# NJU-3DV/Relightable3DGaussian

Hardware: AMD Instinct MI355X
Metric: train iters/s, synthetic lego-like 800x800, 300000 Gaussians (stage-2 hot path) (higher is better)
Workload: dtype f32; 1 GPU; stage-2 train iteration (fused glue kernels + one-launch Adam): shading fwd/bwd (K=64) + rasterize fwd (S=16) + loss + rasterize bwd + Adam; 1 view/rank/step, 300000 Gaussians, 800x800, num_rendered~1755016; parallelism=dp1

## Files before the change

### include/r3dg_hip.h

```cpp
#ifndef R3DG_HIP_H
#define R3DG_HIP_H

#include <stddef.h>
#include <stdint.h>

#ifdef __cplusplus
extern "C" {
#endif

#define R3DG_OK 0
#define R3DG_EINVAL (-1)
#define R3DG_EHIP (-2)
#define R3DG_EALLOC (-3)

typedef void* (*r3dg_alloc_fn)(void* user, size_t bytes);

const char* r3dg_last_error(void);
int r3dg_release_scratch(void);
int r3dg_version(void);

int r3dg_max_features_forward(void);
int r3dg_max_features_backward(void);

size_t r3dg_geometry_state_bytes(int P);
size_t r3dg_image_state_bytes(int width, int height);
size_t r3dg_binning_state_bytes(int64_t num_rendered);
int r3dg_geometry_state_offsets(int P, size_t* offsets9);
size_t r3dg_geometry_state_total_offset(int P);
int r3dg_image_state_offsets(int width, int height, size_t* offsets3);
int r3dg_binning_state_offsets(int64_t num_rendered, size_t* offsets4);

int r3dg_rasterize_forward(void* stream, r3dg_alloc_fn geometry_alloc, r3dg_alloc_fn binning_alloc,
                           r3dg_alloc_fn image_alloc, void* alloc_user, int P, int S, int D, int M,
                           const float* d_background, int width, int height, const float* d_means3D,
                           const float* d_shs, const float* d_colors_precomp, const float* d_features,
                           const float* d_opacities, const float* d_scales, float scale_modifier,
                           const float* d_rotations, const float* d_cov3D_precomp, const float* d_viewmatrix,
                           const float* d_projmatrix, const float* d_cam_pos, float tan_fovx, float tan_fovy,
                           float cx, float cy, int prefiltered, int compute_pseudo_normal, float* d_out_color,
                           float* d_out_opacity, float* d_out_depth, float* d_out_feature, float* d_out_normal,
                           float* d_out_surface_xyz, float* d_out_weights, int32_t* d_radii, int debug,
                           int* num_rendered_out);

int r3dg_rasterize_forward_begin(void* stream, r3dg_alloc_fn geometry_alloc, r3dg_alloc_fn binning_alloc,
                                 r3dg_alloc_fn image_alloc, void* alloc_user, int P, int S, int D, int M,
                                 const float* d_background, int width, int height, const float* d_means3D,
                                 const float* d_shs, const float* d_colors_precomp, const float* d_features,
                                 const float* d_opacities, const float* d_scales, float scale_modifier,
                                 const float* d_rotations, const float* d_cov3D_precomp, const float* d_viewmatrix,
                                 const float* d_projmatrix, const float* d_cam_pos, float tan_fovx, float tan_fovy,
                                 float cx, float cy, int prefiltered, int compute_pseudo_normal, float* d_out_color,
                                 float* d_out_opacity, float* d_out_depth, float* d_out_feature, float* d_out_normal,
                                 float* d_out_surface_xyz, float* d_out_weights, int32_t* d_radii, int debug,
                                 void** ticket);
int r3dg_rasterize_forward_finish(void* ticket, int* num_rendered_out);
int r3dg_rasterize_forward_finish_on(void* ticket, void* ordering_stream, int* num_rendered_out);

int r3dg_bounded_forward_supported(int width, int height);
int r3dg_rasterize_forward_begin_bounded(void* stream, r3dg_alloc_fn geometry_alloc, r3dg_alloc_fn binning_alloc,
                                         r3dg_alloc_fn image_alloc, void* alloc_user, int P, int S, int D, int M,
                                         const float* d_background, int width, int height, const float* d_means3D,
                                         const float* d_shs, const float* d_colors_precomp, const float* d_features,
                                         const float* d_opacities, const float* d_scales, float scale_modifier,
                                         const float* d_rotations, const float* d_cov3D_precomp,
                                         const float* d_viewmatrix, const float* d_projmatrix, const float* d_cam_pos,
                                         float tan_fovx, float tan_fovy, float cx, float cy, int prefiltered,
                                         int compute_pseudo_normal, float* d_out_color, float* d_out_opacity,
                                         float* d_out_depth, float* d_out_feature, float* d_out_normal,
                                         float* d_out_surface_xyz, float* d_out_weights, int32_t* d_radii, int debug,
                                         void* ordering_stream, long long capacity, float* d_overflow_flag,
                                         unsigned int* d_overflow_count, void** ticket);
int r3dg_rasterize_forward_finish_bounded(void* ticket, void* main_stream);

int r3dg_rasterize_backward(void* stream, int P, int S, int D, int M, int R, const float* d_background, int width,
                            int height, const float* d_means3D, const float* d_shs, const float* d_features,
                            const float* d_colors_precomp, const float* d_scales, float scale_modifier,
                            const float* d_rotations, const float* d_cov3D_precomp, const float* d_viewmatrix,
                            const float* d_projmatrix, const float* d_campos, float tan_fovx, float tan_fovy,
                            const int32_t* d_radii, const void* d_geom_buffer, const void* d_binning_buffer,
                            const void* d_img_buffer, const float* d_dL_dpix, const float* d_dL_dpix_o,
                            const float* d_dL_dpix_d, const float* d_dL_dpix_f, float* d_dL_dmean2D,
                            float* d_dL_dconic, float* d_dL_dopacity, float* d_dL_dcolor, float* d_dL_dfeature,
                            float* d_dL_dmean3D, float* d_dL_dcov3D, float* d_dL_dsh, float* d_dL_dscale,
                            float* d_dL_drot, int backward_geometry, int debug);

int r3dg_rasterize_backward_split(void* stream, void* geometry_stream, int P, int S, int D, int M, int R,
                                  const float* d_background, int width, int height, const float* d_means3D,
                                  const float* d_shs, const float* d_features, const float* d_colors_precomp,
                                  const float* d_scales, float scale_modifier, const float* d_rotations,
                                  const float* d_cov3D_precomp, const float* d_viewmatrix, const float* d_projmatrix,
                                  const float* d_campos, float tan_fovx, float tan_fovy, const int32_t* d_radii,
                                  const void* d_geom_buffer, const void* d_binning_buffer, const void* d_img_buffer,
                                  const float* d_dL_dpix, const float* d_dL_dpix_o, const float* d_dL_dpix_d,
                                  const float* d_dL_dpix_f, float* d_dL_dmean2D, float* d_dL_dconic,
                                  float* d_dL_dopacity, float* d_dL_dcolor, float* d_dL_dfeature, float* d_dL_dmean3D,
                                  float* d_dL_dcov3D, float* d_dL_dsh, float* d_dL_dscale, float* d_dL_drot,
                                  int backward_geometry, int debug, int n_active_features,
                                  const int* active_features);

int r3dg_rasterize_backward_features(void* stream, int P, int S, int R, int width, int height, const void* d_geom_buffer,
                                     const void* d_binning_buffer, const void* d_img_buffer, const float* d_dL_dpix_f,
                                     float* d_dL_dfeature, int n_active_features, const int* active_features, int debug);

int r3dg_mark_visible(void* stream, int P, const float* d_means3D, const float* d_viewmatrix,
                      const float* d_projmatrix, uint8_t* d_present);

int r3dg_shade_forward(void* stream, int P, int K, int M, const float* d_base_color, const float* d_roughness,
                       const float* d_normals, const float* d_viewdirs, const float* d_incidents, const float* d_env,
                       int He, int We, const float* d_env_transform, const float* d_visibility,
                       const float* d_incident_dirs, const float* d_incident_areas, float* d_out);
#define R3DG_SHADE_TRAIN_OUTPUTS 1
#define R3DG_SHADE_TAPS_ARE_RADIANCE 2
#define R3DG_SHADE_LEAVE_ROOM 4
#define R3DG_SHADE_ROTATED 8
int r3dg_shade_forward_cached(void* stream, int P, int K, int M, const float* d_base_color, const float* d_roughness,
                              const float* d_normals, const float* d_viewdirs, const float* d_incidents,
                              const float* d_env, int He, int We, const float* d_env_transform,
                              const float* d_visibility, const float* d_incident_dirs, const float* d_incident_areas,
                              float uniform_area, const uint32_t* d_taps, int flags, float* d_out);
int r3dg_shade_build_taps(void* stream, int64_t num_samples, const float* d_incident_dirs, const float* d_env_transform,
                          int He, int We, const float* d_env_radiance, uint32_t* d_taps);
int r3dg_shade_build_transport(void* stream, int P, int K, int M, const float* d_normals, const float* d_incidents,
                               const float* d_visibility, const float* d_incident_dirs, const float* d_incident_areas,
                               float uniform_area, float* d_radiance_inout, float* d_consts);
int r3dg_shade_forward_transport(void* stream, int P, int K, const float* d_base_color, const float* d_roughness,
                                 const float* d_normals, const float* d_viewdirs, const float* d_transport,
                                 const float* d_consts, const float* d_zsamples, const float* d_incident_dirs,
                                 float* d_out);
int r3dg_shade_build_transport_rayset(void* stream, int P, int K, int M, const float* d_normals, const float* d_incidents,
                                      const float* d_visibility, const float* d_zsamples, float uniform_area,
                                      const float* d_env, int He, int We, const float* d_env_transform,
                                      float* d_transport, float* d_consts);
int r3dg_shade_build_transport_baked(void* stream, int P, int K, int M, const float* d_normals, const float* d_incidents,
                                     const float* d_visibility_sh, const float* d_zsamples, float uniform_area,
                                     const float* d_env, int He, int We, const float* d_env_transform,
                                     float* d_transport, float* d_consts);
int r3dg_visibility_sh_expand(void* stream, int P, int K, const float* d_normals, const float* d_zsamples,
                              const float* d_visibility_sh, float* d_visibility_out);
int r3dg_shade_build_split(void* stream, int P, int K, const int32_t* d_perm, const float* d_normals, const float* d_incidents,
                           const float* d_visibility, const float* d_incident_dirs, const float* d_zsamples,
                           float uniform_area, float* d_lt, float* d_vis_t, float* d_consts);
size_t r3dg_shade_env_footprints_bytes(int He, int We);
int r3dg_shade_env_footprints(void* stream, int He, int We, const float* d_env, float* d_env_footprints);
int r3dg_shade_forward_split(void* stream, int P, int K, const int32_t* d_perm, const float* d_base_color,
                             const float* d_roughness, const float* d_normals, const float* d_viewdirs, const float* d_lt,
                             const float* d_vis_t, const float* d_consts, const float* d_zsamples,
                             const float* d_env_transform, const float* d_env_footprints, int He, int We, float* d_out);
int r3dg_shade_frs_supported(int K, int M, int He, int We);
size_t r3dg_shade_frs_tables_bytes(int K);
int r3dg_shade_frs_build_tables(void* stream, int K, const float* d_zsamples, float* d_tables);
int r3dg_shade_frs_classify(void* stream, int P, const float* d_ray_normals, uint8_t* d_valid);
int r3dg_shade_frs_build_taps(void* stream, int P, int K, const float* d_ray_normals, const float* d_zsamples, int He, int We,
                              uint32_t* d_taps);
int r3dg_stream_wait_stream(void* waiter, void* signaller);
int r3dg_spin(void* stream, float microseconds);
int r3dg_store_u64_to_host(void* stream, const void* d_src, void* h_pinned_dst);
int r3dg_clock_probe(void* stream, int iters, unsigned long long* d_out3, float* d_sink, int* wall_clock_khz);

int r3dg_shade_frs_rotate(void* stream, int P, const float* d_incidents, const float* d_ray_normals, float* d_cprime);
int r3dg_shade_frs_forward(void* stream, int P, int K, const float* d_base_color, const float* d_roughness,
                           const float* d_normals, const float* d_viewdirs, const float* d_incidents, const float* d_env,
                           int He, int We, const float* d_visibility, float uniform_area, const uint32_t* d_taps,
                           const float* d_ray_normals, const float* d_zsamples, const float* d_tables,
                           const uint8_t* d_valid, const int32_t* d_invalid_list, int n_invalid, float* d_cprime, int flags,
                           float* d_out, void* listed_stream, float* d_feature_rows);
int r3dg_shade_frs_backward(void* stream, int P, int K, const float* d_base_color, const float* d_roughness,
                            const float* d_normals, const float* d_viewdirs, const float* d_incidents, const float* d_env,
                            int He, int We, const float* d_visibility, float uniform_area, const uint32_t* d_taps,
                            const float* d_ray_normals, const float* d_zsamples, const float* d_tables,
                            const uint8_t* d_valid, const int32_t* d_invalid_list, int n_invalid, const float* d_cprime,
                            float* d_dcprime, const float* d_dL_dpbr, const float* d_dL_ddiffuse_light,
                            float* d_dL_dbase_color, float* d_dL_droughness, float* d_dL_dviewdirs, float* d_dL_dincidents,
                            float* d_dL_denv, const float* d_block_absmax, int n_block_absmax, void* rotate_stream);
#define R3DG_SHADE_NO_ROTATION_BACK ((void*)(intptr_t)-1)
#define R3DG_CHAIN_LISTED_ROWS_IN_DCPRIME 1
#define R3DG_CHAIN_NO_GRADIENT_OUT 2
int r3dg_shade_frs_incident_chain(void* stream, int P, const float* d_ray_normals, const uint8_t* d_valid,
                                  const float* d_dcprime, float* d_dL_dincidents, float* d_incidents, float* d_exp_avg,
                                  float* d_exp_avg_sq, float* d_cprime, float lr, float lr_tail, float beta1, float beta2,
                                  float eps, int step, float grad_scale, const float* d_skip_flag, int chain_flags);

int r3dg_shade_backward(void* stream, int P, int K, int M, const float* d_base_color, const float* d_roughness,
                        const float* d_normals, const float* d_viewdirs, const float* d_incidents, const float* d_env,
                        int He, int We, const float* d_env_transform, const float* d_visibility,
                        const float* d_incident_dirs, const float* d_incident_areas, const float* d_dL_dpbr,
                        const float* d_dL_ddiffuse_light, float* d_dL_dbase_color, float* d_dL_droughness,
                        float* d_dL_dviewdirs, float* d_dL_dincidents, float* d_dL_denv);

int r3dg_shade_backward_cached(void* stream, int P, int K, int M, const float* d_base_color, const float* d_roughness,
                               const float* d_normals, const float* d_viewdirs, const float* d_incidents,
                               const float* d_env, int He, int We, const float* d_env_transform,
                               const float* d_visibility, const float* d_incident_dirs, const float* d_incident_areas,
                               const uint32_t* d_taps, const float* d_dL_dpbr, const float* d_dL_ddiffuse_light,
                               float* d_dL_dbase_color, float* d_dL_droughness, float* d_dL_dviewdirs,
                               float* d_dL_dincidents, float* d_dL_denv, const float* d_block_absmax,
                               int n_block_absmax);

int r3dg_render_equation_forward(void* stream, int P, int Si, int Sd, int Sv, const float* d_base_color,
                                 const float* d_roughness, const float* d_metallic, const float* d_normals,
                                 const float* d_viewdirs, const float* d_incidents_shs, const float* d_direct_shs,
                                 const float* d_visibility_shs, int sample_num, const float* d_rand_float,
                                 float* d_incident_dirs, float* d_pbr, float* d_diffuse_light);
int r3dg_render_equation_forward_complex(void* stream, int P, int Si, int Sd, int Sv, const float* d_base_color,
                                         const float* d_roughness, const float* d_metallic, const float* d_normals,
                                         const float* d_viewdirs, const float* d_incidents_shs,
                                         const float* d_direct_shs, const float* d_visibility_shs, int sample_num,
                                         float* d_incident_dirs, float* d_pbr, float* d_incident_lights,
                                         float* d_local_incident_lights, float* d_global_incident_lights,
                                         float* d_incident_visibility, float* d_diffuse_light,
                                         float* d_local_diffuse_light, float* d_accum, float* d_rgb_d, float* d_rgb_s);
int r3dg_render_equation_backward(void* stream, int P, int Si, int Sd, int Sv, const float* d_base_color,
                                  const float* d_roughness, const float* d_metallic, const float* d_normals,
                                  const float* d_viewdirs, const float* d_incidents_shs, const float* d_direct_shs,
                                  const float* d_visibility_shs, int sample_num, const float* d_incident_dirs,
                                  const float* d_dL_dpbr, const float* d_dL_ddiffuse_light, float* d_dL_dbase_color,
                                  float* d_dL_droughness, float* d_dL_dmetallic, float* d_dL_dnormals,
                                  float* d_dL_dviewdirs, float* d_dL_dincidents_shs, float* d_dL_ddirect_shs,
                                  float* d_dL_dvisibility_shs);

#define R3DG_SUM_SLOTS 32

int r3dg_stage2_activate(void* stream, int P, const float* d_xyz, const float* d_scaling_raw,
                         const float* d_rotation_raw, const float* d_opacity_raw, const float* d_normal_raw,
                         const float* d_base_raw, const float* d_rough_raw, const float* d_campos, float* d_scales,
                         float* d_rotations, float* d_opacity, float* d_normal, float* d_base_color,
                         float* d_roughness, float* d_viewdirs, const float* d_viewmatrix, float* d_features);
int r3dg_stage2_pack_features(void* stream, int P, const float* d_xyz, const float* d_viewmatrix, const float* d_normal,
                              const float* d_base_color, const float* d_roughness, const float* d_shade_out,
                              float* d_features, float* d_light_l1_sum);
int r3dg_stage2_unpack_gradients(void* stream, int P, const float* d_dL_dfeatures, const float* d_shade_out,
                                 float light_weight, float* d_dL_dpbr, float* d_dL_ddiffuse_light,
                                 float* d_block_absmax, float* d_light_l1_sum);
int r3dg_stage2_activate_backward(void* stream, int P, const float* d_xyz, const float* d_scaling_raw,
                                  const float* d_rotation_raw, const float* d_opacity_raw, const float* d_normal_raw,
                                  const float* d_base_raw, const float* d_rough_raw, const float* d_viewmatrix,
                                  const float* d_campos, const float* d_dL_dfeatures, const float* d_dL_dbase_color,
                                  const float* d_dL_droughness, const float* d_dL_dviewdirs, const float* d_dL_dscales,
                                  const float* d_dL_drotations, const float* d_dL_dopacity, const float* d_dL_dmeans3D,
                                  float* d_g_xyz, float* d_g_scaling, float* d_g_rotation, float* d_g_opacity,
                                  float* d_g_normal, float* d_g_base, float* d_g_rough);
int r3dg_stage2_loss(void* stream, int width, int height, const float* d_image, const float* d_opacity,
                     const float* d_feature, const float* d_pseudo_normal, const int32_t* d_n_contrib,
                     const float* d_gt, const float* d_background, const float* d_image_mask, float w_l1, float w_pbr,
                     float w_normal, const float* d_extra_dL_dimage, const float* d_extra_dL_dsrgb, float* d_dL_dimage,
                     float* d_dL_dopacity, float* d_dL_dfeature, float* d_sums,
                     int sparse_feature_gradients);
int r3dg_stage2_smooth_forward(void* stream, int width, int height, const float* d_opacity, const float* d_feature,
                               const int32_t* d_n_contrib, const float* d_gt, const float* d_image_mask,
                               float w_base_color, float w_roughness, float w_light, float* d_scratch, float* d_sums3);
int r3dg_stage2_smooth_backward(void* stream, int width, int height, const float* d_opacity, const float* d_feature,
                                const int32_t* d_n_contrib, const float* d_image_mask, const float* d_scratch,
                                float w_base_color, float w_roughness, float w_light, int accumulate_normal,
                                float* d_dL_dopacity, float* d_dL_dfeature);
int r3dg_stage2_smooth_fused(void* stream, int width, int height, const float* d_opacity, const float* d_feature,
                             const int32_t* d_n_contrib, const float* d_gt, const float* d_image_mask, float w_base_color,
                             float w_roughness, float w_light, int accumulate_normal, float* d_dL_dopacity,
                             float* d_dL_dfeature, float* d_sums3);
int r3dg_stage2_pbr_srgb(void* stream, int width, int height, const float* d_opacity, const float* d_feature,
                         const int32_t* d_n_contrib, const float* d_background, float* d_srgb);

int r3dg_stage2_activate_with(void* stream, int P, const float* d_xyz, const float* d_scaling_raw,
                              const float* d_rotation_raw, const float* d_opacity_raw, const float* d_normal_raw,
                              const float* d_base_raw, const float* d_rough_raw, const float* d_campos, float* d_scales,
                              float* d_rotations, float* d_opacity, float* d_normal, float* d_base_color,
                              float* d_roughness, float* d_viewdirs, const float* d_viewmatrix, float* d_features,
                              int n_env, const float* d_env_raw, float* d_env, float* d_zero, int n_zero);
int r3dg_stage2_activate_backward_with(void* stream, int P, const float* d_xyz, const float* d_scaling_raw,
                                       const float* d_rotation_raw, const float* d_opacity_raw, const float* d_normal_raw,
                                       const float* d_base_raw, const float* d_rough_raw, const float* d_viewmatrix,
                                       const float* d_campos, const float* d_dL_dfeatures, const float* d_dL_dbase_color,
                                       const float* d_dL_droughness, const float* d_dL_dviewdirs, const float* d_dL_dscales,
                                       const float* d_dL_drot, const float* d_dL_dopacity, const float* d_dL_dmeans3D,
                                       float* d_g_xyz, float* d_g_scaling, float* d_g_rotation, float* d_g_opacity,
                                       float* d_g_normal, float* d_g_base, float* d_g_rough, int He, int We,
                                       const float* d_env_raw, const float* d_env, float* d_dL_denv, float w_tv,
                                       float* d_g_env_raw, float* d_tv_sum, int consume);
int r3dg_stage2_normals_srgb(void* stream, int width, int height, const float* d_viewmatrix, float tan_fovx, float tan_fovy,
                             float cx, float cy, const float* d_opacity, const float* d_depth, float* d_pseudo_normal,
                             float* d_surface_xyz, const float* d_feature, const int32_t* d_n_contrib,
                             const float* d_background, float* d_srgb);

int r3dg_ssim_forward(void* stream, int width, int height, int channels, const float* d_x, const float* d_y,
                      float* d_partials, float* d_sum);
int r3dg_ssim_backward(void* stream, int width, int height, int channels, const float* d_x, const float* d_y,
                       const float* d_partials, float scale, float* d_grad_x);
int r3dg_ssim_forward_pair(void* stream, int width, int height, int channels, const float* d_x0, const float* d_x1,
                           const float* d_y, float* d_partials0, float* d_partials1, float* d_sum0, float* d_sum1);
int r3dg_ssim_backward_pair(void* stream, int width, int height, int channels, const float* d_x0, const float* d_x1,
                            const float* d_y, const float* d_partials0, const float* d_partials1, float scale0,
                            float scale1, float* d_grad_x0, float* d_grad_x1);

int r3dg_stage1_pack_features(void* stream, int P, const float* d_xyz, const float* d_viewmatrix, const float* d_normal,
                              float* d_features);
int r3dg_stage1_loss(void* stream, int width, int height, const float* d_image, const float* d_opacity,
                     const float* d_feature, const float* d_pseudo_normal, const int32_t* d_n_contrib, const float* d_gt,
                     const float* d_image_mask, float w_l1, float w_mask_entropy, float w_normal, float w_normal_smooth,
                     float w_depth_var, const float* d_extra_dL_dimage, float* d_edge_scratch, float* d_dL_dimage,
                     float* d_dL_dopacity, float* d_dL_dfeature, float* d_sums);
int r3dg_stage1_activate_backward(void* stream, int P, const float* d_xyz, const float* d_scaling_raw,
                                  const float* d_rotation_raw, const float* d_opacity_raw, const float* d_normal_raw,
                                  const float* d_viewmatrix, const float* d_dL_dfeatures, const float* d_dL_dscales,
                                  const float* d_dL_drotations, const float* d_dL_dopacity, const float* d_dL_dmeans3D,
                                  float* d_g_xyz, float* d_g_scaling, float* d_g_rotation, float* d_g_opacity,
                                  float* d_g_normal);

int r3dg_supervision_count(void* stream, int width, int height, const float* d_gt_depth, const float* d_image_mask,
                           uint32_t* d_count);
int r3dg_stage2_supervision(void* stream, int width, int height, const float* d_opacity, const float* d_feature,
                            const int32_t* d_n_contrib, const float* d_gt_depth, const float* d_mvs_normal,
                            const float* d_image_mask, const uint32_t* d_count, float w_depth, float w_normal_mvs,
                            int accumulate_normal, float* d_dL_dopacity, float* d_dL_dfeature, float* d_sums2);
int r3dg_stage1_depth_smooth(void* stream, int width, int height, const float* d_opacity, const float* d_feature,
                             const int32_t* d_n_contrib, const float* d_gt, float w_depth_smooth, float* d_edge_scratch,
                             float* d_dL_dopacity, float* d_dL_dfeature, float* d_sum);
int r3dg_stage1_gaussian_terms(void* stream, int P, const float* d_weights, const float* d_opacity, const float* d_normal,
                               const float* d_scales, const float* d_xyz, const float* d_campos, float w_point_entropy,
                               float w_orientation, float w_scaling, float* d_dL_dopacity, float* d_dL_dfeatures,
                               float* d_dL_dscales, float* d_dL_dmeans3D, float* d_sums3);

int r3dg_stage2_env_backward(void* stream, int He, int We, const float* d_raw, const float* d_env, float* d_dL_denv,
                             float w_tv, float* d_g_raw, float* d_tv_sum, int consume);

#define R3DG_ADAM_MAX_GROUPS 16
typedef struct r3dg_adam_group {
    float* param;
    const float* grad;
    float* exp_avg;
    float* exp_avg_sq;
    uint64_t n;
    float lr, lr_tail;
    uint32_t period, split;
} r3dg_adam_group;
int r3dg_adam_step(void* stream, int n_groups, const r3dg_adam_group* groups, float beta1, float beta2, float eps,
                   int step, float grad_scale, const float* d_skip_flag);

int r3dg_rasterize_backward_sh_adam_supported(int M);
int r3dg_rasterize_backward_split_sh_adam(void* stream, void* geometry_stream, int P, int S, int D, int M, int R,
                                          const float* d_background, int width, int height, const float* d_means3D,
                                          const float* d_shs, const float* d_features, const float* d_colors_precomp,
                                          const float* d_scales, float scale_modifier, const float* d_rotations,
                                          const float* d_cov3D_precomp, const float* d_viewmatrix,
                                          const float* d_projmatrix, const float* d_campos, float tan_fovx, float tan_fovy,
                                          const int32_t* d_radii, const void* d_geom_buffer, const void* d_binning_buffer,
                                          const void* d_img_buffer, const float* d_dL_dpix, const float* d_dL_dpix_o,
                                          const float* d_dL_dpix_d, const float* d_dL_dpix_f, float* d_dL_dmean2D,
                                          float* d_dL_dconic, float* d_dL_dopacity, float* d_dL_dcolor,
                                          float* d_dL_dfeature, float* d_dL_dmean3D, float* d_dL_dcov3D, float* d_dL_dsh,
                                          float* d_dL_dscale, float* d_dL_drot, int backward_geometry, int debug,
                                          int n_active_features, const int* active_features,
                                          const r3dg_adam_group* sh_adam, float beta1, float beta2, float eps, int step,
                                          float grad_scale, const float* d_skip_flag);

int r3dg_relight_pack_features(void* stream, int P, const float* d_xyz, const float* d_viewmatrix, const float* d_normal,
                               const float* d_base_color, const float* d_roughness, const float* d_shade_out,
                               float* d_features);
int r3dg_relight_compose(void* stream, int width, int height, float focal_x, float focal_y, float cx, float cy,
                         const float* d_viewmatrix, const float* d_light_transform, const float* d_envmap, int He, int We,
                         const float* d_image, const float* d_opacity, const float* d_feature,
                         const int32_t* d_n_contrib, float* d_pbr_env, float* d_render_env, float* d_env_only);

#define R3DG_EVAL_ROW 8
#define R3DG_EVAL_MEDIAN_STATE_WORDS 1024
int r3dg_relight_capture(void* stream, int width, int height, const float* d_feature, const float* d_opacity,
                         const int32_t* d_n_contrib, const float* d_background, const float* d_mask, float* d_pbr,
                         float* d_base_color, float* d_roughness, float* d_normal, float* d_visibility, float* d_diffuse,
                         float* d_specular, float* d_lights, float* d_local_lights, float* d_global_lights,
                         float* d_depth_var);
int r3dg_eval_image_metrics(void* stream, int width, int height, int channels, const float* d_pred, const float* d_gt,
                            const float* d_mask, const float* d_fill, int fill_is_image, double* d_tile_sums,
                            double* d_row);
int r3dg_eval_median_ratio(void* stream, int width, int height, const float* d_pred, const float* d_gt,
                           const float* d_mask, uint32_t* d_state, double* d_row);

#define R3DG_SCENE_COLUMNS 130
#define R3DG_SCENE_STAGE1_COLUMNS 62
#define R3DG_SCENE_GROUPS 13
#define R3DG_SCENE_MAX_COLUMNS 250
#define R3DG_SCENE_PLACEMENT_FLOATS 111
#define R3DG_SCENE_ZERO_INCIDENTS 1
#define R3DG_SCENE_ROTATE_SH 2
int r3dg_scene_place_records(void* stream, int P, int A, const float* d_records, const int32_t* d_column_map,
                             const float* d_placement, int flags, long long row_offset, void** dst_groups);
int r3dg_scene_place_groups(void* stream, int P, void** src_groups, const float* d_placement, int flags,
                            long long row_offset, void** dst_groups);
int r3dg_scene_pack_records(void* stream, int P, int columns, void** src_groups, float* d_records);

int r3dg_relight_quantize(void* stream, int width, int height, int channels, const float* d_image, uint8_t* d_bytes);

int r3dg_view_unpack(void* stream, int width, int height, int channels, const uint8_t* d_pixels, const float* d_background,
                     float* d_image, float* d_mask);

int r3dg_view_unpack_masked(void* stream, int width, int height, const uint8_t* d_pixels, const uint8_t* d_mask_bytes,
                            float* d_image, float* d_mask);

#define R3DG_VIEW_RESIZE_MAX_SCALE 16
int r3dg_view_resize(void* stream, int width, int height, int channels, const uint8_t* d_pixels, const uint8_t* d_mask_bytes,
                     const float* d_background, int out_width, int out_height, float* d_image, float* d_mask);

int r3dg_densify_accumulate(void* stream, int P, const float* d_viewspace_grad, const float* d_normal_grad,
                            const int32_t* d_radii, const float* d_weights, float* d_xyz_gradient_accum,
                            float* d_normal_gradient_accum, float* d_denom, float* d_weights_accum,
                            float* d_max_radii2D,
                            const float* d_skip_flag);

typedef struct r3dg_densify_config {
    int32_t mode;
    int32_t n_split;
    float grad_threshold, grad_normal_threshold, min_opacity, weights_threshold;
    float dense_size, world_size_limit, split_divisor, max_screen_size;
} r3dg_densify_config;

size_t r3dg_densify_temp_bytes(int P);
int r3dg_densify_plan(void* stream, int P, const r3dg_densify_config* config, const float* d_scaling_raw,
                      const float* d_opacity_raw, const float* d_xyz_gradient_accum,
                      const float* d_normal_gradient_accum, const float* d_denom, const float* d_weights_accum,
                      const float* d_max_radii2D, int32_t* d_src_row, int32_t* d_kind, int32_t* d_counts, void* d_temp);

#define R3DG_DENSIFY_MAX_GROUPS 24
#define R3DG_DENSIFY_ROLE_COPY 0
#define R3DG_DENSIFY_ROLE_XYZ 1
#define R3DG_DENSIFY_ROLE_SCALING 2
typedef struct r3dg_densify_group {
    const float* src_param;
    const float* src_exp_avg;
    const float* src_exp_avg_sq;
    float* dst_param;
    float* dst_exp_avg;
    float* dst_exp_avg_sq;
    uint32_t row_floats, role;
} r3dg_densify_group;
int r3dg_densify_gather(void* stream, int rows_out, const int32_t* d_src_row, const int32_t* d_kind, int n_groups,
                        const r3dg_densify_group* groups, const float* d_xyz, const float* d_scaling_raw,
                        const float* d_rotation_raw, const float* d_normal_table, float split_divisor);

int r3dg_reset_opacity(void* stream, int P, float* d_opacity_raw, float* d_exp_avg, float* d_exp_avg_sq);

size_t r3dg_knn_temp_bytes(int P);
int r3dg_knn_dist2(void* stream, int P, const float* d_points, float* d_mean_dist2, void* d_temp);

size_t r3dg_bvh_build_temp_bytes(int P);
int r3dg_bvh_build(void* stream, int P, int32_t* d_nodes, float* d_aabbs, int64_t* d_morton, void* d_temp);
int r3dg_bvh_trace_opacity(void* stream, int64_t num_rays, int num_gaussians, const int32_t* d_nodes, const float* d_aabbs,
                           const float* d_rays_o, const float* d_rays_d, const float* d_means3D,
                           const float* d_covs3D, const float* d_opacities, const float* d_normals,
                           int32_t* d_num_contributes, float* d_rendered_opacity, int32_t* d_stack_overflow);

size_t r3dg_bvh_trace_records_bytes(int num_gaussians);
int r3dg_bvh_pack_traversal(void* stream, int num_gaussians, const int32_t* d_nodes, const float* d_aabbs,
                            const float* d_means3D, const float* d_covs3D, const float* d_opacities,
                            const float* d_normals, void* d_records);
int r3dg_bvh_trace_opacity_packed(void* stream, int64_t num_rays, int num_gaussians, void* d_records, const float* d_rays_o,
                                  const float* d_rays_d, int32_t* d_num_contributes, float* d_rendered_opacity,
                                  int32_t* d_stack_overflow);

int r3dg_bvh_prepare_leaves(void* stream, int P, const float* d_means3D, const float* d_scales, const float* d_rotations,
                            int32_t* d_nodes, float* d_aabbs, float* d_covs3D_inv);
int r3dg_bvh_trace_bundles(void* stream, int num_gaussians, int K, void* d_records, const int32_t* d_nodes,
                           const float* d_zsamples, int leaf_lo, int leaf_hi, float origin_offset, float* d_visibility,
                           int32_t* d_num_contributes, float* d_dirs_out, int32_t* d_stack_overflow);

int r3dg_bvh_trace_hemisphere(void* stream, int num_gaussians, int T, void* d_records, const int32_t* d_nodes,
                              const float* d_raw_dirs, int leaf_lo, int leaf_hi, float origin_offset, float* d_visibility,
                              float* d_dirs_out, int32_t* d_num_contributes, int32_t* d_stack_overflow);
int r3dg_visibility_sh_fit(void* stream, int P, int T, int64_t steps_done, const float* d_dirs, const float* d_visibility,
                           float lr, float beta1, float beta2, float eps, float* d_coeffs, float* d_exp_avg,
                           float* d_exp_avg_sq, float* d_loss_partials);
int r3dg_visibility_sh_fit_loss_rows(int P);
int r3dg_bvh_trace_visits(void* stream, int num_gaussians, const void* d_records, uint64_t* node_and_leaf_steps);

int r3dg_bvh_trace_count(void* stream, int64_t num_rays, const int32_t* d_nodes, const float* d_aabbs,
                         const float* d_rays_o, const float* d_rays_d, int32_t* d_num_contributes,
                         int32_t* d_stack_overflow);
int r3dg_bvh_trace_fill(void* stream, int64_t num_rays, const int32_t* d_nodes, const float* d_aabbs,
                        const float* d_rays_o, const float* d_rays_d, const float* d_means3D,
                        const int32_t* d_num_contributes, const int64_t* d_offsets_inclusive, uint64_t* d_keys,
                        int32_t* d_point_list, float* d_position_list, int32_t* d_ray_id_list);

size_t r3dg_sort_temp_bytes(int64_t n);
int r3dg_sort_pairs(void* stream, int64_t n, uint64_t* d_keys_in, uint32_t* d_vals_in, uint64_t* d_keys_out,
                    uint32_t* d_vals_out, int end_bit, void* d_temp);

enum r3dg_option {
    R3DG_OPT_TILE_ORDER = 0,
    R3DG_OPT_CULL,
    R3DG_OPT_TILE_BINNING,
    R3DG_OPT_BINNING_BLOCK_K,
    R3DG_OPT_STAGE_SH_ROWS,
    R3DG_OPT_SHADE_FWD_BLOCKS_PER_CU,
    R3DG_OPT_TRACE_FORMULATION,
    R3DG_OPT_TRACE_REFILL,
    R3DG_OPT_TRACE_NODE_WEIGHT,
    R3DG_OPT_TRACE_LEAF_WEIGHT,
    R3DG_OPT_RESERVE_CUS,
    R3DG_OPT_TRACE_COUNT_VISITS,
    R3DG_OPT_BWD_LEAN,
    R3DG_OPT_COUNT
};
int r3dg_set_option(int option, int value);
int r3dg_get_option(int option, int* value);
void* r3dg_context_create(void);
void r3dg_context_destroy(void* ctx);
int r3dg_context_set_option(void* ctx, int option, int value);
int r3dg_context_make_current(void* ctx, void** previous);
int r3dg_selftest_transpose_reduce(void* stream, int N, int dpp, const float* d_in, float* d_out, int* d_chan,
                                   int* d_owner);

int r3dg_profile_enable(int on);
int r3dg_profile_pause(int paused);
int r3dg_profile_num_stages(void);
const char* r3dg_profile_stage_name(int stage);
int r3dg_profile_read(double* ms_out, int* count_out);

#ifdef __cplusplus
}
#endif
#endif
```

### relightable3dgaussian_amd/_abi.py

```python
import ctypes as C
import os
import re

HEADER = os.path.join(os.path.dirname(os.path.dirname(os.path.abspath(__file__))), "include", "r3dg_hip.h")
ALLOC_FN = C.CFUNCTYPE(C.c_void_p, C.c_void_p, C.c_size_t)
_ALLOC_FN_DECL = "typedef void* (*r3dg_alloc_fn)(void* user, size_t bytes)"

_SCALARS = {"int": C.c_int, "unsigned int": C.c_uint, "long long": C.c_longlong, "unsigned long long": C.c_ulonglong,
            "float": C.c_float, "double": C.c_double, "size_t": C.c_size_t, "int32_t": C.c_int32, "uint32_t": C.c_uint32,
            "int64_t": C.c_int64, "uint64_t": C.c_uint64, "uint8_t": C.c_uint8}
_RETURNS = dict(_SCALARS, **{"void": None, "void *": C.c_void_p, "const char *": C.c_char_p})
_HOST_POINTEES = ("int", "size_t", "double", "uint64_t")
_INT_EXPR = r"(?:0[xX][0-9a-fA-F]+|\d+|<<|>>|[\s()+\-*|&~])+"


def parse(text):
    def fail(pos, what):
        raise ValueError("r3dg_hip.h:%d: %s" % (text.count("\n", 0, pos) + 1, what))

    def blank(m):
        return "\n" * m.group(0).count("\n")

    def declarator(pos, decl, what):
        tok = decl.replace("*", " * ").split()
        name = tok.pop() if tok else ""
        stars = tok.count("*")
        base = " ".join(t for t in tok if t not in ("const", "*"))
        if not re.fullmatch(r"[A-Za-z_]\w*", name) or name in _SCALARS or not base or tok[len(tok) - stars:] != ["*"] * stars:
            fail(pos, "%s %r is not `type name`" % (what, decl.strip()))
        return base, stars, name

    text = re.sub(r"/\*.*?\*/", blank, text, flags=re.S)
    text = re.sub(r"^#ifdef __cplusplus\n.*?^#endif", blank, text, flags=re.S | re.M)
    prototypes, constants, structs = {}, {}, {}

    def define(m):
        name, value = m.group(1), m.group(2).strip()
        if name.startswith("R3DG_") and value:
            if name == "R3DG_SHADE_NO_ROTATION_BACK":
                value = "-1"
            if not re.fullmatch(_INT_EXPR, value):
                fail(m.start(), "#define %s: %r is not an integer expression" % (name, value))
            constants[name] = int(eval(value, {"__builtins__": {}}))
        return ""
    text = re.sub(r"^#[ \t]*define[ \t]+(\w+)(.*)$", define, text, flags=re.M)
    text = re.sub(r"^#.*$", "", text, flags=re.M)

    def struct(m):
        fields = []
        for decl in filter(str.strip, m.group(2).split(";")):
            first, *more = decl.split(",")
            for d in [first] + [declarator(m.start(), first, "field")[0] + " " + d for d in more]:
                base, stars, name = declarator(m.start(), d, "field")
                if base not in _SCALARS or stars > 1:
                    fail(m.start(), "field %r: unknown type" % d.strip())
                fields.append((name, C.c_void_p if stars else _SCALARS[base]))
        structs[m.group(1)] = type(m.group(1), (C.Structure,), {"_fields_": fields})
        return blank(m)
    text = re.sub(r"typedef\s+struct\s+(r3dg_\w+)\s*\{([^{}]*)\}\s*\1\s*;", struct, text)

    enum = re.search(r"enum\s+r3dg_option\s*\{([^{}]*)\}\s*;", text)
    entries = [[s.strip() for s in e.split("=")] for e in enum.group(1).split(",")] if enum else [[""]]
    if any(not re.fullmatch(r"R3DG_OPT_[A-Z0-9_]+", e[0]) or e[1:] not in ([], [str(i)]) for i, e in enumerate(entries)) or \
            entries[-1][0] != "R3DG_OPT_COUNT":
        fail(enum.start() if enum else 0, "enum r3dg_option: expected R3DG_OPT_* numbered from 0, R3DG_OPT_COUNT last")
    options = tuple(e[0][len("R3DG_OPT_"):] for e in entries[:-1])
    text = text[:enum.start()] + blank(enum) + text[enum.end():]

    for m in re.finditer(r"\s*([^;]*[^;\s])\s*;?", text):
        stmt, at = " ".join(m.group(1).split()), m.start(1)
        if stmt == _ALLOC_FN_DECL:
            continue
        p = re.fullmatch(r"([\w\s*]+?)\s*\b(r3dg_\w+)\s*\(([^()]*)\)", stmt)
        ret = " ".join(p.group(1).replace("*", " * ").split()) if p else None
        if ret not in _RETURNS:
            fail(at, "not a prototype this reader understands: %r" % stmt)
        args = []
        for decl in ([] if p.group(3).strip() == "void" else p.group(3).split(",")):
            base, stars, name = declarator(at, decl, p.group(2) + ": parameter")
            known = base in _SCALARS or (base == "void" and stars > 0)
            if stars == 0 and (known or base == "r3dg_alloc_fn"):
                args.append(ALLOC_FN if base == "r3dg_alloc_fn" else _SCALARS[base])
            elif stars == 2 and known:
                args.append(C.POINTER(C.c_void_p))
            elif stars == 1 and (base == "void" or base in structs or (known and name.startswith("d_"))):
                args.append(C.c_void_p)
            elif stars == 1 and base in _HOST_POINTEES:
                args.append(C.POINTER(_SCALARS[base]))
            else:
                fail(at, "%s: cannot classify parameter %r" % (p.group(2), decl.strip()))
        prototypes[p.group(2)] = (_RETURNS[ret], args)
    return prototypes, constants, options, structs


with open(HEADER) as _f:
    prototypes, constants, options, structs = parse(_f.read())
```

### relightable3dgaussian_amd/csrc/capi_stage.hip

```cpp
#include "capi_internal.hpp"

using namespace r3dg;

extern "C" {

int r3dg_stage2_activate(void* stream_, int P, const float* xyz, const float* scaling_raw, const float* rotation_raw,
                         const float* opacity_raw, const float* normal_raw, const float* base_raw,
                         const float* rough_raw, const float* campos, float* scales, float* rot, float* opacity,
                         float* normal, float* base_color, float* roughness, float* viewdirs, const float* viewmatrix,
                         float* features)
{
    return r3dg_stage2_activate_with(stream_, P, xyz, scaling_raw, rotation_raw, opacity_raw, normal_raw, base_raw, rough_raw,
                                     campos, scales, rot, opacity, normal, base_color, roughness, viewdirs, viewmatrix, features,
                                     0, nullptr, nullptr, nullptr, 0);
}

int r3dg_stage2_activate_with(void* stream_, int P, const float* xyz, const float* scaling_raw, const float* rotation_raw,
                              const float* opacity_raw, const float* normal_raw, const float* base_raw,
                              const float* rough_raw, const float* campos, float* scales, float* rot, float* opacity,
                              float* normal, float* base_color, float* roughness, float* viewdirs, const float* viewmatrix,
                              float* features, int n_env, const float* env_raw, float* env, float* zero, int n_zero)
{
    if (P < 0) return invalid("stage2_activate: bad P");
    if (n_env < 0 || n_zero < 0) return invalid("stage2_activate: bad side-job size");
    if (n_env > 0 && (!env_raw || !env)) return invalid("stage2_activate: null texture buffer");
    if (n_zero > 0 && !zero) return invalid("stage2_activate: null buffer to zero");
    if (P == 0 && n_env == 0 && n_zero == 0) return R3DG_OK;
    if (P == 0) {
        return guarded([&]() -> int {
            launch_s2_activate((hipStream_t)stream_, 0, nullptr, nullptr, nullptr, nullptr, nullptr, nullptr, nullptr, nullptr,
                               nullptr, nullptr, nullptr, nullptr, nullptr, nullptr, nullptr, nullptr, nullptr, n_env, env_raw,
                               env, zero, n_zero);
            return R3DG_OK;
        });
    }
    if (!xyz || !scaling_raw || !rotation_raw || !opacity_raw || !normal_raw || !scales || !rot || !opacity || !normal)
        return invalid("stage2_activate: null buffer");
    if (base_raw && (!rough_raw || !campos || !base_color || !roughness || !viewdirs))
        return invalid("stage2_activate: stage-2 inputs/outputs incomplete");
    if (features && (!base_raw || !viewmatrix)) return invalid("stage2_activate: feature rows need the stage-2 inputs and the view matrix");
    return guarded([&]() -> int {
        StageTimer t((hipStream_t)stream_, ST_S2_ACTIVATE);
        launch_s2_activate((hipStream_t)stream_, P, xyz, scaling_raw, rotation_raw, opacity_raw, normal_raw, base_raw,
                           rough_raw, campos, scales, rot, opacity, normal, base_color, roughness, viewdirs, viewmatrix, features,
                           n_env, env_raw, env, zero, n_zero);
        return R3DG_OK;
    });
}

int r3dg_stage2_pack_features(void* stream_, int P, const float* xyz, const float* viewmatrix, const float* normal,
                              const float* base_color, const float* roughness, const float* shade_out, float* features,
                              float* light_l1_sum)
{
    if (P < 0) return invalid("stage2_pack_features: bad P");
    if (P == 0) return R3DG_OK;
    if (!xyz || !viewmatrix || !normal || !base_color || !roughness || !shade_out || !features)
        return invalid("stage2_pack_features: null buffer");
    return guarded([&]() -> int {
        StageTimer t((hipStream_t)stream_, ST_S2_PACK);
        launch_s2_pack((hipStream_t)stream_, P, xyz, viewmatrix, normal, base_color, roughness, shade_out, features,
                       light_l1_sum);
        return R3DG_OK;
    });
}

int r3dg_stage2_unpack_gradients(void* stream_, int P, const float* dL_dfeatures, const float* shade_out,
                                 float light_weight, float* dL_dpbr, float* dL_ddiffuse, float* block_absmax,
                                 float* light_l1_sum)
{
    if (P < 0) return invalid("stage2_unpack_gradients: bad P");
    if (P == 0) return R3DG_OK;
    if (!dL_dfeatures || !shade_out || !dL_dpbr || !dL_ddiffuse) return invalid("stage2_unpack_gradients: null buffer");
    return guarded([&]() -> int {
        StageTimer t((hipStream_t)stream_, ST_S2_UNPACK);
        launch_s2_unpack((hipStream_t)stream_, P, dL_dfeatures, shade_out, light_weight, dL_dpbr, dL_ddiffuse, block_absmax,
                         light_l1_sum);
        return R3DG_OK;
    });
}

int r3dg_stage2_activate_backward(void* stream_, int P, const float* xyz, const float* scaling_raw,
                                  const float* rotation_raw, const float* opacity_raw, const float* normal_raw,
                                  const float* base_raw, const float* rough_raw, const float* viewmatrix,
                                  const float* campos, const float* dL_dfeatures, const float* dL_dbase_shade,
                                  const float* dL_drough_shade, const float* dL_dviewdirs, const float* dL_dscales,
                                  const float* dL_drot, const float* dL_dopacity, const float* dL_dmeans3D, float* g_xyz,
                                  float* g_scaling, float* g_rotation, float* g_opacity, float* g_normal, float* g_base,
                                  float* g_rough)
{
    return r3dg_stage2_activate_backward_with(stream_, P, xyz, scaling_raw, rotation_raw, opacity_raw, normal_raw, base_raw,
                                              rough_raw, viewmatrix, campos, dL_dfeatures, dL_dbase_shade, dL_drough_shade,
                                              dL_dviewdirs, dL_dscales, dL_drot, dL_dopacity, dL_dmeans3D, g_xyz, g_scaling,
                                              g_rotation, g_opacity, g_normal, g_base, g_rough, 0, 0, nullptr, nullptr, nullptr,
                                              0.f, nullptr, nullptr, 0);
}

int r3dg_stage2_activate_backward_with(void* stream_, int P, const float* xyz, const float* scaling_raw,
                                  const float* rotation_raw, const float* opacity_raw, const float* normal_raw,
                                  const float* base_raw, const float* rough_raw, const float* viewmatrix,
                                  const float* campos, const float* dL_dfeatures, const float* dL_dbase_shade,
                                  const float* dL_drough_shade, const float* dL_dviewdirs, const float* dL_dscales,
                                  const float* dL_drot, const float* dL_dopacity, const float* dL_dmeans3D, float* g_xyz,
                                  float* g_scaling, float* g_rotation, float* g_opacity, float* g_normal, float* g_base,
                                  float* g_rough, int He, int We,
                                       const float* env_raw, const float* env, float* dL_denv, float w_tv,
                                       float* g_env_raw, float* tv_sum, int consume)
{
    if (P < 0) return invalid("stage2_activate_backward: bad P");
    if (He < 0 || We < 0) return invalid("stage2_activate_backward: bad texture size");
    const bool env_job = He * We != 0;
    if (env_job && (!env_raw || !env || !dL_denv || !g_env_raw)) return invalid("stage2_activate_backward: null texture buffer");
    if (P == 0) return env_job ? r3dg_stage2_env_backward(stream_, He, We, env_raw, env, dL_denv, w_tv, g_env_raw, tv_sum, consume) : R3DG_OK;
    if (!base_raw || !rough_raw || !dL_dfeatures || !dL_dbase_shade || !dL_drough_shade || !g_base || !g_rough)
        return invalid("stage2_activate_backward: null buffer");
    if (g_xyz != nullptr &&
        (!xyz || !scaling_raw || !rotation_raw || !opacity_raw || !normal_raw || !viewmatrix || !campos || !dL_dviewdirs ||
         !dL_dscales || !dL_drot || !dL_dopacity || !dL_dmeans3D || !g_scaling || !g_rotation || !g_opacity || !g_normal))
        return invalid("stage2_activate_backward: null buffer");
    return guarded([&]() -> int {
        StageTimer t((hipStream_t)stream_, ST_S2_ACTIVATE_BWD);
        launch_s2_activate_backward((hipStream_t)stream_, P, xyz, scaling_raw, rotation_raw, opacity_raw, normal_raw,
                                    base_raw, rough_raw, viewmatrix, campos, dL_dfeatures, dL_dbase_shade,
                                    dL_drough_shade, dL_dviewdirs, dL_dscales, dL_drot, dL_dopacity, dL_dmeans3D, g_xyz,
                                    g_scaling, g_rotation, g_opacity, g_normal, g_base, g_rough, env_job ? He : 0, env_job ? We : 0,
                                    env_job ? env_raw : nullptr, env, dL_denv, w_tv, g_env_raw, tv_sum, consume);
        return R3DG_OK;
    });
}

int r3dg_stage2_loss(void* stream_, int width, int height, const float* image, const float* opacity,
                     const float* feature, const float* pseudo_normal, const int32_t* n_contrib, const float* gt,
                     const float* bg, const float* image_mask, float w_l1, float w_pbr, float w_normal,
                     const float* extra_dimage, const float* extra_dsrgb, float* dL_dimage, float* dL_dopacity,
                     float* dL_dfeature, float* sums, int sparse_feature_gradients)
{
    if (width < 0 || height < 0) return invalid("stage2_loss: bad image size");
    if ((long long)width * height == 0) return R3DG_OK;
    if (!image || !opacity || !feature || !pseudo_normal || !n_contrib || !gt || !bg || !dL_dimage || !dL_dopacity ||
        !dL_dfeature || !sums)
        return invalid("stage2_loss: null buffer");
    return guarded([&]() -> int {
        StageTimer t((hipStream_t)stream_, ST_S2_LOSS);
        launch_s2_loss((hipStream_t)stream_, width * height, image, opacity, feature, pseudo_normal, n_contrib, gt, bg,
                       image_mask, w_l1, w_pbr, w_normal, extra_dimage, extra_dsrgb, dL_dimage, dL_dopacity, dL_dfeature, sums,
                       sparse_feature_gradients);
        return R3DG_OK;
    });
}

int r3dg_stage2_smooth_forward(void* stream_, int width, int height, const float* opacity, const float* feature,
                               const int32_t* n_contrib, const float* gt, const float* image_mask, float w_base_color,
                               float w_roughness, float w_light, float* scratch, float* sums3)
{
    if (width < 0 || height < 0) return invalid("stage2_smooth_forward: bad image size");
    if ((long long)width * height == 0) return R3DG_OK;
    if (!opacity || !feature || !n_contrib || !gt || !scratch || !sums3) return invalid("stage2_smooth_forward: null buffer");
    return guarded([&]() -> int {
        StageTimer t((hipStream_t)stream_, ST_S2_LOSS);
        launch_s2_smooth_forward((hipStream_t)stream_, width, height, opacity, feature, n_contrib, gt, image_mask,
                                 w_base_color, w_roughness, w_light, scratch, sums3);
        return R3DG_OK;
    });
}

int r3dg_stage2_smooth_backward(void* stream_, int width, int height, const float* opacity, const float* feature,
                                const int32_t* n_contrib, const float* image_mask, const float* scratch, float w_base_color,
                                float w_roughness, float w_light, int accumulate_normal, float* dL_dopacity,
                                float* dL_dfeature)
{
    if (width < 0 || height < 0) return invalid("stage2_smooth_backward: bad image size");
    if ((long long)width * height == 0) return R3DG_OK;
    if (!opacity || !feature || !n_contrib || !scratch || !dL_dopacity || !dL_dfeature)
        return invalid("stage2_smooth_backward: null buffer");
    return guarded([&]() -> int {
        StageTimer t((hipStream_t)stream_, ST_S2_LOSS);
        launch_s2_smooth_backward((hipStream_t)stream_, width, height, opacity, feature, n_contrib, image_mask, scratch,
                                  w_base_color != 0.f, w_roughness != 0.f, w_light != 0.f, accumulate_normal, dL_dopacity,
                                  dL_dfeature);
        return R3DG_OK;
    });
}

int r3dg_stage2_smooth_fused(void* stream_, int width, int height, const float* opacity, const float* feature,
                             const int32_t* n_contrib, const float* gt, const float* image_mask, float w_base_color,
                             float w_roughness, float w_light, int accumulate_normal, float* dL_dopacity, float* dL_dfeature,
                             float* sums3)
{
    if (width < 0 || height < 0) return invalid("stage2_smooth_fused: bad image size");
    if ((long long)width * height == 0) return R3DG_OK;
    if (!opacity || !feature || !n_contrib || !gt || !dL_dopacity || !dL_dfeature || !sums3)
        return invalid("stage2_smooth_fused: null buffer");
    return guarded([&]() -> int {
        StageTimer t((hipStream_t)stream_, ST_S2_LOSS);
        launch_s2_smooth_fused((hipStream_t)stream_, width, height, opacity, feature, n_contrib, gt, image_mask, w_base_color,
                               w_roughness, w_light, accumulate_normal, dL_dopacity, dL_dfeature, sums3);
        return R3DG_OK;
    });
}

int r3dg_stage1_pack_features(void* stream_, int P, const float* xyz, const float* viewmatrix, const float* normal,
                              float* features)
{
    if (P < 0) return invalid("stage1_pack_features: bad P");
    if (P == 0) return R3DG_OK;
    if (!xyz || !viewmatrix || !normal || !features) return invalid("stage1_pack_features: null buffer");
    return guarded([&]() -> int {
        StageTimer t((hipStream_t)stream_, ST_S2_PACK);
        launch_s1_pack((hipStream_t)stream_, P, xyz, viewmatrix, normal, features);
        return R3DG_OK;
    });
}

int r3dg_stage1_loss(void* stream_, int width, int height, const float* image, const float* opacity,
                     const float* feature, const float* pseudo_normal, const int32_t* n_contrib, const float* gt,
                     const float* image_mask, float w_l1, float w_mask_entropy, float w_normal, float w_normal_smooth,
                     float w_depth_var, const float* extra_dimage, float* edge_scratch, float* dL_dimage,
                     float* dL_dopacity, float* dL_dfeature, float* sums)
{
    if (width < 0 || height < 0) return invalid("stage1_loss: bad image size");
    if ((long long)width * height == 0) return R3DG_OK;
    if (!image || !opacity || !feature || !pseudo_normal || !n_contrib || !gt || !dL_dimage || !dL_dopacity ||
        !dL_dfeature || !sums)
        return invalid("stage1_loss: null buffer");
    if (w_normal_smooth != 0.f && !edge_scratch) return invalid("stage1_loss: the normal-smoothness term needs edge_scratch");
    return guarded([&]() -> int {
        StageTimer t((hipStream_t)stream_, ST_S2_LOSS);
        if (w_normal_smooth != 0.f)
            launch_s1_edge((hipStream_t)stream_, width, height, feature, opacity, n_contrib, gt, edge_scratch, sums + 4 * R3DG_SUM_SLOTS);
        launch_s1_loss((hipStream_t)stream_, width, height, image, opacity, feature, pseudo_normal, n_contrib, gt, image_mask,
                       w_l1, w_mask_entropy, w_normal, w_normal_smooth, w_depth_var, extra_dimage,
                       w_normal_smooth != 0.f ? edge_scratch : nullptr, dL_dimage, dL_dopacity, dL_dfeature, sums);
        return R3DG_OK;
    });
}

int r3dg_stage1_activate_backward(void* stream_, int P, const float* xyz, const float* scaling_raw,
                                  const float* rotation_raw, const float* opacity_raw, const float* normal_raw,
                                  const float* viewmatrix, const float* dL_dfeatures, const float* dL_dscales,
                                  const float* dL_drot, const float* dL_dopacity, const float* dL_dmeans3D, float* g_xyz,
                                  float* g_scaling, float* g_rotation, float* g_opacity, float* g_normal)
{
    if (P < 0) return invalid("stage1_activate_backward: bad P");
    if (P == 0) return R3DG_OK;
    if (!xyz || !scaling_raw || !rotation_raw || !opacity_raw || !normal_raw || !viewmatrix || !dL_dfeatures ||
        !dL_dscales || !dL_drot || !dL_dopacity || !dL_dmeans3D || !g_xyz || !g_scaling || !g_rotation || !g_opacity ||
        !g_normal)
        return invalid("stage1_activate_backward: null buffer");
    return guarded([&]() -> int {
        StageTimer t((hipStream_t)stream_, ST_S2_ACTIVATE_BWD);
        launch_s1_activate_backward((hipStream_t)stream_, P, xyz, scaling_raw, rotation_raw, opacity_raw, normal_raw,
                                    viewmatrix, dL_dfeatures, dL_dscales, dL_drot, dL_dopacity, dL_dmeans3D, g_xyz,
                                    g_scaling, g_rotation, g_opacity, g_normal);
        return R3DG_OK;
    });
}

int r3dg_stage2_pbr_srgb(void* stream_, int width, int height, const float* opacity, const float* feature,
                         const int32_t* n_contrib, const float* bg, float* srgb)
{
    if (width < 0 || height < 0) return invalid("stage2_pbr_srgb: bad image size");
    if ((long long)width * height == 0) return R3DG_OK;
    if (!opacity || !feature || !n_contrib || !bg || !srgb) return invalid("stage2_pbr_srgb: null buffer");
    return guarded([&]() -> int {
        launch_s2_pbr_srgb((hipStream_t)stream_, width * height, opacity, feature, n_contrib, bg, srgb);
        return R3DG_OK;
    });
}

int r3dg_stage2_normals_srgb(void* stream_, int width, int height, const float* viewmatrix, float tan_fovx, float tan_fovy,
                             float cx, float cy, const float* opacity, const float* depth, float* pseudo_normal,
                             float* surface_xyz, const float* feature, const int32_t* n_contrib, const float* bg, float* srgb)
{
    if (width < 0 || height < 0) return invalid("stage2_normals_srgb: bad image size");
    if ((long long)width * height == 0) return R3DG_OK;
    if ((long long)width * height > 0x7fffffffLL) return invalid("stage2_normals_srgb: image too large");
    if (!viewmatrix || !opacity || !depth || !pseudo_normal || !surface_xyz || !feature || !n_contrib || !bg || !srgb)
        return invalid("stage2_normals_srgb: null buffer");
    return guarded([&]() -> int {
        StageTimer t((hipStream_t)stream_, ST_NORMAL);
        const float focal_y = height / (2.0f * tan_fovy), focal_x = width / (2.0f * tan_fovx);
        launch_s2_normals_srgb((hipStream_t)stream_, width, height, viewmatrix, focal_x, focal_y, cx, cy, opacity, depth,
                               pseudo_normal, surface_xyz, feature, n_contrib, bg, srgb);
        return R3DG_OK;
    });
}

int r3dg_ssim_forward_pair(void* stream_, int width, int height, int channels, const float* x0, const float* x1,
                           const float* y, float* partials0, float* partials1, float* sum0, float* sum1)
{
    if (width < 0 || height < 0 || channels < 0) return invalid("ssim_forward: bad shape");
    if ((long long)width * height * channels == 0) return R3DG_OK;
    if (!x0 || !y || !partials0 || (x1 && !partials1)) return invalid("ssim_forward: null buffer");
    if ((long long)channels * 2 > 65535) return invalid("ssim_forward: too many channels");
    return guarded([&]() -> int {
        StageTimer t((hipStream_t)stream_, ST_SSIM);
        const float* x[2] = {x0, x1};
        float* partials[2] = {partials0, partials1};
        float* sum[2] = {sum0, sum1};
        launch_ssim_forward((hipStream_t)stream_, width, height, channels, x1 ? 2 : 1, x, y, partials, sum);
        return R3DG_OK;
    });
}

int r3dg_ssim_backward_pair(void* stream_, int width, int height, int channels, const float* x0, const float* x1,
                            const float* y, const float* partials0, const float* partials1, float scale0, float scale1,
                            float* grad_x0, float* grad_x1)
{
    if (width < 0 || height < 0 || channels < 0) return invalid("ssim_backward: bad shape");
    if ((long long)width * height * channels == 0) return R3DG_OK;
    if (!x0 || !y || !partials0 || !grad_x0 || (x1 && (!partials1 || !grad_x1))) return invalid("ssim_backward: null buffer");
    if ((long long)channels * 2 > 65535) return invalid("ssim_backward: too many channels");
    return guarded([&]() -> int {
        StageTimer t((hipStream_t)stream_, ST_SSIM);
        const float* x[2] = {x0, x1};
        float* partials[2] = {const_cast<float*>(partials0), const_cast<float*>(partials1)};
        const float scale[2] = {scale0, scale1};
        float* grad[2] = {grad_x0, grad_x1};
        launch_ssim_backward((hipStream_t)stream_, width, height, channels, x1 ? 2 : 1, x, y, partials, scale, grad);
        return R3DG_OK;
    });
}

int r3dg_ssim_forward(void* stream_, int width, int height, int channels, const float* x, const float* y,
                      float* partials, float* sum)
{
    return r3dg_ssim_forward_pair(stream_, width, height, channels, x, nullptr, y, partials, nullptr, sum, nullptr);
}

int r3dg_ssim_backward(void* stream_, int width, int height, int channels, const float* x, const float* y,
                       const float* partials, float scale, float* grad_x)
{
    return r3dg_ssim_backward_pair(stream_, width, height, channels, x, nullptr, y, partials, nullptr, scale, 0.f, grad_x,
                                   nullptr);
}

int r3dg_stage2_env_backward(void* stream_, int He, int We, const float* raw, const float* env, float* dL_denv,
                             float w_tv, float* g_raw, float* tv_sum, int consume)
{
    if (He < 0 || We < 0) return invalid("stage2_env_backward: bad texture size");
    if (He * We == 0) return R3DG_OK;
    if (!raw || !env || !dL_denv || !g_raw) return invalid("stage2_env_backward: null buffer");
    return guarded([&]() -> int {
        launch_s2_env_backward((hipStream_t)stream_, He, We, raw, env, dL_denv, w_tv, g_raw, tv_sum, consume);
        return R3DG_OK;
    });
}

int r3dg_adam_step(void* stream_, int n_groups, const r3dg_adam_group* groups, float beta1, float beta2, float eps,
                   int step, float grad_scale, const float* skip_flag)
{
    if (n_groups < 0 || n_groups > R3DG_ADAM_MAX_GROUPS) return invalid("adam_step: bad group count");
    if (step < 1) return invalid("adam_step: step counts from 1");
    if (n_groups == 0) return R3DG_OK;
    if (!groups) return invalid("adam_step: null group table");
    for (int i = 0; i < n_groups; i++) {
        if (groups[i].n >= (1ull << 32)) return invalid("adam_step: group larger than 2^32 elements");
        if (groups[i].n && (!groups[i].param || !groups[i].grad || !groups[i].exp_avg || !groups[i].exp_avg_sq))
            return invalid("adam_step: null buffer in group");
    }
    return guarded([&]() -> int {
        StageTimer t((hipStream_t)stream_, ST_ADAM);
        launch_adam((hipStream_t)stream_, n_groups, groups, beta1, beta2, eps, step, grad_scale, skip_flag);
        return R3DG_OK;
    });
}

int r3dg_relight_pack_features(void* stream_, int P, const float* xyz, const float* viewmatrix, const float* normal,
                               const float* base_color, const float* roughness, const float* shade_out, float* features)
{
    if (P < 0) return invalid("relight_pack_features: bad P");
    if (P == 0) return R3DG_OK;
    if (!xyz || !viewmatrix || !normal || !base_color || !roughness || !shade_out || !features)
        return invalid("relight_pack_features: null buffer");
    if ((size_t)features & 15) return invalid("relight_pack_features: features must be 16-byte aligned");
    return guarded([&]() -> int {
        StageTimer t((hipStream_t)stream_, ST_RELIGHT_PACK);
        launch_relight_pack((hipStream_t)stream_, P, xyz, viewmatrix, normal, base_color, roughness, shade_out, features);
        return R3DG_OK;
    });
}

int r3dg_relight_compose(void* stream_, int width, int height, float focal_x, float focal_y, float cx, float cy,
                         const float* viewmatrix, const float* light_transform, const float* envmap, int He, int We,
                         const float* image, const float* opacity, const float* feature, const int32_t* n_contrib,
                         float* pbr_env, float* render_env, float* env_only)
{
    if (width < 0 || height < 0 || He < 1 || We < 1) return invalid("relight_compose: bad shape");
    if ((long long)width * height == 0) return R3DG_OK;
    if ((long long)width * height >= (1ll << 31)) return invalid("relight_compose: image too large");
    if (!viewmatrix || !envmap || !opacity || !feature || !n_contrib) return invalid("relight_compose: null buffer");
    if (render_env && !image) return invalid("relight_compose: render_env needs the rendered image");
    if (!(focal_x > 0.f) || !(focal_y > 0.f)) return invalid("relight_compose: focal lengths must be positive");
    return guarded([&]() -> int {
        StageTimer t((hipStream_t)stream_, ST_RELIGHT_COMPOSE);
        launch_relight_compose((hipStream_t)stream_, width, height, focal_x, focal_y, cx, cy, viewmatrix, light_transform,
                               envmap, He, We, image, opacity, feature, n_contrib, pbr_env, render_env, env_only);
        return R3DG_OK;
    });
}

int r3dg_relight_capture(void* stream_, int width, int height, const float* feature, const float* opacity,
                         const int32_t* n_contrib, const float* background, const float* mask, float* pbr,
                         float* base_color, float* roughness, float* normal, float* visibility, float* diffuse,
                         float* specular, float* lights, float* local_lights, float* global_lights, float* depth_var)
{
    if (width < 0 || height < 0) return invalid("relight_capture: bad shape");
    if ((long long)width * height == 0) return R3DG_OK;
    if ((long long)width * height >= (1ll << 31)) return invalid("relight_capture: image too large");
    if (!feature || !opacity || !n_contrib) return invalid("relight_capture: null buffer");
    if ((pbr || mask) && !background) return invalid("relight_capture: the pbr map and the mask need a background");
    const CaptureMaps maps = {pbr, base_color, roughness, normal, visibility, diffuse, specular, lights, local_lights,
                              global_lights, depth_var};
    return guarded([&]() -> int {
        launch_relight_capture((hipStream_t)stream_, width, height, feature, opacity, n_contrib, background, mask, maps);
        return R3DG_OK;
    });
}

int r3dg_eval_image_metrics(void* stream_, int width, int height, int channels, const float* pred, const float* gt,
                            const float* mask, const float* fill, int fill_is_image, double* tile_sums, double* row)
{
    if (width < 1 || height < 1 || channels < 1 || channels > 3) return invalid("eval_image_metrics: bad shape");
    if ((long long)width * height >= (1ll << 31)) return invalid("eval_image_metrics: image too large");
    if (!pred || !gt || !tile_sums || !row) return invalid("eval_image_metrics: null buffer");
    if (fill && !mask) return invalid("eval_image_metrics: a fill needs a mask");
    return guarded([&]() -> int {
        launch_eval_image_metrics((hipStream_t)stream_, width, height, channels, pred, gt, mask, fill, fill_is_image, tile_sums,
                                  row);
        return R3DG_OK;
    });
}

int r3dg_eval_median_ratio(void* stream_, int width, int height, const float* pred, const float* gt, const float* mask,
                           uint32_t* state, double* row)
{
    if (width < 0 || height < 0) return invalid("eval_median_ratio: bad shape");
    if ((long long)width * height >= (1ll << 31)) return invalid("eval_median_ratio: image too large");
    if (!state || !row) return invalid("eval_median_ratio: null buffer");
    if ((long long)width * height != 0 && (!pred || !gt)) return invalid("eval_median_ratio: null image");
    return guarded([&]() -> int {
        launch_eval_median_ratio((hipStream_t)stream_, width, height, pred, gt, mask, state, row);
        return R3DG_OK;
    });
}

int r3dg_densify_accumulate(void* stream_, int P, const float* viewspace_grad, const float* normal_grad,
                            const int32_t* radii, const float* weights, float* xyz_accum, float* normal_accum,
                            float* denom, float* weights_accum, float* max_radii2D, const float* skip_flag)
{
    if (P < 0) return invalid("densify_accumulate: bad P");
    if (P == 0) return R3DG_OK;
    if (!viewspace_grad || !radii || !weights || !xyz_accum || !normal_accum || !denom || !weights_accum || !max_radii2D)
        return invalid("densify_accumulate: null buffer");
    return guarded([&]() -> int {
        StageTimer t((hipStream_t)stream_, ST_DENSIFY);
        launch_densify_accumulate((hipStream_t)stream_, P, viewspace_grad, normal_grad, radii, weights, xyz_accum,
                                  normal_accum, denom, weights_accum, max_radii2D, skip_flag);
        return R3DG_OK;
    });
}

size_t r3dg_densify_temp_bytes(int P) { return densify_temp_bytes((size_t)(P > 0 ? P : 0)); }

int r3dg_densify_plan(void* stream_, int P, const r3dg_densify_config* cfg, const float* scaling_raw,
                      const float* opacity_raw, const float* xyz_accum, const float* normal_accum, const float* denom,
                      const float* weights_accum, const float* max_radii2D, int32_t* src_row, int32_t* kind,
                      int32_t* counts, void* temp)
{
    if (P < 0) return invalid("densify_plan: bad P");
    if (!cfg || !counts) return invalid("densify_plan: null config / counts");
    if (cfg->mode != 0 && cfg->mode != 1) return invalid("densify_plan: mode is 0 (densify_and_prune) or 1 (prune)");
    if (cfg->n_split < 1 || cfg->n_split > 8) return invalid("densify_plan: n_split out of range");
    if (cfg->mode == 0 && !(cfg->split_divisor > 0.f)) return invalid("densify_plan: split_divisor must be positive");
    if ((int64_t)P * (cfg->n_split > 2 ? cfg->n_split : 2) >= (1ll << 31)) return invalid("densify_plan: row map too large");
    if (P > 0 && (!scaling_raw || !opacity_raw || !xyz_accum || !normal_accum || !denom || !weights_accum ||
                  !max_radii2D || !src_row || !kind || !temp))
        return invalid("densify_plan: null buffer");
    return guarded([&]() -> int {
        hipStream_t s = (hipStream_t)stream_;
        if (P == 0) {
            R3DG_HIP(hipMemsetAsync(counts, 0, 8 * sizeof(int32_t), s));
            return R3DG_OK;
        }
        StageTimer t(s, ST_DENSIFY);
        launch_densify_plan(s, P, *cfg, scaling_raw, opacity_raw, xyz_accum, normal_accum, denom, weights_accum,
                            max_radii2D, src_row, kind, counts, temp);
        return R3DG_OK;
    });
}

int r3dg_densify_gather(void* stream_, int rows_out, const int32_t* src_row, const int32_t* kind, int n_groups,
                        const r3dg_densify_group* groups, const float* xyz, const float* scaling_raw,
                        const float* rotation_raw, const float* normal_table, float split_divisor)
{
    if (rows_out < 0) return invalid("densify_gather: bad row count");
    if (n_groups < 0 || n_groups > R3DG_DENSIFY_MAX_GROUPS) return invalid("densify_gather: bad group count");
    if (rows_out == 0 || n_groups == 0) return R3DG_OK;
    if (!groups || !src_row || !kind) return invalid("densify_gather: null table / row map");
    for (int i = 0; i < n_groups; i++) {
        const r3dg_densify_group& g = groups[i];
        if (g.row_floats == 0 || !g.src_param || !g.dst_param) return invalid("densify_gather: empty group");
        if ((g.src_exp_avg != nullptr) != (g.src_exp_avg_sq != nullptr) ||
            (g.src_exp_avg && (!g.dst_exp_avg || !g.dst_exp_avg_sq)))
            return invalid("densify_gather: moments must be given as complete source/destination pairs");
        if (g.role == R3DG_DENSIFY_ROLE_XYZ && g.row_floats != 3) return invalid("densify_gather: xyz rows are 3 floats");
        if (g.role == R3DG_DENSIFY_ROLE_SCALING && g.row_floats != 3)
            return invalid("densify_gather: scaling rows are 3 floats");
        if (g.role > R3DG_DENSIFY_ROLE_SCALING) return invalid("densify_gather: unknown role");
        if (g.role != R3DG_DENSIFY_ROLE_COPY && (!xyz || !scaling_raw || !rotation_raw || !(split_divisor > 0.f)))
            return invalid("densify_gather: split sources missing");
        if ((uint64_t)rows_out * g.row_floats >= (1ull << 41)) return invalid("densify_gather: group too large");
    }
    return guarded([&]() -> int {
        StageTimer t((hipStream_t)stream_, ST_DENSIFY);
        launch_densify_gather((hipStream_t)stream_, rows_out, src_row, kind, n_groups, groups, xyz, scaling_raw,
                              rotation_raw, normal_table, split_divisor);
        return R3DG_OK;
    });
}

int r3dg_reset_opacity(void* stream_, int P, float* opacity_raw, float* exp_avg, float* exp_avg_sq)
{
    if (P < 0) return invalid("reset_opacity: bad P");
    if (P == 0) return R3DG_OK;
    if (!opacity_raw) return invalid("reset_opacity: null buffer");
    return guarded([&]() -> int {
        launch_reset_opacity((hipStream_t)stream_, P, 0.01f, opacity_raw, exp_avg, exp_avg_sq);
        return R3DG_OK;
    });
}

}
```

### relightable3dgaussian_amd/csrc/launchers.hpp

```cpp
#pragma once
#include "common.hpp"

namespace r3dg {

__attribute__((visibility("hidden"))) int persistent_cus();

void release_gradient_records();
void launch_mark_visible(hipStream_t s, int P, const float* means3D, const float* vm, uint8_t* present);
void launch_preprocess(hipStream_t s, int P, int D, int M, const float* means3D, const float* scales, float scale_modifier,
                       const float* rotations, const float* opacities, const float* shs, uint8_t* clamped,
                       const float* cov3D_precomp, const float* colors_precomp, const float* vm, const float* pm,
                       const float* cam_pos, int W, int H, float tan_fovx, float tan_fovy, float focal_x, float focal_y,
                       int* radii, float* means2D, float* depths, float* cov3Ds, float* rgb, float* conic_opacity,
                       float* splat, int gx, int gy, uint32_t* tiles_touched, uint32_t* block_sums,
                       unsigned long long* total, bool scan_now, uint32_t* zero_words, int zero_n);
void launch_duplicate_with_keys(hipStream_t s, int P, const float* means2D, const float* depths,
                                const uint32_t* tiles_touched, const uint32_t* block_offsets, uint32_t* point_offsets,
                                uint64_t* keys, uint32_t* values, const int* radii, int gx, int gy);
void launch_identify_tile_ranges(hipStream_t s, int L, const uint64_t* keys, uint32_t* ranges);
void launch_tile_order(hipStream_t s, int T, const uint32_t* ranges, uint32_t* order, uint32_t small_cap, uint32_t* big_list,
                       uint32_t* big_count);
void launch_render_forward(hipStream_t s, int W, int H, int S, const uint32_t* tile_order, const uint32_t* ranges,
                           const uint32_t* point_list, const float* splat, const float* features, float* final_T,
                           uint32_t* n_contrib, const float* bg, float* out_color, float* out_opacity, float* out_depth,
                           float* out_feature, float* out_weights);
void launch_pseudo_normal(hipStream_t s, int W, int H, const float* vm, float focal_x, float focal_y, float cx, float cy,
                          const float* opacities, const float* depths, float* normals, float* surface_xyz, bool debug);
void launch_render_backward(hipStream_t s, int P, int W, int H, int S, int n_active, const int* active,
                            const uint32_t* tile_order, const uint32_t* ranges, const uint32_t* point_list, const float* bg,
                            const float* splat, const float* features, const float* final_Ts, const uint32_t* n_contrib,
                            const float* dL_dpix, const float* dL_dpix_o, const float* dL_dpix_d, const float* dL_dpix_f,
                            float* dL_dmean2D, float* dL_dconic, float* dL_dopacity, float* dL_dcolor, float* dL_dfeature,
                            int bg_geom);
void launch_render_backward_features(hipStream_t s, int W, int H, int S, int n_active, const int* active,
                                     const uint32_t* tile_order, const uint32_t* ranges, const uint32_t* point_list,
                                     const float* splat, const float* final_Ts, const uint32_t* n_contrib,
                                     const float* dL_dpix_f, float* dL_dfeature);
struct ShAdamArgs {
    r3dg_adam_group g;
    float beta1, beta2, eps, bias1, inv_sqrt_bias2, grad_scale;
    const float* skip_flag;
};
bool preprocess_backward_applies_adam(int M);
void launch_preprocess_backward(hipStream_t s, int P, int D, int M, const float* means, const int* radii, const float* shs,
                                const uint8_t* clamped, const float* scales, const float* rotations, float scale_modifier,
                                const float* cov3Ds, const float* vm, const float* proj, float h_x, float h_y,
                                float tan_fovx, float tan_fovy, const float* campos, float* dL_dmean2D,
                                const float* dL_dconic, const float* conic_opacity, int W, int H, float* dL_dmeans,
                                const float* dL_dcolor, float* dL_dcov3D, float* dL_dsh, float* dL_dscale, float* dL_drot,
                                const ShAdamArgs* adam);
void launch_shade_forward(hipStream_t s, int P, int K, int M, const float* base_color, const float* roughness,
                          const float* normals, const float* viewdirs, const float* incidents, const float* env, int He,
                          int We, const float* tr, const float* visibility, const float* dirs, const float* areas,
                          float* out, const uint32_t* taps, bool train_outputs, float uniform_area, bool taps_are_radiance,
                          bool leave_room);
size_t shade_frs_table_floats(int K);
bool shade_frs_supported(int K, int M, int He, int We);
void launch_shade_frs_build_tables(hipStream_t s, int K, const float* zsamples, float* tables);
void launch_shade_frs_classify(hipStream_t s, int P, const float* ray_normals, uint8_t* valid);
void launch_shade_frs_build_taps(hipStream_t s, int P, int K, const float* ray_normals, const float* zsamples, int He,
                                 int We, uint32_t* taps);
void launch_shade_frs_forward_aux(hipStream_t s, int P, const float* incidents, const float* ray_normals, float* cprime);
void launch_shade_frs_forward_main(hipStream_t s, int P, int K, const float* base_color, const float* roughness,
                                   const float* normals, const float* viewdirs, const float* env, int He, int We,
                                   const float* visibility, float uniform_area, const uint32_t* taps,
                                   const float* ray_normals, const float* tables, const uint8_t* valid, const float* cprime,
                                   bool leave_room, float* out, float* feat);
void launch_shade_frs_forward_listed(hipStream_t s, int K, const float* base_color, const float* roughness,
                                     const float* normals, const float* viewdirs, const float* incidents, const float* env,
                                     int He, int We, const float* visibility, const float* ray_normals,
                                     const float* zsamples, float uniform_area, const int* invalid_list, int n_invalid,
                                     float* out, float* feat);
void launch_shade_frs_incident_chain(hipStream_t s, int P, const float* ray_normals, const uint8_t* valid, const float* dcp,
                                     float* d_inc, float* incidents, float* exp_avg, float* exp_avg_sq, float* cprime,
                                     float lr, float lr_tail, float beta1, float beta2, float eps, int step,
                                     float grad_scale, const float* skip_flag, int listed_in_dcprime, bool write_gradient);
const unsigned int* launch_shade_frs_backward_aux(hipStream_t s, int P, const float* g_pbr, const float* g_diff,
                                                  const float* block_absmax, int n_block_absmax, int* gmax_n);
void launch_shade_frs_backward_main(hipStream_t s, int P, int K, const float* base_color, const float* roughness,
                                    const float* normals, const float* viewdirs, const float* env, int He, int We,
                                    const float* visibility, float uniform_area, const uint32_t* taps,
                                    const float* ray_normals, const float* tables, const uint8_t* valid, const float* cprime,
                                    float* dcp, const float* g_pbr, const float* g_diff, float* d_base, float* d_rough,
                                    float* d_view, float* d_env, const unsigned int* gmax, int gmax_n);
void launch_shade_frs_backward_rotate(hipStream_t s, int P, const float* ray_normals, const float* dcp, float* d_inc,
                                      const uint8_t* valid);
void launch_shade_frs_backward_listed(hipStream_t s, int K, const float* base_color, const float* roughness,
                                      const float* normals, const float* viewdirs, const float* incidents, const float* env,
                                      int He, int We, const float* visibility, const float* ray_normals,
                                      const float* zsamples, float uniform_area, const int* invalid_list, int n_invalid,
                                      const float* g_pbr, const float* g_diff, float* d_base, float* d_rough, float* d_view,
                                      float* d_inc, float* d_env, const unsigned int* gmax, int gmax_n);
void launch_shade_build_taps(hipStream_t s, size_t n, const float* dirs, const float* tr, int He, int We, const float* env,
                             uint32_t* taps);
void launch_shade_build_split(hipStream_t s, int P, int K, const int* perm, const float* normals, const float* incidents,
                              const float* visibility, const float* dirs, const float* zsamples, float uniform_area,
                              float* lt, float* vis_t, float* consts);
void launch_shade_forward_split(hipStream_t s, int P, int K, const int* perm, const float* base_color,
                                const float* roughness, const float* normals, const float* viewdirs, const float* lt,
                                const float* vis_t, const float* consts, const float* zsamples, const float* tr,
                                const float* env4, int He, int We, float* out);
void launch_shade_env_footprints(hipStream_t s, int He, int We, const float* env, float* fp);
void launch_shade_build_transport(hipStream_t s, int P, int K, int M, const float* normals, const float* incidents,
                                  const float* visibility, const float* dirs, const float* areas, float uniform_area,
                                  float* radiance_to_transport, float* consts);
void launch_shade_build_transport_rayset(hipStream_t s, int P, int K, int M, const float* normals, const float* incidents,
                                         const float* visibility, const float* zsamples, float uniform_area, const float* env,
                                         int He, int We, const float* tr, float* transport, float* consts);
void launch_shade_build_transport_baked(hipStream_t s, int P, int K, int M, const float* normals, const float* incidents,
                                        const float* visibility_sh, const float* zsamples, float uniform_area, const float* env,
                                        int He, int We, const float* tr, float* transport, float* consts);
void launch_visibility_sh_expand(hipStream_t s, int P, int K, const float* normals, const float* zsamples,
                                 const float* visibility_sh, float* out);
void launch_shade_forward_transport(hipStream_t s, int P, int K, const float* base_color, const float* roughness,
                                    const float* normals, const float* viewdirs, const float* transport, const float* consts,
                                    const float* zsamples, const float* dirs, float* out);
void launch_shade_backward(hipStream_t s, int P, int K, int M, const float* base_color, const float* roughness,
                           const float* normals, const float* viewdirs, const float* incidents, const float* env, int He,
                           int We, const float* tr, const float* visibility, const float* dirs, const float* areas,
                           const float* g_pbr, const float* g_diff, float* d_base, float* d_rough, float* d_view,
                           float* d_inc, float* d_env, const uint32_t* taps, const float* block_absmax, int n_block_absmax);
void launch_re_forward(hipStream_t s, bool complex_, int P, int Si, int Sd, int Sv, const float* base_color,
                       const float* roughness, const float* metallic, const float* normals, const float* viewdirs,
                       const float* inc, const float* direct, const float* vis, int K, const float* rand_float,
                       float* incident_dirs, float* out_pbr, float* out_lights, float* out_local, float* out_global,
                       float* out_vis, float* out_diffuse, float* out_local_diffuse, float* out_accum, float* out_rgb_d,
                       float* out_rgb_s);
void launch_re_backward(hipStream_t s, int P, int Si, int Sd, int Sv, const float* base_color, const float* roughness,
                        const float* metallic, const float* normals, const float* viewdirs, const float* inc,
                        const float* direct, const float* vis, int K, const float* incident_dirs, const float* dL_dpbr,
                        const float* dL_ddl, float* dL_dbase, float* dL_drough, float* dL_dmetal, float* dL_dnormals,
                        float* dL_dviewdirs, float* dL_dinc, float* dL_ddirect, float* dL_dvis);
void launch_s2_activate(hipStream_t s, int P, const float* xyz, const float* scaling_raw, const float* rotation_raw,
                        const float* opacity_raw, const float* normal_raw, const float* base_raw, const float* rough_raw,
                        const float* campos, float* scales, float* rot, float* opacity, float* normal, float* base_color,
                        float* roughness, float* viewdirs, const float* viewmatrix, float* features, int n_env,
                        const float* env_raw, float* env, float* zero, int n_zero);
void launch_s2_pack(hipStream_t s, int P, const float* xyz, const float* viewmatrix, const float* normal,
                    const float* base_color, const float* roughness, const float* shade_out, float* features,
                    float* light_l1_sum);
void launch_s2_unpack(hipStream_t s, int P, const float* dL_dfeatures, const float* shade_out, float light_weight,
                      float* dL_dpbr, float* dL_ddiffuse, float* block_absmax, float* light_l1_sum);
void launch_s2_activate_backward(hipStream_t s, int P, const float* xyz, const float* scaling_raw, const float* rotation_raw,
                                 const float* opacity_raw, const float* normal_raw, const float* base_raw,
                                 const float* rough_raw, const float* viewmatrix, const float* campos,
                                 const float* dL_dfeatures, const float* dL_dbase_shade, const float* dL_drough_shade,
                                 const float* dL_dviewdirs, const float* dL_dscales, const float* dL_drot,
                                 const float* dL_dopacity, const float* dL_dmeans3D, float* g_xyz, float* g_scaling,
                                 float* g_rotation, float* g_opacity, float* g_normal, float* g_base, float* g_rough, int He,
                                 int We, const float* env_raw, const float* env, float* dL_denv, float w_tv,
                                 float* g_env_raw, float* tv_sum, int consume);
void launch_s2_loss(hipStream_t s, int HW, const float* image, const float* opacity, const float* feature,
                    const float* pseudo_normal, const int* n_contrib, const float* gt, const float* bg,
                    const float* image_mask, float w_l1, float w_pbr, float w_normal, const float* extra_dimage,
                    const float* extra_dsrgb, float* dL_dimage, float* dL_dopacity, float* dL_dfeature, float* sums,
                    int sparse);
void launch_s2_smooth_forward(hipStream_t s, int W, int H, const float* opacity, const float* feature, const int* n_contrib,
                              const float* gt, const float* image_mask, float w_base, float w_rough, float w_light,
                              float* scratch, float* sums3);
void launch_s2_smooth_fused(hipStream_t s, int W, int H, const float* opacity, const float* feature, const int* n_contrib,
                            const float* gt, const float* image_mask, float w_base, float w_rough, float w_light,
                            int accumulate_normal, float* dL_dopacity, float* dL_dfeature, float* sums3);
void launch_s2_smooth_backward(hipStream_t s, int W, int H, const float* opacity, const float* feature, const int* n_contrib,
                               const float* image_mask, const float* scratch, int has_base, int has_rough, int has_light,
                               int accumulate_normal, float* dL_dopacity, float* dL_dfeature);
void launch_s2_pbr_srgb(hipStream_t s, int HW, const float* opacity, const float* feature, const int* n_contrib,
                        const float* bg, float* srgb);
void launch_s2_normals_srgb(hipStream_t s, int W, int H, const float* vm, float focal_x, float focal_y, float cx, float cy,
                            const float* opacity, const float* depths, float* normals, float* surface_xyz,
                            const float* feature, const int* n_contrib, const float* bg, float* srgb);
void launch_ssim_forward(hipStream_t s, int W, int H, int C, int n_images, const float* const* x, const float* y,
                         float* const* partials, float* const* sum);
void launch_ssim_backward(hipStream_t s, int W, int H, int C, int n_images, const float* const* x, const float* y,
                          float* const* partials, const float* scale, float* const* grad_x);
void launch_adam(hipStream_t s, int n_groups, const r3dg_adam_group* groups, float beta1, float beta2, float eps, int step,
                 float grad_scale, const float* skip_flag);
void launch_s1_pack(hipStream_t s, int P, const float* xyz, const float* viewmatrix, const float* normal, float* features);
void launch_s1_edge(hipStream_t s, int W, int H, const float* feature, const float* opacity, const int* n_contrib,
                    const float* gt, float* edge_g, float* sum_out);
void launch_s1_loss(hipStream_t s, int W, int H, const float* image, const float* opacity, const float* feature,
                    const float* pseudo_normal, const int* n_contrib, const float* gt, const float* image_mask, float w_l1,
                    float w_entropy, float w_normal, float w_smooth, float w_var, const float* extra_dimage,
                    const float* edge_g, float* dL_dimage, float* dL_dopacity, float* dL_dfeature, float* sums);
void launch_s1_activate_backward(hipStream_t s, int P, const float* xyz, const float* scaling_raw, const float* rotation_raw,
                                 const float* opacity_raw, const float* normal_raw, const float* viewmatrix,
                                 const float* dL_dfeatures, const float* dL_dscales, const float* dL_drot,
                                 const float* dL_dopacity, const float* dL_dmeans3D, float* g_xyz, float* g_scaling,
                                 float* g_rotation, float* g_opacity, float* g_normal);
void launch_s2_env_backward(hipStream_t s, int He, int We, const float* raw, const float* env, float* dL_denv, float w_tv,
                            float* g_raw, float* tv_sum, int consume);
uint32_t tile_sort_small_cap();
void launch_tile_sort(hipStream_t s, int T, const uint32_t* tile_order, const uint32_t* ranges, const uint32_t* big_list,
                      uint32_t* big_count, uint64_t* keys, uint32_t* vals, uint64_t* scratch, bool entries);
void launch_tile_binning(hipStream_t s, int P, int T, const float* means2D, const float* depths, const int* radii,
                         const uint32_t* tiles_touched, uint32_t* block_offsets, int gx, int gy, uint32_t* tile_counts,
                         uint32_t* cursor, uint32_t* ranges, uint32_t* point_offsets, uint64_t* entries,
                         unsigned long long* total, long long capacity, float* overflow_flag, unsigned int* overflow_count,
                         bool fused, uint32_t* order, uint32_t small_cap, uint32_t* big_list, uint32_t* big_count);
int tile_binning_max_tiles();
void launch_densify_accumulate(hipStream_t s, int P, const float* viewspace_grad, const float* normal_grad, const int* radii,
                               const float* weights, float* xyz_accum, float* normal_accum, float* denom,
                               float* weights_accum, float* max_radii2D, const float* skip_flag);
size_t densify_temp_bytes(size_t P);
void launch_densify_plan(hipStream_t s, int P, const r3dg_densify_config& cfg, const float* scaling_raw,
                         const float* opacity_raw, const float* xyz_accum, const float* normal_accum, const float* denom,
                         const float* weights_accum, const float* max_radii2D, int32_t* src_row, int32_t* kind,
                         int32_t* counts, void* temp);
void launch_densify_gather(hipStream_t s, int P_out, const int32_t* src_row, const int32_t* kind, int n_groups,
                           const r3dg_densify_group* groups, const float* xyz, const float* scaling_raw,
                           const float* rotation_raw, const float* normal_table, float split_divisor);
void launch_reset_opacity(hipStream_t s, int P, float cap, float* opacity_raw, float* exp_avg, float* exp_avg_sq);
void launch_relight_pack(hipStream_t s, int P, const float* xyz, const float* viewmatrix, const float* normal,
                         const float* base_color, const float* roughness, const float* shade_out, float* features);
void launch_relight_compose(hipStream_t s, int W, int H, float fx, float fy, float cx, float cy, const float* viewmatrix,
                            const float* tr, const float* env, int He, int We, const float* image, const float* opacity,
                            const float* feature, const int* n_contrib, float* pbr_env, float* render_env, float* env_only);
struct CaptureMaps {
    float *pbr, *base_color, *roughness, *normal, *visibility, *diffuse, *specular, *lights, *local_lights, *global_lights,
        *depth_var;
};
void launch_relight_capture(hipStream_t s, int W, int H, const float* feature, const float* opacity, const int* n_contrib,
                            const float* background, const float* mask, const CaptureMaps& maps);
struct SceneGroups {
    float* p[R3DG_SCENE_GROUPS];
};
void launch_scene_place_records(hipStream_t s, int P, int A, const float* records, const int* column_map, const float* placement,
                                int flags, long long row_offset, const SceneGroups& dst);
void launch_scene_place_groups(hipStream_t s, int P, const SceneGroups& src, const float* placement, int flags,
                               long long row_offset, const SceneGroups& dst);
void launch_scene_pack_records(hipStream_t s, int P, int columns, const SceneGroups& src, float* records);
void launch_relight_quantize(hipStream_t s, int W, int H, int C, const float* image, uint8_t* bytes);
void launch_view_unpack(hipStream_t s, int W, int H, int C, const uint8_t* pixels, const float* background, float* image,
                        float* mask);
void launch_view_unpack_masked(hipStream_t s, int W, int H, const uint8_t* pixels, const uint8_t* mask_bytes, float* image,
                               float* mask);
void launch_view_resize(hipStream_t s, int W, int H, int C, const uint8_t* pixels, const uint8_t* mask_bytes, const float* background,
                        int OW, int OH, float* image, float* mask);
void launch_eval_metric_tiles(hipStream_t s, int W, int H, int C, const float* pred, const float* gt, const float* mask,
                              const float* fill, int fill_is_image, double* tile_sums);
void launch_eval_image_metrics(hipStream_t s, int W, int H, int C, const float* pred, const float* gt, const float* mask,
                               const float* fill, int fill_is_image, double* tile_sums, double* row);
void launch_eval_median_ratio(hipStream_t s, int W, int H, const float* pred, const float* gt, const float* mask,
                              uint32_t* state, double* row);
size_t knn_temp_bytes(size_t P);
void knn_dist2(hipStream_t s, int P, const float* pts, float* dists, void* temp);
size_t bvh_build_temp_bytes(size_t P);
void bvh_build(hipStream_t s, int P, int32_t* nodes, float* aabbs, uint64_t* morton, void* temp);
void bvh_prepare_leaves(hipStream_t s, int P, const float* means, const float* scales, const float* rotations, int32_t* nodes,
                        float* aabbs, float* covs_inv);
void bvh_trace_count(hipStream_t s, int num_rays, const int32_t* nodes, const float* aabbs, const float* rays_o,
                     const float* rays_d, int32_t* counts, int* overflow);
void bvh_trace_fill(hipStream_t s, int num_rays, const int32_t* nodes, const float* aabbs, const float* rays_o,
                    const float* rays_d, const float* means, const int32_t* counts, const int64_t* offsets_inclusive,
                    uint64_t* keys, int32_t* points, float* positions, int32_t* ray_ids);
void bvh_trace_opacity(hipStream_t s, int num_rays, int P, const int32_t* nodes, const float* aabbs, const float* rays_o,
                       const float* rays_d, const float* means, const float* covs, const float* opac, const float* normals,
                       int32_t* contributes, float* out, int* overflow);
size_t bvh_trace_records_bytes(size_t P);
void bvh_pack_traversal(hipStream_t s, int P, const int32_t* nodes, const float* aabbs, const float* means,
                        const float* covs, const float* opac, const float* normals, void* records);
void bvh_trace_visits(hipStream_t s, int P, const void* records, unsigned long long out[2]);
void bvh_trace_opacity_packed(hipStream_t s, int num_rays, int P, void* records, const float* rays_o, const float* rays_d,
                              int32_t* contributes, float* out, int* overflow);
void bvh_trace_bundles(hipStream_t s, int P, int K, void* records, const int32_t* nodes, const float* zsamples, int leaf_lo,
                       int leaf_hi, float origin_offset, float* out, int32_t* contributes, float* dirs_out, int* overflow);
void bvh_trace_hemisphere(hipStream_t s, int P, int T, void* records, const int32_t* nodes, const float* raw_dirs, int leaf_lo,
                          int leaf_hi, float origin_offset, float* out, float* dirs_out, int32_t* contributes, int* overflow);
int visibility_sh_fit_loss_rows(int P);
void visibility_sh_fit(hipStream_t s, int P, int T, long long steps_done, const float* dirs, const float* visibility, float lr,
                       float beta1, float beta2, float eps, float* coeffs, float* exp_avg, float* exp_avg_sq,
                       float* loss_partials);
void launch_transpose_selftest(hipStream_t s, int N, int dpp, const float* in, float* out, int* chan, int* owner);

}
```

### relightable3dgaussian_amd/csrc/stage2_glue.hip

```cpp
#include "launchers.hpp"
#include "glue_math.hpp"
#include "pseudo_normal.hpp"
#include "r3dg_hip.h"

namespace r3dg {

struct ActivateSide {
    int nb_main;
    int n_env;
    const float* env_raw;
    float* env;
    float* zero;
    int n_zero;
};

__global__ void __launch_bounds__(256)
s2_activate_kernel(int P, const float* __restrict__ xyz, const float* __restrict__ scaling_raw,
                   const float* __restrict__ rotation_raw, const float* __restrict__ opacity_raw,
                   const float* __restrict__ normal_raw, const float* __restrict__ base_raw,
                   const float* __restrict__ rough_raw, const float* __restrict__ campos,
                   float* __restrict__ scales, float* __restrict__ rot, float* __restrict__ opacity,
                   float* __restrict__ normal, float* __restrict__ base_color, float* __restrict__ roughness,
                   float* __restrict__ viewdirs, const float* __restrict__ viewmatrix, float* __restrict__ features,
                   ActivateSide side)
{
    if ((int)blockIdx.x >= side.nb_main) {
        const int nb_side = (int)gridDim.x - side.nb_main;
        for (int k = ((int)blockIdx.x - side.nb_main) * 256 + (int)threadIdx.x; k < side.n_env; k += nb_side * 256) {
            const float r = side.env_raw[k];
            side.env[k] = r > 20.f ? r : log1pf(expf(r));
        }
        for (int k = ((int)blockIdx.x - side.nb_main) * 256 + (int)threadIdx.x; k < side.n_zero; k += nb_side * 256)
            side.zero[k] = 0.f;
        return;
    }
    const int i = blockIdx.x * 256 + threadIdx.x;
    if (i >= P) return;
    const size_t i3 = 3 * (size_t)i, i4 = 4 * (size_t)i;
#pragma unroll
    for (int c = 0; c < 3; c++) scales[i3 + c] = __expf(scaling_raw[i3 + c]);
    {
        const float q[4] = {rotation_raw[i4], rotation_raw[i4 + 1], rotation_raw[i4 + 2], rotation_raw[i4 + 3]};
        const float inv = 1.f / fmaxf(sqrtf(q[0] * q[0] + q[1] * q[1] + q[2] * q[2] + q[3] * q[3]), 1e-12f);
#pragma unroll
        for (int c = 0; c < 4; c++) rot[i4 + c] = q[c] * inv;
    }
    opacity[i] = sigmoidf_(opacity_raw[i]);
    float inv, nrm[3];
    {
        const float v[3] = {normal_raw[i3], normal_raw[i3 + 1], normal_raw[i3 + 2]};
        normalize3(v, 1e-3f, nrm, inv);
        normal[i3] = nrm[0]; normal[i3 + 1] = nrm[1]; normal[i3 + 2] = nrm[2];
    }
    if (base_raw != nullptr) {
        float bc[3];
#pragma unroll
        for (int c = 0; c < 3; c++) base_color[i3 + c] = bc[c] = 0.03f + 0.77f * sigmoidf_(base_raw[i3 + c]);
        const float rg = 0.09f + 0.9f * sigmoidf_(rough_raw[i]);
        roughness[i] = rg;
        const float p[3] = {xyz[i3], xyz[i3 + 1], xyz[i3 + 2]};
        const float d[3] = {campos[0] - p[0], campos[1] - p[1], campos[2] - p[2]};
        float o[3];
        normalize3(d, 1e-12f, o, inv);
        viewdirs[i3] = o[0]; viewdirs[i3 + 1] = o[1]; viewdirs[i3 + 2] = o[2];
        if (features != nullptr) {
            const float depth = p[0] * viewmatrix[2] + p[1] * viewmatrix[6] + p[2] * viewmatrix[10] + viewmatrix[14];
            float* f = features + 16 * (size_t)i;
            *reinterpret_cast<float2*>(f) = make_float2(depth, depth * depth);
            f[5] = nrm[0]; f[6] = nrm[1]; f[7] = nrm[2];
            *reinterpret_cast<float4*>(f + 8) = make_float4(bc[0], bc[1], bc[2], rg);
        }
    }
}

__global__ void __launch_bounds__(256)
s2_pack_features_kernel(int P, const float* __restrict__ xyz, const float* __restrict__ viewmatrix,
                        const float* __restrict__ normal, const float* __restrict__ base_color,
                        const float* __restrict__ roughness, const float* __restrict__ shade_out,
                        float* __restrict__ features, float* __restrict__ light_l1_sum)
{
    __shared__ float s_part[4];
    const int i = blockIdx.x * 256 + threadIdx.x;
    float l1 = 0.f;
    if (i < P) {
        const size_t i3 = 3 * (size_t)i;
        const float depth = xyz[i3] * viewmatrix[2] + xyz[i3 + 1] * viewmatrix[6] + xyz[i3 + 2] * viewmatrix[10] +
                            viewmatrix[14];
        const float* so = shade_out + 19 * (size_t)i;
        const float dl[3] = {so[3], so[4], so[5]};
        float4* f = reinterpret_cast<float4*>(features + 16 * (size_t)i);
        f[0] = make_float4(depth, depth * depth, so[0], so[1]);
        f[1] = make_float4(so[2], normal[i3], normal[i3 + 1], normal[i3 + 2]);
        f[2] = make_float4(base_color[i3], base_color[i3 + 1], base_color[i3 + 2], roughness[i]);
        f[3] = make_float4(dl[0], dl[1], dl[2], so[18]);
        const float m = (dl[0] + dl[1] + dl[2]) / 3.f;
        l1 = fabsf(dl[0] - m) + fabsf(dl[1] - m) + fabsf(dl[2] - m);
    }
    const float tot = block_sum_256(l1, s_part);
    if (threadIdx.x == 0 && light_l1_sum != nullptr) atomicAdd(sum_slot(light_l1_sum), tot);
}


__global__ void __launch_bounds__(256)
s2_unpack_kernel(int P, const float* __restrict__ dL_dfeatures, const float* __restrict__ shade_out, float light_weight,
                 float* __restrict__ dL_dpbr, float* __restrict__ dL_ddiffuse, float* __restrict__ block_absmax,
                 float* __restrict__ light_l1_sum)
{
    __shared__ float s_m[4];
    __shared__ float s_l1[4];
    const int i = blockIdx.x * 256 + threadIdx.x;
    float m = 0.f, l1 = 0.f;
    bool bad = false;
    if (i < P) {
        const float4* g = reinterpret_cast<const float4*>(dL_dfeatures + 16 * (size_t)i);
        const float4 g0 = g[0], g1 = g[1], g3 = g[3];
        const size_t i3 = 3 * (size_t)i;
        dL_dpbr[i3] = g0.z; dL_dpbr[i3 + 1] = g0.w; dL_dpbr[i3 + 2] = g1.x;
        const float* so = shade_out + 19 * (size_t)i;
        const float dl[3] = {so[3], so[4], so[5]};
        const float mean = (dl[0] + dl[1] + dl[2]) / 3.f;
        const float s[3] = {signf_(dl[0] - mean), signf_(dl[1] - mean), signf_(dl[2] - mean)};
        const float sm = (s[0] + s[1] + s[2]) / 3.f;
        l1 = fabsf(dl[0] - mean) + fabsf(dl[1] - mean) + fabsf(dl[2] - mean);
        const float d0 = g3.x + light_weight * (s[0] - sm), d1 = g3.y + light_weight * (s[1] - sm),
                    d2 = g3.z + light_weight * (s[2] - sm);
        dL_ddiffuse[i3] = d0; dL_ddiffuse[i3 + 1] = d1; dL_ddiffuse[i3 + 2] = d2;
        const float v[6] = {fabsf(g0.z), fabsf(g0.w), fabsf(g1.x), fabsf(d0), fabsf(d1), fabsf(d2)};
#pragma unroll
        for (int c = 0; c < 6; c++) {
            bad = bad || !(v[c] <= 3.0e38f);
            m = fmaxf(m, v[c]);
        }
    }
    if (light_l1_sum != nullptr) {
        const float tot = block_sum_256(l1, s_l1);
        if (threadIdx.x == 0) atomicAdd(sum_slot(light_l1_sum), tot);
    }
    if (block_absmax == nullptr) return;
#pragma unroll
    for (int o = 32; o > 0; o >>= 1) m = fmaxf(m, __shfl_xor(m, o, 64));
    if (__ballot(bad) != 0ull) m = __uint_as_float(0x7f800000u);
    if ((threadIdx.x & 63) == 0) s_m[threadIdx.x >> 6] = m;
    __syncthreads();
    if (threadIdx.x == 0) block_absmax[blockIdx.x] = fmaxf(fmaxf(s_m[0], s_m[1]), fmaxf(s_m[2], s_m[3]));
}

struct EnvBackward {
    int He, We;
    const float* raw;
    const float* env;
    float* dL_denv;
    float w_tv;
    float* g_raw;
    float* tv_sum;
    int consume;
};

__device__ __forceinline__ void env_backward_block(int block, const EnvBackward& a)
{
    __shared__ float s_part[4];
    const int He = a.He, We = a.We;
    const int n = He * We * 3;
    const int i = block * 256 + threadIdx.x;
    float tv = 0.f;
    if (i < n) {
        const int w = (i / 3) % We, h = i / (3 * We);
        const float inv_v = He > 1 ? 1.f / (3.f * (He - 1) * We) : 0.f, inv_h = We > 1 ? 1.f / (3.f * He * (We - 1)) : 0.f;
        const float x = a.env[i];
        float g = 0.f;
        if (h > 0) g += inv_v * 2.f * (x - a.env[i - 3 * We]);
        if (h < He - 1) { const float d = a.env[i + 3 * We] - x; g -= inv_v * 2.f * d; tv += inv_v * d * d; }
        if (w > 0) g += inv_h * 2.f * (x - a.env[i - 3]);
        if (w < We - 1) { const float d = a.env[i + 3] - x; g -= inv_h * 2.f * d; tv += inv_h * d * d; }
        const float r = a.raw[i];
        const float dsoft = r > 20.f ? 1.f : sigmoidf_(r);
        a.g_raw[i] = (a.dL_denv[i] + a.w_tv * g) * dsoft;
        if (a.consume) a.dL_denv[i] = 0.f;
    }
    const float tot = block_sum_256(tv, s_part);
    if (threadIdx.x == 0 && a.tv_sum != nullptr) atomicAdd(sum_slot(a.tv_sum), tot);
}

__global__ void __launch_bounds__(256)
s2_env_backward_kernel(EnvBackward a)
{
    env_backward_block((int)blockIdx.x, a);
}

__global__ void __launch_bounds__(256)
s2_activate_backward_kernel(int P, const float* __restrict__ xyz, const float* __restrict__ scaling_raw,
                            const float* __restrict__ rotation_raw, const float* __restrict__ opacity_raw,
                            const float* __restrict__ normal_raw, const float* __restrict__ base_raw,
                            const float* __restrict__ rough_raw, const float* __restrict__ viewmatrix,
                            const float* __restrict__ campos, const float* __restrict__ dL_dfeatures,
                            const float* __restrict__ dL_dbase_shade, const float* __restrict__ dL_drough_shade,
                            const float* __restrict__ dL_dviewdirs, const float* __restrict__ dL_dscales,
                            const float* __restrict__ dL_drot, const float* __restrict__ dL_dopacity,
                            const float* __restrict__ dL_dmeans3D, float* __restrict__ g_xyz,
                            float* __restrict__ g_scaling, float* __restrict__ g_rotation,
                            float* __restrict__ g_opacity, float* __restrict__ g_normal, float* __restrict__ g_base,
                            float* __restrict__ g_rough, int nb_main, EnvBackward env_job)
{
    if ((int)blockIdx.x >= nb_main) {
        env_backward_block((int)blockIdx.x - nb_main, env_job);
        return;
    }
    const int i = blockIdx.x * 256 + threadIdx.x;
    if (i >= P) return;
    const size_t i3 = 3 * (size_t)i, i4 = 4 * (size_t)i;
    const float4* gf = reinterpret_cast<const float4*>(dL_dfeatures + 16 * (size_t)i);
    const float4 f0 = gf[0], f1 = gf[1], f2 = gf[2];
    {
        const float gfeat[3] = {f2.x, f2.y, f2.z};
#pragma unroll
        for (int c = 0; c < 3; c++) {
            const float s = sigmoidf_(base_raw[i3 + c]);
            g_base[i3 + c] = (gfeat[c] + dL_dbase_shade[i3 + c]) * 0.77f * s * (1.f - s);
        }
        const float s = sigmoidf_(rough_raw[i]);
        g_rough[i] = (f2.w + dL_drough_shade[i]) * 0.9f * s * (1.f - s);
    }
    if (g_xyz == nullptr) return;

#pragma unroll
    for (int c = 0; c < 3; c++) g_scaling[i3 + c] = dL_dscales[i3 + c] * __expf(scaling_raw[i3 + c]);
    {
        const float q[4] = {rotation_raw[i4], rotation_raw[i4 + 1], rotation_raw[i4 + 2], rotation_raw[i4 + 3]};
        const float g[4] = {dL_drot[i4], dL_drot[i4 + 1], dL_drot[i4 + 2], dL_drot[i4 + 3]};
        const float n = sqrtf(q[0] * q[0] + q[1] * q[1] + q[2] * q[2] + q[3] * q[3]);
        if (n > 1e-12f) {
            const float inv = 1.f / n;
            const float u[4] = {q[0] / n, q[1] / n, q[2] / n, q[3] / n};
            const float d = u[0] * g[0] + u[1] * g[1] + u[2] * g[2] + u[3] * g[3];
#pragma unroll
            for (int c = 0; c < 4; c++) g_rotation[i4 + c] = (g[c] - u[c] * d) * inv;
        } else {
#pragma unroll
            for (int c = 0; c < 4; c++) g_rotation[i4 + c] = g[c] * 1e12f;
        }
    }
    {
        const float s = sigmoidf_(opacity_raw[i]);
        g_opacity[i] = dL_dopacity[i] * s * (1.f - s);
    }
    {
        const float v[3] = {normal_raw[i3], normal_raw[i3 + 1], normal_raw[i3 + 2]};
        const float g[3] = {f1.y, f1.z, f1.w};
        float o[3];
        normalize3_backward(v, 1e-3f, g, o);
        g_normal[i3] = o[0]; g_normal[i3 + 1] = o[1]; g_normal[i3 + 2] = o[2];
    }
    {
        const float p[3] = {xyz[i3], xyz[i3 + 1], xyz[i3 + 2]};
        const float depth = p[0] * viewmatrix[2] + p[1] * viewmatrix[6] + p[2] * viewmatrix[10] + viewmatrix[14];
        const float gd = f0.x + 2.f * depth * f0.y;
        const float d[3] = {campos[0] - p[0], campos[1] - p[1], campos[2] - p[2]};
        const float gv[3] = {dL_dviewdirs[i3], dL_dviewdirs[i3 + 1], dL_dviewdirs[i3 + 2]};
        float gdd[3];
        normalize3_backward(d, 1e-12f, gv, gdd);
        g_xyz[i3] = dL_dmeans3D[i3] + gd * viewmatrix[2] - gdd[0];
        g_xyz[i3 + 1] = dL_dmeans3D[i3 + 1] + gd * viewmatrix[6] - gdd[1];
        g_xyz[i3 + 2] = dL_dmeans3D[i3 + 2] + gd * viewmatrix[10] - gdd[2];
    }
}

__global__ void __launch_bounds__(256)
s2_pbr_srgb_kernel(int HW, const float* __restrict__ opacity, const float* __restrict__ feature,
                   const int* __restrict__ n_contrib, const float* __restrict__ bg, float* __restrict__ srgb)
{
    const int i = blockIdx.x * 256 + threadIdx.x;
    if (i >= HW) return;
    const float op = opacity[i];
    const float scale = n_contrib[i] > 0 ? 1.f / fmaxf(op, 1e-5f) : 0.f;
#pragma unroll
    for (int c = 0; c < 3; c++) {
        const float x = feature[(size_t)(2 + c) * HW + i] * scale * op + (1.f - op) * bg[c];
        const float v = x <= 0.0031308f ? 12.92f * x : 1.055f * srgb_pow(fmaxf(x, 0.0031308f), 1.f / 2.4f) - 0.055f;
        srgb[(size_t)c * HW + i] = fminf(fmaxf(v, 0.f), 1.f);
    }
}

__global__ void __launch_bounds__(256)
s2_normals_srgb_kernel(int W, int H, float focal_x, float focal_y, float cx, float cy, const float* __restrict__ vm,
                       const float* __restrict__ opacity, const float* __restrict__ depths, float* __restrict__ normals,
                       float* __restrict__ surface_xyz, const float* __restrict__ feature, const int* __restrict__ n_contrib,
                       const float* __restrict__ bg, float* __restrict__ srgb)
{
    const int x = blockIdx.x * 64 + (threadIdx.x & 63), y = blockIdx.y * 4 + (threadIdx.x >> 6);
    if (x >= W || y >= H) return;
    const int HW = W * H, i = y * W + x;
    {
        const float op = opacity[i];
        const float scale = n_contrib[i] > 0 ? 1.f / fmaxf(op, 1e-5f) : 0.f;
#pragma unroll
        for (int c = 0; c < 3; c++) {
            const float v0 = feature[(size_t)(2 + c) * HW + i] * scale * op + (1.f - op) * bg[c];
            const float v = v0 <= 0.0031308f ? 12.92f * v0 : 1.055f * srgb_pow(fmaxf(v0, 0.0031308f), 1.f / 2.4f) - 0.055f;
            srgb[(size_t)c * HW + i] = fminf(fmaxf(v, 0.f), 1.f);
        }
    }
    pseudo_normal_pixel(x, y, W, H, focal_x, focal_y, cx, cy, vm, opacity, depths, normals, surface_xyz);
}

template <bool SPARSE>
__global__ void __launch_bounds__(256)
s2_loss_kernel(int HW, const float* __restrict__ image, const float* __restrict__ opacity,
               const float* __restrict__ feature, const float* __restrict__ pseudo_normal,
               const int* __restrict__ n_contrib, const float* __restrict__ gt, const float* __restrict__ bg,
               const float* __restrict__ image_mask, float w_l1, float w_pbr, float w_normal,
               const float* __restrict__ extra_dimage,
               const float* __restrict__ extra_dsrgb, float* __restrict__ dL_dimage,
               float* __restrict__ dL_dopacity, float* __restrict__ dL_dfeature, float* __restrict__ sums)
{
    __shared__ float s_part[4];
    float s_l1 = 0.f, s_pbr = 0.f, s_n = 0.f;
    for (int i = blockIdx.x * 256 + threadIdx.x; i < HW; i += gridDim.x * 256) {
        const float op = opacity[i];
        const int nc = n_contrib[i];
        float v_gt[3], v_im[3], v_ei[3], v_F[3], v_es[3], v_Fn[3], v_pn[3];
        const bool normal_on = !SPARSE || w_normal != 0.f;
#pragma unroll
        for (int c = 0; c < 3; c++) {
            v_gt[c] = gt[(size_t)c * HW + i];
            v_im[c] = image[(size_t)c * HW + i];
            v_F[c] = feature[(size_t)(2 + c) * HW + i];
        }
#pragma unroll
        for (int c = 0; c < 3; c++) {
            v_ei[c] = extra_dimage ? extra_dimage[(size_t)c * HW + i] : 0.f;
            v_es[c] = extra_dsrgb ? extra_dsrgb[(size_t)c * HW + i] : 0.f;
        }
        float mk = 1.f;
        if (normal_on) {
            mk = image_mask ? image_mask[i] : 1.f;
#pragma unroll
            for (int c = 0; c < 3; c++) {
                v_Fn[c] = feature[(size_t)(5 + c) * HW + i];
                v_pn[c] = pseudo_normal[(size_t)c * HW + i];
            }
        }
        const bool mask = nc > 0;
        const float opc = fmaxf(op, 1e-5f);
        const float scale = mask ? 1.f / opc : 0.f;
        const float dscale_dop = (mask && op >= 1e-5f) ? -1.f / (opc * opc) : 0.f;
        float g_op = 0.f;
#pragma unroll
        for (int c = 0; c < 3; c++) {
            const float g = v_gt[c];
            const float d0 = v_im[c] - g;
            s_l1 += fabsf(d0);
            dL_dimage[(size_t)c * HW + i] = w_l1 * signf_(d0) + v_ei[c];
            const float F = v_F[c];
            const float r = F * scale;
            const float x = r * op + (1.f - op) * bg[c];
            const bool lin = x <= 0.0031308f;
            const float xs = fmaxf(x, 0.0031308f);
            const float curve = lin ? 12.92f * x : 1.055f * srgb_pow(xs, 1.f / 2.4f) - 0.055f;
            const bool unclipped = curve >= 0.f && curve <= 1.f;
            const float srgb = fminf(fmaxf(curve, 0.f), 1.f);
            const float d1 = srgb - g;
            s_pbr += fabsf(d1);
            const float dsrgb = !unclipped ? 0.f : (lin ? 12.92f : 1.055f / 2.4f * srgb_pow(xs, 1.f / 2.4f - 1.f));
            const float gx = (w_pbr * signf_(d1) + v_es[c]) * dsrgb;
            dL_dfeature[(size_t)(2 + c) * HW + i] = gx * op * scale;
            g_op += gx * (r - bg[c] + op * F * dscale_dop);
            if (normal_on) {
                const float Fn = v_Fn[c];
                const float dn = (Fn * scale - v_pn[c]) * mk;
                s_n += dn * dn;
                const float gn = 2.f * w_normal * dn * mk;
                dL_dfeature[(size_t)(5 + c) * HW + i] = gn * scale;
                g_op += gn * Fn * dscale_dop;
            }
        }
        dL_dopacity[i] = g_op;
        if (!SPARSE) {
            dL_dfeature[i] = 0.f;
            dL_dfeature[(size_t)HW + i] = 0.f;
#pragma unroll
            for (int c = 8; c < 16; c++) dL_dfeature[(size_t)c * HW + i] = 0.f;
        }
    }
    const float t0 = block_sum_256(s_l1, s_part);
    __syncthreads();
    const float t1 = block_sum_256(s_pbr, s_part);
    __syncthreads();
    const float t2 = block_sum_256(s_n, s_part);
    if (threadIdx.x == 0) {
        atomicAdd(sum_slot(sums + 0 * R3DG_SUM_SLOTS), t0);
        atomicAdd(sum_slot(sums + 1 * R3DG_SUM_SLOTS), t1);
        atomicAdd(sum_slot(sums + 2 * R3DG_SUM_SLOTS), t2);
    }
}

void launch_s2_activate(hipStream_t s, int P, const float* xyz, const float* scaling_raw, const float* rotation_raw,
                        const float* opacity_raw, const float* normal_raw, const float* base_raw,
                        const float* rough_raw, const float* campos, float* scales, float* rot, float* opacity,
                        float* normal, float* base_color, float* roughness, float* viewdirs, const float* viewmatrix,
                        float* features, int n_env, const float* env_raw, float* env, float* zero, int n_zero)
{
    ActivateSide side;
    side.nb_main = (P + 255) / 256;
    side.n_env = env_raw != nullptr && env != nullptr ? n_env : 0;
    side.env_raw = env_raw;
    side.env = env;
    side.zero = zero;
    side.n_zero = zero != nullptr ? n_zero : 0;
    const int work = side.n_env > side.n_zero ? side.n_env : side.n_zero;
    const int nb_side = work > 0 ? (work + 255) / 256 < 8 ? (work + 255) / 256 : 8 : 0;
    s2_activate_kernel<<<side.nb_main + nb_side, 256, 0, s>>>(P, xyz, scaling_raw, rotation_raw, opacity_raw, normal_raw,
                                                              base_raw, rough_raw, campos, scales, rot, opacity, normal,
                                                              base_color, roughness, viewdirs, viewmatrix, features, side);
    check_launch(s, false, "s2_activate_kernel");
}

void launch_s2_pack(hipStream_t s, int P, const float* xyz, const float* viewmatrix, const float* normal,
                    const float* base_color, const float* roughness, const float* shade_out, float* features,
                    float* light_l1_sum)
{
    s2_pack_features_kernel<<<(P + 255) / 256, 256, 0, s>>>(P, xyz, viewmatrix, normal, base_color, roughness,
                                                            shade_out, features, light_l1_sum);
    check_launch(s, false, "s2_pack_features_kernel");
}

void launch_s2_unpack(hipStream_t s, int P, const float* dL_dfeatures, const float* shade_out, float light_weight,
                      float* dL_dpbr, float* dL_ddiffuse, float* block_absmax, float* light_l1_sum)
{
    s2_unpack_kernel<<<(P + 255) / 256, 256, 0, s>>>(P, dL_dfeatures, shade_out, light_weight, dL_dpbr, dL_ddiffuse,
                                                    block_absmax, light_l1_sum);
    check_launch(s, false, "s2_unpack_kernel");
}

void launch_s2_activate_backward(hipStream_t s, int P, const float* xyz, const float* scaling_raw,
                                 const float* rotation_raw, const float* opacity_raw, const float* normal_raw,
                                 const float* base_raw, const float* rough_raw, const float* viewmatrix,
                                 const float* campos, const float* dL_dfeatures, const float* dL_dbase_shade,
                                 const float* dL_drough_shade, const float* dL_dviewdirs, const float* dL_dscales,
                                 const float* dL_drot, const float* dL_dopacity, const float* dL_dmeans3D, float* g_xyz,
                                 float* g_scaling, float* g_rotation, float* g_opacity, float* g_normal, float* g_base,
                                 float* g_rough, int He, int We, const float* env_raw, const float* env, float* dL_denv,
                                 float w_tv, float* g_env_raw, float* tv_sum, int consume)
{
    EnvBackward job;
    job.He = He; job.We = We; job.raw = env_raw; job.env = env; job.dL_denv = dL_denv; job.w_tv = w_tv; job.g_raw = g_env_raw;
    job.tv_sum = tv_sum; job.consume = consume;
    const int nb_main = (P + 255) / 256;
    const int nb_env = env_raw != nullptr ? (He * We * 3 + 255) / 256 : 0;
    s2_activate_backward_kernel<<<nb_main + nb_env, 256, 0, s>>>(
        P, xyz, scaling_raw, rotation_raw, opacity_raw, normal_raw, base_raw, rough_raw, viewmatrix, campos,
        dL_dfeatures, dL_dbase_shade, dL_drough_shade, dL_dviewdirs, dL_dscales, dL_drot, dL_dopacity, dL_dmeans3D, g_xyz,
        g_scaling, g_rotation, g_opacity, g_normal, g_base, g_rough, nb_main, job);
    check_launch(s, false, "s2_activate_backward_kernel");
}

void launch_s2_normals_srgb(hipStream_t s, int W, int H, const float* vm, float focal_x, float focal_y, float cx, float cy,
                            const float* opacity, const float* depths, float* normals, float* surface_xyz, const float* feature,
                            const int* n_contrib, const float* bg, float* srgb)
{
    dim3 grid((W + 63) / 64, (H + 3) / 4);
    s2_normals_srgb_kernel<<<grid, 256, 0, s>>>(W, H, focal_x, focal_y, cx, cy, vm, opacity, depths, normals, surface_xyz,
                                                feature, n_contrib, bg, srgb);
    check_launch(s, false, "s2_normals_srgb_kernel");
}

void launch_s2_pbr_srgb(hipStream_t s, int HW, const float* opacity, const float* feature, const int* n_contrib,
                        const float* bg, float* srgb)
{
    s2_pbr_srgb_kernel<<<(HW + 255) / 256, 256, 0, s>>>(HW, opacity, feature, n_contrib, bg, srgb);
    check_launch(s, false, "s2_pbr_srgb_kernel");
}

constexpr int LOSS_BLOCKS = 768;

void launch_s2_loss(hipStream_t s, int HW, const float* image, const float* opacity, const float* feature,
                    const float* pseudo_normal, const int* n_contrib, const float* gt, const float* bg,
                    const float* image_mask, float w_l1, float w_pbr, float w_normal, const float* extra_dimage,
                    const float* extra_dsrgb, float* dL_dimage, float* dL_dopacity, float* dL_dfeature, float* sums,
                    int sparse)
{
    if (sparse)
        s2_loss_kernel<true><<<min((HW + 255) / 256, LOSS_BLOCKS), 256, 0, s>>>(
            HW, image, opacity, feature, pseudo_normal, n_contrib, gt, bg, image_mask, w_l1, w_pbr, w_normal, extra_dimage,
            extra_dsrgb, dL_dimage, dL_dopacity, dL_dfeature, sums);
    else
        s2_loss_kernel<false><<<min((HW + 255) / 256, LOSS_BLOCKS), 256, 0, s>>>(
            HW, image, opacity, feature, pseudo_normal, n_contrib, gt, bg, image_mask, w_l1, w_pbr, w_normal, extra_dimage,
            extra_dsrgb, dL_dimage, dL_dopacity, dL_dfeature, sums);
    check_launch(s, false, "s2_loss_kernel");
}

void launch_s2_env_backward(hipStream_t s, int He, int We, const float* raw, const float* env, float* dL_denv,
                            float w_tv, float* g_raw, float* tv_sum, int consume)
{
    EnvBackward job;
    job.He = He; job.We = We; job.raw = raw; job.env = env; job.dL_denv = dL_denv; job.w_tv = w_tv; job.g_raw = g_raw;
    job.tv_sum = tv_sum; job.consume = consume;
    s2_env_backward_kernel<<<(He * We * 3 + 255) / 256, 256, 0, s>>>(job);
    check_launch(s, false, "s2_env_backward_kernel");
}

}
```

### relightable3dgaussian_amd/fused_adam.py

```python
import ctypes as C

import torch

from . import _abi, _lib

AdamGroup = _abi.structs["r3dg_adam_group"]


class FusedAdam:
    MAX_GROUPS = _abi.constants["R3DG_ADAM_MAX_GROUPS"]

    def __init__(self, groups, betas=(0.9, 0.999), eps=1e-15):
        if len(groups) > self.MAX_GROUPS:
            raise RuntimeError("FusedAdam supports at most %d groups" % self.MAX_GROUPS)
        self.groups = groups
        self.betas, self.eps = betas, eps
        self.step_count = 0
        for g in groups:
            p = g["param"]
            if not p.is_contiguous() or p.dtype != torch.float32:
                raise RuntimeError("FusedAdam needs contiguous float32 parameters")
            if g.get("lr_tail") is None:
                g["lr_tail"] = g["lr"]
            g["exp_avg"] = torch.zeros_like(p)
            g["exp_avg_sq"] = torch.zeros_like(p)

    def step(self, grads, grad_scale=1.0, skip_flag=None):
        self.begin_step()
        self.step_groups(range(len(self.groups)), grads, grad_scale, skip_flag)

    def begin_step(self):
        self.step_count += 1

    def fused_step_of(self, i, step, grad_scale=1.0, skip_flag=None):
        g = self.groups[i]
        p = g["param"]
        self._fused_desc = AdamGroup(p.data_ptr(), None, g["exp_avg"].data_ptr(), g["exp_avg_sq"].data_ptr(), p.numel(),
                                     g["lr"], g["lr_tail"], g.get("period", 0), g.get("split", 0))
        return (C.addressof(self._fused_desc), self.betas[0], self.betas[1], self.eps, int(step), float(grad_scale),
                skip_flag.data_ptr() if skip_flag is not None else None)

    def step_groups(self, indices, grads, grad_scale=1.0, skip_flag=None):
        L = _lib.lib()
        indices = list(indices)
        table = (AdamGroup * len(indices))()
        for j, i in enumerate(indices):
            g, gr = self.groups[i], grads[i]
            p = g["param"]
            if gr.shape != p.shape or not gr.is_contiguous() or gr.dtype != torch.float32:
                raise RuntimeError("FusedAdam: gradient %d does not match its parameter" % i)
            table[j] = AdamGroup(p.data_ptr(), gr.data_ptr(), g["exp_avg"].data_ptr(), g["exp_avg_sq"].data_ptr(),
                                 p.numel(), g["lr"], g["lr_tail"], g.get("period", 0), g.get("split", 0))
        with torch.cuda.device(self.groups[0]["param"].device):
            st = L.r3dg_adam_step(_lib.current_stream(), len(indices), C.cast(table, C.c_void_p), self.betas[0],
                                  self.betas[1], self.eps, self.step_count, float(grad_scale),
                                  skip_flag.data_ptr() if skip_flag is not None else None)
        _lib.check(st, "adam_step")
```

### relightable3dgaussian_amd/fused_step.py

```python
import collections
import contextlib
import os

import torch
import torch.nn.functional as F

from . import _lib, rasterizer_ops, shading_ops
from .fused_adam import AdamGroup, FusedAdam
from .fused_base import _STREAMS, SUM_SLOTS, FusedStepBase, _in_context, _world_of, grad_slab, learning_rates, shared_stream
from .fused_samples import SampleSet, of_samples
from .fused_stage1 import FusedStage1Step
from .grad_comm import BucketComm
from .shading_ops import LEAVE_ROOM, TRAIN_OUTPUTS
from .train_step import FROZEN_GEOMETRY_GROUPS, LAMBDA_DSSIM, STAGE2_WEIGHTS, update_visibility, update_visibility_device

PARAM_NAMES = ("xyz", "normal", "scaling", "rotation", "opacity", "shs", "base_color", "roughness", "incidents", "env")

_View = collections.namedtuple("_View", "cam bg gt mask H W N vm campos main raw order_stream gt_depth mvs_normal")


class FusedStage2Step(FusedStepBase):

    _chain_kernel = True
    _opt_order = PARAM_NAMES

    def __init__(self, params, sample_num, lr=1e-4, lr_rest_scale=1.0, loss_weights=None, process_group=None, lrs=None,
                 bounded=True, device_visibility=False):
        unknown = set(loss_weights or ()) - set(STAGE2_WEIGHTS)
        if unknown:
            raise RuntimeError("FusedStage2Step: unknown loss weights %s" % sorted(unknown))
        dev = params.xyz.device
        super().__init__(params, [k for k in PARAM_NAMES if k not in ("shs", "incidents")], process_group,
                         *_world_of(process_group), bounded, order_stream=shared_stream(dev, "order"))
        P, self.K = self.P, sample_num
        self._incidents = torch.cat([params.incidents_dc.detach(), params.incidents_rest.detach()], 1).contiguous()
        if self._incidents.shape[1] != self.M:
            raise RuntimeError("FusedStage2Step: colour and incident-light SH must hold the same number of coefficients")
        for k in ("visibility_dc", "visibility_rest"):
            t = getattr(params, k, None)
            setattr(self, k, None if t is None else t.detach().clone().contiguous())
        self.w = dict(STAGE2_WEIGHTS, **(loss_weights or {}))
        rate, tail = learning_rates(lr, lrs, lr_rest_scale)
        self.frozen = {k for k in PARAM_NAMES if rate(k) == 0.0 and (k not in ("shs", "incidents") or tail(k) == 0.0)}
        self.frozen_geometry = all(k in self.frozen for k in FROZEN_GEOMETRY_GROUPS)
        f = dict(dtype=torch.float32, device=dev)
        self.a_scales, self.a_rot = torch.empty(P, 3, **f), torch.empty(P, 4, **f)
        self.a_opacity, self.a_normal = torch.empty(P, 1, **f), torch.empty(P, 3, **f)
        self.a_base, self.a_rough = torch.empty(P, 3, **f), torch.empty(P, 1, **f)
        self.a_viewdirs = torch.empty(P, 3, **f)
        self.shade_out = torch.empty(P, shading_ops.NOUT, **f)
        self.features = torch.empty(P, 16, **f)
        self._supervised = self.w["depth"] != 0.0 or self.w["normal_mvs_depth"] != 0.0
        self.sums = torch.zeros(12 if self._supervised else 10, SUM_SLOTS, **f)
        self._sup_counts = {}
        self._sup_count_cur = None
        self.d_pbr, self.d_diffuse = torch.empty(P, 3, **f), torch.empty(P, 3, **f)
        self._absmax = torch.zeros((P + 255) // 256, **f)
        geo = ("xyz", "normal", "scaling", "rotation", "opacity")
        if self.frozen_geometry:
            order = ("flag", "base_color", "roughness", "env", "incidents", "shs") + geo
        else:
            order = ("shs", "flag") + geo + ("base_color", "roughness", "env", "incidents")
        raw = {k: self._incidents if k == "incidents" else getattr(self, k) for k in PARAM_NAMES}
        self.grad_flat, self.grads, start = grad_slab(order, raw, dev)
        self._flag = self.grads.pop("flag")
        self._skip_cur = None
        flat, s_inc = self.grad_flat, start["incidents"]
        if self.frozen_geometry:
            self._bucket_a, self._bucket_c, self._bucket_b = None, flat[:s_inc], flat[s_inc:start["shs"]]
            self._bucket_all = flat[:start["shs"]]
        else:
            self._bucket_a, self._bucket_c, self._bucket_b = flat[:start["xyz"]], flat[start["xyz"]:s_inc], flat[s_inc:]
            self._bucket_all = flat
        self._comm = BucketComm(dev, process_group, self.world, self.dp)
        self.exposed_comm_ms, self.comm_table = self._comm.exposed_comm_ms, self._comm.comm_table
        self._handles = self._pending_b = None
        self._acc = torch.empty((11 + 16) * P, **f)
        self._early_pending = False
        self._early = self._b_early = self._a_late = False
        self._dp_chain = None
        self._env_c = self._d_env = None
        self._adam_stream = self._geo_done = None
        self._direct_rows = os.environ.get("R3DG_DIRECT_ROWS", "1") != "0"
        if self.dp:
            self._ctx.set("RESERVE_CUS", int(os.environ.get("R3DG_RESERVE_CUS_FOR_COMM", "8")))
            if int(os.environ.get("GPU_MAX_HW_QUEUES", "4")) < 8:
                import warnings
                warnings.warn("FusedStage2Step under data parallelism: GPU_MAX_HW_QUEUES=%s (< 8) -- RCCL's streams and this "
                              "iteration's three streams will share hardware queues and serialise; export GPU_MAX_HW_QUEUES=8 "
                              "before the process starts (bench.py does)" % os.environ.get("GPU_MAX_HW_QUEUES", "unset (4)"))
        self.serial_streams = False
        self.last_active_features = None
        self._single_bucket = self.dp and os.environ.get("R3DG_DP_BUCKETS", "3") == "1"
        self._samples = SampleSet(sample_num, self.M, (update_visibility, update_visibility_device), process_group, device_visibility)
        with torch.no_grad(), self._ctx:
            self.refresh_activations()
            self._samples.acquire(self.xyz, self.a_scales, self.a_rot, self.a_opacity, self.a_normal)
        self._pre_rotated = None
        self._chain_deferred = None
        two_rates = lambda k: dict(lr_tail=tail(k), period=3 * self.M, split=3) if k in ("shs", "incidents") else {}
        self.opt = FusedAdam([dict(param=raw[k], lr=rate(k), **two_rates(k)) for k in self._opt_order])
        live = lambda idx: tuple(i for i in idx if self._opt_order[i] not in self.frozen)
        self._groups_a, self._groups_c, self._groups_b = live((5,)), live((0, 1, 2, 3, 4, 6, 7, 9)), live((8,))

    visibility, incident_dirs, incident_areas, tracer, device_visibility = map(of_samples, (
        "visibility", "incident_dirs", "incident_areas", "tracer", "device_visibility"))
    visibility_refreshes, _ray_normals, _frs, _taps, _taps_src, _uniform_area = map(of_samples, (
        "refreshes", "ray_normals", "frs", "taps", "src", "uniform_area"))

    incidents_dc = property(lambda self: self.incidents[:, :1])
    incidents_rest = property(lambda self: self.incidents[:, 1:])

    @property
    def incidents(self):
        if self._early_pending:
            self.flush()
        return self._incidents

    @incidents.setter
    def incidents(self, value):
        if self._early_pending:
            self.flush()
        self._incidents = value
        self._pre_rotated = None

    measure_comm = property(lambda self: self._comm.measure_comm, lambda self, v: setattr(self._comm, "measure_comm", v))
    comm_probe_every = property(lambda self: self._comm.comm_probe_every,
                                lambda self, v: setattr(self._comm, "comm_probe_every", v))

    get_scaling = lambda self: torch.exp(self.scaling)
    get_rotation = lambda self: F.normalize(self.rotation)
    get_opacity = lambda self: torch.sigmoid(self.opacity)
    get_shs = lambda self: self.shs
    get_normal = lambda self: F.normalize(self.normal, dim=-1, eps=1e-3)

    def refresh_activations(self, cam=None, env_out=None, zero=None):
        L = _lib.lib()
        campos = cam.camera_center if cam is not None else torch.zeros(3, device=self.dev)
        with torch.cuda.device(self.dev):
            st = L.r3dg_stage2_activate_with(
                _lib.current_stream(), self.P, self.xyz.data_ptr(), self.scaling.data_ptr(), self.rotation.data_ptr(),
                self.opacity.data_ptr(), self.normal.data_ptr(), self.base_color.data_ptr(), self.roughness.data_ptr(),
                campos.contiguous().data_ptr(), self.a_scales.data_ptr(), self.a_rot.data_ptr(),
                self.a_opacity.data_ptr(), self.a_normal.data_ptr(), self.a_base.data_ptr(), self.a_rough.data_ptr(),
                self.a_viewdirs.data_ptr(),
                cam.world_view_transform.contiguous().data_ptr() if cam is not None and self._direct_rows else None,
                self.features.data_ptr() if cam is not None and self._direct_rows else None,
                0 if env_out is None else env_out.numel(), None if env_out is None else self.env.data_ptr(),
                None if env_out is None else env_out.data_ptr(), None if zero is None else zero.data_ptr(),
                0 if zero is None else zero.numel())
        _lib.check(st, "stage2_activate")

    @_in_context
    def refresh_visibility(self):
        self.flush()
        self.refresh_activations()
        self._samples.refresh(self.xyz, self.a_scales, self.a_rot, self.a_opacity, self.a_normal)
        self._pre_rotated = None

    def taps(self, He, We):
        return self._samples.select(He, We)

    def _rotation_is_current(self):
        pr = self._pre_rotated
        return pr is not None and pr[0] is self._samples.frs and pr[1] is self._incidents and pr[2] == self._incidents._version

    def _early_stream(self):
        if self._adam_stream is None:
            self._adam_stream = shared_stream(self.dev, "early")
        return self._adam_stream

    def _aux_stream(self):
        if self._samples.frs is None or self.dp or self.serial_streams:
            return None
        return self._early_stream()

    def _listed_stream(self):
        frs = self._samples.frs
        if frs is None or frs.n_invalid == 0 or self.serial_streams:
            return None
        return self._early_stream()

    @_in_context
    def forward_backward(self, cam, bg, gt, early_adam=False, image_mask=None, split_geometry=None, chain_incidents=False,
                         gt_depth=None, mvs_normal=None, sh_adam_in_backward=False):
        H, W = cam.image_height, cam.image_width
        if self._supervised and (gt_depth is None or (self.w["normal_mvs_depth"] != 0.0 and mvs_normal is None)):
            raise RuntimeError("FusedStage2Step: the depth / normal_mvs_depth terms need gt_depth%s" % (
                "" if self.w["normal_mvs_depth"] == 0.0 else " and mvs_normal"))
        main = torch.cuda.current_stream(self.dev)
        v = _View(cam, bg, gt, image_mask, H, W, H * W, cam.world_view_transform.contiguous(), cam.camera_center.contiguous(),
                  main, main.cuda_stream, None if self.serial_streams else self._order_stream, gt_depth, mvs_normal)
        with torch.cuda.device(self.dev):
            pending, env_c, flag_cur, use_bounded, rotated_for = self._front_end(v)
            taps, packed = self._shade_forward(v, env_c, rotated_for)
            fw = pending.finish(v.order_stream)
            self._skip_cur = flag_cur
            g, active = self._image_loss(v, fw)
            fused_a = sh_adam_in_backward and self._fuses_sh_adam()
            dL_dfeatures, bw, geo_stream, handle_a = self._raster_backward(
                v, fw, g, active, early_adam if split_geometry is None else split_geometry, fused_a)
            b_early = self._schedule_early(v, handle_a, geo_stream, use_bounded, early_adam, chain_incidents, fused_a)
            self._shade_backward(v, env_c, taps, packed, dL_dfeatures, bw, geo_stream, b_early, chain_incidents)
            self._remaining_buckets(handle_a)
        return self._end_forward_backward(fw, None if bw is None else bw[0], use_bounded, v.N)

    def _front_end(self, v):
        rotated_for = None
        aux = self._aux_stream()
        if self._chain_deferred is not None:
            self.flush()
        if aux is not None:
            _lib.stream_wait(aux, v.main)
            rotated_for = self._samples.frs
            if not self._rotation_is_current():
                with torch.cuda.stream(aux):
                    rotated_for.rotate(self._incidents)
        if self._env_c is None or self._env_c.shape != self.env.shape[1:]:
            self._env_c = torch.empty(tuple(self.env.shape[1:]), dtype=torch.float32, device=self.dev)
        env_c = self._env_c
        self.refresh_activations(v.cam, env_out=env_c, zero=self.sums)
        self._iter += 1
        flag_cur = self._flag_of_iteration()
        use_bounded = self._use_bounded(v.W, v.H)
        if self._early_pending and (aux is None or not (use_bounded and v.order_stream is not None)):
            _lib.stream_wait(v.main, self._adam_stream)
            self._early_pending = False
        if use_bounded:
            bounded = dict(capacity=self._capacity, overflow_flag=flag_cur, overflow_count=self._overflow_count,
                           ordering_stream=v.order_stream)
        else:
            flag_cur.zero_()
            bounded = {}
        cam, empty = v.cam, torch.Tensor([])
        pending = rasterizer_ops.rasterize_gaussians_begin(
            v.bg, self.xyz, self.features, empty, self.a_opacity, self.a_scales, self.a_rot, 1.0, empty, v.vm,
            cam.full_proj_transform, cam.tanfovx, cam.tanfovy, cam.cx, cam.cy, v.H, v.W, self.shs, 3, v.campos, False,
            True, False, want_weights=False,
            defer_pseudo_normal=True, **bounded)
        if self._pending_b is not None:
            self.flush()
        if aux is not None:
            _lib.stream_wait(v.main, aux)
            self._early_pending = False
        return pending, env_c, flag_cur, use_bounded, rotated_for

    def _shade_forward(self, v, env_c, rotated_for):
        L = _lib.lib()
        He, We = env_c.shape[0], env_c.shape[1]
        sm = self._samples
        taps = sm.select(He, We)
        frs, area = sm.frs, sm.uniform_area
        if frs is not None:
            rotated = rotated_for is frs or (self.dp and self._rotation_is_current())
            frs.forward(self.a_base, self.a_rough, self.a_normal, self.a_viewdirs, self._incidents, env_c,
                        sm.visibility, self.shade_out, uniform_area=area,
                        leave_room=v.order_stream is not None and not self.dp,
                        listed_stream=self._listed_stream(), rotated=rotated,
                        feature_rows=self.features if self._direct_rows else None)
        else:
            _lib.check(L.r3dg_shade_forward_cached(
                v.raw, self.P, self.K, self.M, self.a_base.data_ptr(), self.a_rough.data_ptr(), self.a_normal.data_ptr(),
                self.a_viewdirs.data_ptr(), self._incidents.data_ptr(), env_c.data_ptr(), He, We, None,
                sm.visibility.data_ptr(), sm.incident_dirs.data_ptr(),
                None if area is not None else sm.incident_areas.data_ptr(), area or 0.0,
                taps.data_ptr(), TRAIN_OUTPUTS | (LEAVE_ROOM if v.order_stream is not None else 0),
                self.shade_out.data_ptr()), "shade_forward")
        if frs is not None and self._listed_stream() is not None:
            _lib.stream_wait(v.main, self._listed_stream())
        packed = not (frs is not None and self._direct_rows)
        if packed:
            _lib.check(L.r3dg_stage2_pack_features(v.raw, self.P, self.xyz.data_ptr(), v.vm.data_ptr(), self.a_normal.data_ptr(),
                self.a_base.data_ptr(), self.a_rough.data_ptr(), self.shade_out.data_ptr(), self.features.data_ptr(),
                self.sums[3].data_ptr()), "stage2_pack_features")
        return taps, packed

    def _image_loss(self, v, fw):
        L = _lib.lib()
        cam, W, H, N = v.cam, v.W, v.H, v.N
        _R, n_contrib, image, opacity, depth, feature, pseudo_normal, sxyz = fw[:8]
        g = torch.empty((47, H, W), dtype=torch.float32, device=self.dev)
        gt_c, bg_c = v.gt.contiguous(), v.bg.contiguous()
        srgb, part_i, part_p, gs_i, gs_p = g[20:23], g[23:32], g[32:41], g[41:44], g[44:47]
        lam = LAMBDA_DSSIM
        _lib.check(L.r3dg_stage2_normals_srgb(v.raw, W, H, v.vm.data_ptr(), float(cam.tanfovx), float(cam.tanfovy), float(cam.cx),
            float(cam.cy), opacity.data_ptr(), depth.data_ptr(), pseudo_normal.data_ptr(), sxyz.data_ptr(), feature.data_ptr(),
            n_contrib.data_ptr(), bg_c.data_ptr(), srgb.data_ptr()), "stage2_normals_srgb")
        _lib.check(L.r3dg_ssim_forward_pair(v.raw, W, H, 3, image.data_ptr(), srgb.data_ptr(), gt_c.data_ptr(), part_i.data_ptr(),
                                            part_p.data_ptr(), self.sums[5].data_ptr(), self.sums[6].data_ptr()), "ssim_forward")
        _lib.check(L.r3dg_ssim_backward_pair(v.raw, W, H, 3, image.data_ptr(), srgb.data_ptr(), gt_c.data_ptr(),
                                             part_i.data_ptr(), part_p.data_ptr(), -self.w["l1"] * lam / (3.0 * N),
                                             -self.w["pbr"] * lam / (3.0 * N), gs_i.data_ptr(), gs_p.data_ptr()),
                   "ssim_backward")
        mask_c = None if v.mask is None else v.mask.contiguous()
        _lib.check(L.r3dg_stage2_loss(v.raw, W, H, image.data_ptr(), opacity.data_ptr(), feature.data_ptr(),
            pseudo_normal.data_ptr(), n_contrib.data_ptr(), gt_c.data_ptr(), bg_c.data_ptr(), _lib.ptr(mask_c),
            self.w["l1"] * (1.0 - lam) / (3.0 * N), self.w["pbr"] * (1.0 - lam) / (3.0 * N), self.w["normal"] / (3.0 * N),
            gs_i.data_ptr(), gs_p.data_ptr(), g[0:3].data_ptr(), g[3:4].data_ptr(), g[4:20].data_ptr(), self.sums.data_ptr(), 1),
            "stage2_loss")
        active = [2, 3, 4] + ([5, 6, 7] if self.w["normal"] != 0.0 else [])
        w_bc, w_r, w_ls = (self.w[k] / (3.0 * N) for k in ("base_color_smooth", "roughness_smooth", "light_smooth"))
        if w_bc != 0.0 or w_r != 0.0 or w_ls != 0.0:
            _lib.check(L.r3dg_stage2_smooth_fused(v.raw, W, H, opacity.data_ptr(), feature.data_ptr(), n_contrib.data_ptr(),
                gt_c.data_ptr(), _lib.ptr(mask_c), w_bc, w_r, w_ls, 1 if self.w["normal"] != 0.0 else 0, g[3:4].data_ptr(),
                g[4:20].data_ptr(), self.sums[7].data_ptr()), "stage2_smooth_fused")
            active += ([8, 9, 10] if w_bc != 0.0 else []) + ([11] if w_r != 0.0 else [])
            if w_ls != 0.0:
                active += [12, 13, 14] + ([5, 6, 7] if self.w["normal"] == 0.0 else [])
        if self._supervised:
            w_d, w_nm = self.w["depth"], self.w["normal_mvs_depth"] / (3.0 * N)
            depth_c = v.gt_depth.contiguous()
            mvs_c = None if w_nm == 0.0 else v.mvs_normal.contiguous()
            self._sup_count_cur = self._supervision_count(v, depth_c, mask_c) if w_d != 0.0 else None
            _lib.check(L.r3dg_stage2_supervision(v.raw, W, H, opacity.data_ptr(), feature.data_ptr(), n_contrib.data_ptr(),
                depth_c.data_ptr(), _lib.ptr(mvs_c), _lib.ptr(mask_c), _lib.ptr(self._sup_count_cur), w_d, w_nm,
                1 if 5 in active else 0, g[3:4].data_ptr(), g[4:20].data_ptr(), self.sums[10].data_ptr()), "stage2_supervision")
            active += ([0] if w_d != 0.0 else []) + ([5, 6, 7] if w_nm != 0.0 and 5 not in active else [])
        self.last_active_features = sorted(set(active))
        return g, active

    def _supervision_count(self, v, depth_c, mask_c):
        key = id(v.gt_depth)
        hit = self._sup_counts.get(key)
        mv = None if v.mask is None else v.mask._version
        if hit is not None and hit[0] is v.gt_depth and hit[1] is v.mask and hit[2] == (v.gt_depth._version, mv):
            return hit[3]
        count = torch.empty(1, dtype=torch.int32, device=self.dev)
        _lib.check(_lib.lib().r3dg_supervision_count(v.raw, v.W, v.H, depth_c.data_ptr(), _lib.ptr(mask_c), count.data_ptr()),
                   "supervision_count")
        self._sup_counts[key] = (v.gt_depth, v.mask, (v.gt_depth._version, mv), count)
        return count

    def _fuses_sh_adam(self):
        can = getattr(rasterizer_ops.rasterize_gaussians_backward, "sh_adam_supported", None)
        return (not self.dp and bool(self._groups_a) and not self.frozen_geometry and can is not None
                and os.environ.get("R3DG_SH_ADAM_IN_BACKWARD", "1") != "0" and can(self.M))

    def _raster_backward(self, v, fw, g, active, split_geometry, fused_a=False):
        cam, empty = v.cam, torch.Tensor([])
        R, radii, geom, binning, img = fw[0], fw[9], fw[10], fw[11], fw[12]
        geo_stream = None
        if self.frozen_geometry:
            active = [a for a in active if a not in (0, 5, 6, 7)]
            dL_dfeatures = rasterizer_ops.rasterize_gaussians_backward_features(
                self.P, 16, v.H, v.W, g[4:20], geom, R, binning, img, active_features=sorted(active))
            bw = None
        else:
            geo_stream = self._listed_stream() if split_geometry else None
            fused = dict(sh_adam=self.opt.fused_step_of(self._groups_a[0], self.opt.step_count + 1, 1.0, self._skip_cur)) \
                if fused_a else {}
            bw = rasterizer_ops.rasterize_gaussians_backward(
                v.bg, self.xyz, self.features, radii, empty, self.a_scales, self.a_rot, 1.0, empty, v.vm,
                cam.full_proj_transform, cam.tanfovx, cam.tanfovy, g[0:3], g[3:4], empty, g[4:20],
                self.shs, 3, v.campos, geom, R, binning, img, True, False, dL_dsh_out=self.grads["shs"],
                geometry_stream=geo_stream, active_features=sorted(active), zeroed_accumulators=self._acc, **fused)
            dL_dfeatures = bw[4]
            if geo_stream is not None:
                if self._geo_done is None:
                    self._geo_done = torch.cuda.Event()
                self._geo_done.record(geo_stream)
        handle_a = None
        if self._bucket_a is not None and not self._single_bucket:
            with torch.cuda.stream(geo_stream) if geo_stream is not None else contextlib.nullcontext():
                handle_a = self._comm.allreduce_async(self._bucket_a, "A", self._iter)
        return dL_dfeatures, bw, geo_stream, handle_a

    def _schedule_early(self, v, handle_a, geo_stream, use_bounded, early_adam, chain_incidents, fused_a=False):
        a_launch = early_adam and bool(self._groups_a) and (handle_a is not None or not self.dp)
        b_early = (not self.dp and self._samples.frs is not None and v.order_stream is not None and use_bounded and
                   (a_launch or (bool(self._groups_b) and (self.P * self.K <= 40_000_000 if early_adam else chain_incidents))))
        a_early = a_launch or fused_a
        self._early, self._b_early, self._a_late = a_early or b_early, b_early, b_early and not a_early
        if self._early:
            side = self._early_stream()
            self.opt.begin_step()
            self._early_pending = not self.dp
        if fused_a:
            if b_early:
                _lib.stream_wait(v.order_stream, geo_stream if geo_stream is not None else v.main)
        elif a_early:
            if geo_stream is None and not self.dp:
                side.wait_stream(v.main)
            with torch.cuda.stream(side):
                if self.dp:
                    self._comm.wait(handle_a, "A", self._iter, side)
                    self._skip_cur = self._snapshot_flag()
                self.opt.step_groups(self._groups_a, [self.grads[k] for k in self._opt_order], 1.0 / self.world,
                                     skip_flag=self._skip_cur)
            if b_early:
                _lib.stream_wait(v.order_stream, side)
        return b_early

    def _shade_backward(self, v, env_c, taps, packed, dL_dfeatures, bw, geo_stream, b_early, chain_incidents):
        L = _lib.lib()
        P, gr = self.P, self.grads
        _lib.check(L.r3dg_stage2_unpack_gradients(
            v.raw, P, dL_dfeatures.data_ptr(), self.shade_out.data_ptr(), self.w["light"] / (3.0 * P),
            self.d_pbr.data_ptr(), self.d_diffuse.data_ptr(), self._absmax.data_ptr(),
            None if packed else self.sums[3].data_ptr()), "stage2_unpack_gradients")
        if self._d_env is None or self._d_env.shape != env_c.shape:
            self._d_env = torch.zeros_like(env_c)
        sm = self._samples
        frs = sm.frs
        if frs is not None:
            chain = b_early and bool(self._groups_b)
            dp_chain = (self.dp and chain_incidents and bool(self._groups_b) and not self._single_bucket
                        and os.environ.get("R3DG_DP_CHAIN", "1") != "0")
            d_base, d_rough, d_view, _d_inc, d_env = frs.backward(
                self.a_base, self.a_rough, self.a_normal, self.a_viewdirs, self._incidents, env_c, sm.visibility,
                self.d_pbr, self.d_diffuse, uniform_area=sm.uniform_area,
                out_incidents=frs.dcprime_rows() if dp_chain else gr["incidents"], out_env=self._d_env,
                block_absmax=self._absmax,
                rotate_stream=self._adam_stream if self._early else None, rotation_back=not (chain or dp_chain))
            self._dp_chain = frs if dp_chain else None
            if b_early:
                self._chain_deferred = (frs, self._skip_cur, self.opt.step_count)
        else:
            d_base, d_rough, d_view, _d_inc, d_env = shading_ops.shade_backward(self.a_base, self.a_rough, self.a_normal,
                self.a_viewdirs, self._incidents, env_c, sm.visibility, sm.incident_dirs, sm.incident_areas, self.d_pbr,
                self.d_diffuse, out_incidents=gr["incidents"], taps=taps, out_env=self._d_env, block_absmax=self._absmax)
        if geo_stream is not None:
            v.main.wait_event(self._geo_done)
        env_job = (env_c.shape[0], env_c.shape[1], self.env.data_ptr(), env_c.data_ptr(), d_env.data_ptr(),
                   self.w["env_smooth"], gr["env"].data_ptr(), self.sums[4].data_ptr(), 1)
        geo = (lambda t: None) if self.frozen_geometry else (lambda t: t.data_ptr())
        _means2D, _dcol, dL_dopacity, dL_dmeans3D, _dfeat, _dcov, _dsh, dL_dscales, dL_drot = bw or (None,) * 9
        _lib.check(L.r3dg_stage2_activate_backward_with(v.raw, P, geo(self.xyz), geo(self.scaling), geo(self.rotation),
            geo(self.opacity), geo(self.normal), self.base_color.data_ptr(), self.roughness.data_ptr(), geo(v.vm), geo(v.campos),
            dL_dfeatures.data_ptr(), d_base.data_ptr(), d_rough.data_ptr(), geo(d_view), geo(dL_dscales), geo(dL_drot),
            geo(dL_dopacity), geo(dL_dmeans3D), geo(gr["xyz"]), geo(gr["scaling"]), geo(gr["rotation"]), geo(gr["opacity"]),
            geo(gr["normal"]), gr["base_color"].data_ptr(), gr["roughness"].data_ptr(), *env_job), "stage2_activate_backward")

    def _remaining_buckets(self, handle_a):
        comm, it = self._comm, self._iter
        self._handles = None
        if self._single_bucket:
            self._handles = (None, comm.allreduce_async(self._bucket_all, "ALL", it), None)
        elif self.dp:
            handle_c = comm.allreduce_async(self._bucket_c, "C", it)
            if self._dp_chain is not None:
                handle_b = comm.allreduce_async(self._dp_chain.dcprime.view(-1), "B", it)
            else:
                with torch.cuda.stream(self._adam_stream) if self._early else contextlib.nullcontext():
                    handle_b = comm.allreduce_async(self._bucket_b, "B", it)
            self._handles = (handle_a, handle_c, handle_b)

    def loss(self):
        self.poll_overflow()
        N, P = self._N, self.P
        lam = LAMBDA_DSSIM
        w = torch.tensor([self.w["l1"] * (1 - lam) / (3.0 * N), self.w["pbr"] * (1 - lam) / (3.0 * N),
                          self.w["normal"] / (3.0 * N), self.w["light"] / (3.0 * P), self.w["env_smooth"],
                          -self.w["l1"] * lam / (3.0 * N), -self.w["pbr"] * lam / (3.0 * N),
                          self.w["base_color_smooth"] / (3.0 * N), self.w["roughness_smooth"] / (3.0 * N),
                          self.w["light_smooth"] / (3.0 * N)], device=self.dev)
        if self._supervised:
            count = 0 if self._sup_count_cur is None else int(self._sup_count_cur.item())
            w = torch.cat([w, torch.tensor([self.w["depth"] / count if count else 0.0, self.w["normal_mvs_depth"] / (3.0 * N)],
                                           device=self.dev)])
        return (self.sums.sum(1) * w).sum() + lam * (self.w["l1"] + self.w["pbr"])

    @_in_context
    def optimizer_step(self):
        grads = [self.grads[k] for k in self._opt_order]
        if not self.dp:
            if self._b_early:
                todo = (self._groups_a if self._a_late else ()) + self._groups_c
            elif self._early:
                _lib.stream_wait(torch.cuda.current_stream(), self._adam_stream)
                self._early_pending = False
                todo = self._groups_c + self._groups_b
            else:
                self.opt.begin_step()
                todo = self._groups_a + self._groups_c + self._groups_b
            self._early = self._b_early = self._a_late = False
            if todo:
                self.opt.step_groups(todo, grads, skip_flag=self._skip_cur)
                if set(todo) & set(self._groups_b):
                    self._pre_rotated = None
            if self._chain_deferred is not None:
                self._run_chain()
            return
        scale, wait, it = 1.0 / self.world, self._comm.wait, self._iter
        handle_a, handle_c, handle_b = self._handles
        if self._single_bucket:
            self.opt.begin_step()
            wait(handle_c, "ALL", it)
            self._skip_cur = self._snapshot_flag()
            todo = self._groups_a + self._groups_c + self._groups_b
            if todo:
                self.opt.step_groups(todo, grads, scale, skip_flag=self._skip_cur)
                self._pre_rotated = None
            return
        if self._early:
            torch.cuda.current_stream().wait_stream(self._adam_stream)
            self._early = False
            wait(handle_c, "C", it)
        else:
            self.opt.begin_step()
            wait(handle_a if handle_a is not None else handle_c, "A" if handle_a is not None else "C", it)
            self._skip_cur = self._snapshot_flag()
            if handle_a is not None:
                if self._groups_a:
                    self.opt.step_groups(self._groups_a, grads, scale, skip_flag=self._skip_cur)
                wait(handle_c, "C", it)
        if self._groups_c:
            self.opt.step_groups(self._groups_c, grads, scale, skip_flag=self._skip_cur)
        self._pending_b = (handle_b, grads, scale, self._skip_cur, it)

    def _incident_chain(self, frs, count, scale, skip, **listed):
        grp = self.opt.groups[self._groups_b[0]]
        frs.incident_chain(self._incidents, self.grads["incidents"], grp["exp_avg"], grp["exp_avg_sq"], grp["lr"],
                           grp["lr_tail"], self.opt.betas, self.opt.eps, count, scale, skip_flag=skip, **listed)
        self._pre_rotated = (frs, self._incidents, self._incidents._version)

    def _run_chain(self):
        frs, skip, count = self._chain_deferred
        self._chain_deferred = None
        early = self._adam_stream
        _lib.stream_wait(early, torch.cuda.current_stream(self.dev))
        with torch.cuda.stream(early):
            if self._groups_b:
                lean = (getattr(frs, "chain_gradient_optional", False)
                        and os.environ.get("R3DG_CHAIN_WRITES_GRADIENT", "0") == "0")
                self._incident_chain(frs, count, 1.0, skip, **(dict(write_gradient=False) if lean else {}))
            else:
                frs.rotate(self._incidents)
                self._pre_rotated = (frs, self._incidents, self._incidents._version)

    @_in_context
    def flush(self):
        if self._chain_deferred is not None:
            self._run_chain()
        if self._early_pending:
            _lib.stream_wait(torch.cuda.current_stream(self.dev), self._adam_stream)
            self._early_pending = False
        if self._pending_b is not None:
            handle_b, grads, scale, skip, it_b = self._pending_b
            self._pending_b = None
            self._comm.wait(handle_b, "B", it_b)
            frs, self._dp_chain = self._dp_chain, None
            if frs is not None:
                self._incident_chain(frs, self.opt.step_count, scale, skip, listed_in_dcprime=True)
            elif self._groups_b:
                self.opt.step_groups(self._groups_b, grads, scale, skip_flag=skip)
                self._pre_rotated = None

    @_in_context
    def __call__(self, cam, bg, gt, image_mask=None, gt_depth=None, mvs_normal=None):
        early = os.environ.get("R3DG_EARLY_ADAM", "1" if self.P <= 1_000_000 else "0") != "0" and not self.serial_streams
        outs = self.forward_backward(cam, bg, gt, early_adam=early, image_mask=image_mask, chain_incidents=True,
                                     gt_depth=gt_depth, mvs_normal=mvs_normal, sh_adam_in_backward=True)
        self.optimizer_step()
        return outs
```

Baseline: 835.0 iters/s.

## Fuse Adam update for geometry/material/env groups into activate-backward kernel

The stage-2 activation chain-rule kernel now also applies the Adam update to the xyz, scaling, rotation, opacity, normal, base color, roughness and env parameters right after it computes their gradients. Gradients are staged in LDS and written out with vectorized stores. The optimizer step then skips the groups already closed. This removes a separate Adam launch and a second read of the gradient arrays, at the cost of more register and LDS use in the fused kernel and more complex step-count bookkeeping.

```diff
diff --git a/include/r3dg_hip.h b/include/r3dg_hip.h
--- a/include/r3dg_hip.h
+++ b/include/r3dg_hip.h
@@ -351,6 +351,20 @@
                                           const r3dg_adam_group* sh_adam, float beta1, float beta2, float eps, int step,
                                           float grad_scale, const float* d_skip_flag);
 
+int r3dg_stage2_activate_backward_adam_supported(void);
+int r3dg_stage2_activate_backward_adam(void* stream, int P, const float* d_xyz, const float* d_scaling_raw,
+                                       const float* d_rotation_raw, const float* d_opacity_raw, const float* d_normal_raw,
+                                       const float* d_base_raw, const float* d_rough_raw, const float* d_viewmatrix,
+                                       const float* d_campos, const float* d_dL_dfeatures, const float* d_dL_dbase_color,
+                                       const float* d_dL_droughness, const float* d_dL_dviewdirs, const float* d_dL_dscales,
+                                       const float* d_dL_drot, const float* d_dL_dopacity, const float* d_dL_dmeans3D,
+                                       float* d_g_xyz, float* d_g_scaling, float* d_g_rotation, float* d_g_opacity,
+                                       float* d_g_normal, float* d_g_base, float* d_g_rough, int He, int We,
+                                       const float* d_env_raw, const float* d_env, float* d_dL_denv, float w_tv,
+                                       float* d_g_env_raw, float* d_tv_sum, int consume, const r3dg_adam_group** groups,
+                                       float beta1, float beta2, float eps, int step, float grad_scale,
+                                       const float* d_skip_flag);
+
 int r3dg_relight_pack_features(void* stream, int P, const float* d_xyz, const float* d_viewmatrix, const float* d_normal,
                                const float* d_base_color, const float* d_roughness, const float* d_shade_out,
                                float* d_features);
diff --git a/relightable3dgaussian_amd/_abi.py b/relightable3dgaussian_amd/_abi.py
--- a/relightable3dgaussian_amd/_abi.py
+++ b/relightable3dgaussian_amd/_abi.py
@@ -81,7 +81,7 @@
             known = base in _SCALARS or (base == "void" and stars > 0)
             if stars == 0 and (known or base == "r3dg_alloc_fn"):
                 args.append(ALLOC_FN if base == "r3dg_alloc_fn" else _SCALARS[base])
-            elif stars == 2 and known:
+            elif stars == 2 and (known or base in structs):
                 args.append(C.POINTER(C.c_void_p))
             elif stars == 1 and (base == "void" or base in structs or (known and name.startswith("d_"))):
                 args.append(C.c_void_p)
diff --git a/relightable3dgaussian_amd/csrc/capi_stage.hip b/relightable3dgaussian_amd/csrc/capi_stage.hip
--- a/relightable3dgaussian_amd/csrc/capi_stage.hip
+++ b/relightable3dgaussian_amd/csrc/capi_stage.hip
@@ -1,3 +1,4 @@
+#include "adam_update.hpp"
 #include "capi_internal.hpp"
 
 using namespace r3dg;
@@ -95,22 +96,36 @@
                                               0.f, nullptr, nullptr, 0);
 }
 
-int r3dg_stage2_activate_backward_with(void* stream_, int P, const float* xyz, const float* scaling_raw,
-                                  const float* rotation_raw, const float* opacity_raw, const float* normal_raw,
-                                  const float* base_raw, const float* rough_raw, const float* viewmatrix,
-                                  const float* campos, const float* dL_dfeatures, const float* dL_dbase_shade,
-                                  const float* dL_drough_shade, const float* dL_dviewdirs, const float* dL_dscales,
-                                  const float* dL_drot, const float* dL_dopacity, const float* dL_dmeans3D, float* g_xyz,
-                                  float* g_scaling, float* g_rotation, float* g_opacity, float* g_normal, float* g_base,
-                                  float* g_rough, int He, int We,
-                                       const float* env_raw, const float* env, float* dL_denv, float w_tv,
-                                       float* g_env_raw, float* tv_sum, int consume)
+#define R3DG_ACTIVATE_BACKWARD_PARAMS                                                                                              \
+    void* stream_, int P, const float* xyz, const float* scaling_raw, const float* rotation_raw, const float* opacity_raw,         \
+    const float* normal_raw, const float* base_raw, const float* rough_raw, const float* viewmatrix, const float* campos,          \
+    const float* dL_dfeatures, const float* dL_dbase_shade, const float* dL_drough_shade, const float* dL_dviewdirs,               \
+    const float* dL_dscales, const float* dL_drot, const float* dL_dopacity, const float* dL_dmeans3D, float* g_xyz,               \
+    float* g_scaling, float* g_rotation, float* g_opacity, float* g_normal, float* g_base, float* g_rough, int He, int We,         \
+    const float* env_raw, const float* env, float* dL_denv, float w_tv, float* g_env_raw, float* tv_sum, int consume
+#define R3DG_ACTIVATE_BACKWARD_ARGS                                                                                                \
+    stream_, P, xyz, scaling_raw, rotation_raw, opacity_raw, normal_raw, base_raw, rough_raw, viewmatrix, campos, dL_dfeatures,   \
+    dL_dbase_shade, dL_drough_shade, dL_dviewdirs, dL_dscales, dL_drot, dL_dopacity, dL_dmeans3D, g_xyz, g_scaling, g_rotation,    \
+    g_opacity, g_normal, g_base, g_rough, He, We, env_raw, env, dL_denv, w_tv, g_env_raw, tv_sum, consume
+
+static int activate_backward_impl(R3DG_ACTIVATE_BACKWARD_PARAMS, const CloseAdam* adam)
 {
     if (P < 0) return invalid("stage2_activate_backward: bad P");
     if (He < 0 || We < 0) return invalid("stage2_activate_backward: bad texture size");
     const bool env_job = He * We != 0;
     if (env_job && (!env_raw || !env || !dL_denv || !g_env_raw)) return invalid("stage2_activate_backward: null texture buffer");
-    if (P == 0) return env_job ? r3dg_stage2_env_backward(stream_, He, We, env_raw, env, dL_denv, w_tv, g_env_raw, tv_sum, consume) : R3DG_OK;
+    if (P == 0 && adam == nullptr)
+        return env_job ? r3dg_stage2_env_backward(stream_, He, We, env_raw, env, dL_denv, w_tv, g_env_raw, tv_sum, consume) : R3DG_OK;
+    if (P == 0) {
+        if (!env_job) return R3DG_OK;
+        return guarded([&]() -> int {
+            launch_s2_activate_backward((hipStream_t)stream_, 0, nullptr, nullptr, nullptr, nullptr, nullptr, nullptr, nullptr,
+                                        nullptr, nullptr, nullptr, nullptr, nullptr, nullptr, nullptr, nullptr, nullptr, nullptr,
+                                        nullptr, nullptr, nullptr, nullptr, nullptr, nullptr, nullptr, He, We, env_raw, env,
+                                        dL_denv, w_tv, g_env_raw, tv_sum, consume, adam);
+            return R3DG_OK;
+        });
+    }
     if (!base_raw || !rough_raw || !dL_dfeatures || !dL_dbase_shade || !dL_drough_shade || !g_base || !g_rough)
         return invalid("stage2_activate_backward: null buffer");
     if (g_xyz != nullptr &&
@@ -123,10 +138,51 @@
                                     base_raw, rough_raw, viewmatrix, campos, dL_dfeatures, dL_dbase_shade,
                                     dL_drough_shade, dL_dviewdirs, dL_dscales, dL_drot, dL_dopacity, dL_dmeans3D, g_xyz,
                                     g_scaling, g_rotation, g_opacity, g_normal, g_base, g_rough, env_job ? He : 0, env_job ? We : 0,
-                                    env_job ? env_raw : nullptr, env, dL_denv, w_tv, g_env_raw, tv_sum, consume);
-        return R3DG_OK;
-    });
-}
+                                    env_job ? env_raw : nullptr, env, dL_denv, w_tv, g_env_raw, tv_sum, consume, adam);
+        return R3DG_OK;
+    });
+}
+
+int r3dg_stage2_activate_backward_with(R3DG_ACTIVATE_BACKWARD_PARAMS)
+{
+    return activate_backward_impl(R3DG_ACTIVATE_BACKWARD_ARGS, nullptr);
+}
+
+int r3dg_stage2_activate_backward_adam_supported(void) { return 1; }
+
+int r3dg_stage2_activate_backward_adam(R3DG_ACTIVATE_BACKWARD_PARAMS, const r3dg_adam_group** groups, float beta1, float beta2,
+                                       float eps, int step, float grad_scale, const float* skip_flag)
+{
+    const char* me = "stage2_activate_backward_adam: ";
+    if (P < 0 || He < 0 || We < 0) return invalid(std::string(me) + "bad P / texture size");
+    if (!groups) return invalid(std::string(me) + "null group table");
+    if (step < 1) return invalid(std::string(me) + "step counts from 1");
+    if (P > 0 && !g_xyz) return invalid(std::string(me) + "frozen geometry (d_g_xyz == NULL) keeps the separate Adam launch");
+    const float* const raw[CLOSE_GROUPS] = {xyz, scaling_raw, rotation_raw, opacity_raw, normal_raw, base_raw, rough_raw, env_raw};
+    const float* const grad[CLOSE_GROUPS] = {g_xyz, g_scaling, g_rotation, g_opacity, g_normal, g_base, g_rough, nullptr};
+    const uint64_t width[CLOSE_GROUPS - 1] = {3, 3, 4, 1, 3, 3, 1};
+    const AdamBias b = adam_bias(beta1, beta2, step);
+    CloseAdam adam = {};
+    adam.beta1 = beta1; adam.beta2 = beta2; adam.eps = eps; adam.bias1 = b.bias1; adam.inv_sqrt_bias2 = b.inv_sqrt_bias2;
+    adam.grad_scale = grad_scale; adam.skip_flag = skip_flag;
+    for (int a = 0; a < CLOSE_GROUPS; a++) {
+        if (a < CLOSE_GROUPS - 1 && ((uintptr_t)grad[a] & 15)) return invalid(std::string(me) + "unaligned gradient array");
+        if (!groups[a]) continue;
+        const r3dg_adam_group& g = *groups[a];
+        const uint64_t n = a < CLOSE_GROUPS - 1 ? width[a] * (uint64_t)P : (uint64_t)He * (uint64_t)We * 3;
+        if (g.n != n || n >= (1ull << 32)) return invalid(std::string(me) + "a group's n is not the size of its array (below 2^32)");
+        if (n == 0) continue;
+        if (g.param != raw[a]) return invalid(std::string(me) + "a group's param must be the raw array the call reads");
+        if (!g.param || !g.exp_avg || !g.exp_avg_sq) return invalid(std::string(me) + "null buffer in group");
+        if (((uintptr_t)g.param | (uintptr_t)g.exp_avg | (uintptr_t)g.exp_avg_sq) & 15)
+            return invalid(std::string(me) + "unaligned buffer in group");
+        adam.g[a] = g;
+        adam.any = 1;
+    }
+    return activate_backward_impl(R3DG_ACTIVATE_BACKWARD_ARGS, &adam);
+}
+#undef R3DG_ACTIVATE_BACKWARD_PARAMS
+#undef R3DG_ACTIVATE_BACKWARD_ARGS
 
 int r3dg_stage2_loss(void* stream_, int width, int height, const float* image, const float* opacity,
                      const float* feature, const float* pseudo_normal, const int32_t* n_contrib, const float* gt,
diff --git a/relightable3dgaussian_amd/csrc/launchers.hpp b/relightable3dgaussian_amd/csrc/launchers.hpp
--- a/relightable3dgaussian_amd/csrc/launchers.hpp
+++ b/relightable3dgaussian_amd/csrc/launchers.hpp
@@ -141,6 +141,13 @@
                     float* light_l1_sum);
 void launch_s2_unpack(hipStream_t s, int P, const float* dL_dfeatures, const float* shade_out, float light_weight,
                       float* dL_dpbr, float* dL_ddiffuse, float* block_absmax, float* light_l1_sum);
+constexpr int CLOSE_GROUPS = 8;
+struct CloseAdam {
+    r3dg_adam_group g[CLOSE_GROUPS];
+    float beta1, beta2, eps, bias1, inv_sqrt_bias2, grad_scale;
+    const float* skip_flag;
+    int any;
+};
 void launch_s2_activate_backward(hipStream_t s, int P, const float* xyz, const float* scaling_raw, const float* rotation_raw,
                                  const float* opacity_raw, const float* normal_raw, const float* base_raw,
                                  const float* rough_raw, const float* viewmatrix, const float* campos,
@@ -149,7 +156,7 @@
                                  const float* dL_dopacity, const float* dL_dmeans3D, float* g_xyz, float* g_scaling,
                                  float* g_rotation, float* g_opacity, float* g_normal, float* g_base, float* g_rough, int He,
                                  int We, const float* env_raw, const float* env, float* dL_denv, float w_tv,
-                                 float* g_env_raw, float* tv_sum, int consume);
+                                 float* g_env_raw, float* tv_sum, int consume, const CloseAdam* adam);
 void launch_s2_loss(hipStream_t s, int HW, const float* image, const float* opacity, const float* feature,
                     const float* pseudo_normal, const int* n_contrib, const float* gt, const float* bg,
                     const float* image_mask, float w_l1, float w_pbr, float w_normal, const float* extra_dimage,
diff --git a/relightable3dgaussian_amd/csrc/stage2_glue.hip b/relightable3dgaussian_amd/csrc/stage2_glue.hip
--- a/relightable3dgaussian_amd/csrc/stage2_glue.hip
+++ b/relightable3dgaussian_amd/csrc/stage2_glue.hip
@@ -1,4 +1,5 @@
 #include "launchers.hpp"
+#include "adam_update.hpp"
 #include "glue_math.hpp"
 #include "pseudo_normal.hpp"
 #include "r3dg_hip.h"
@@ -156,7 +157,7 @@
     int consume;
 };
 
-__device__ __forceinline__ void env_backward_block(int block, const EnvBackward& a)
+__device__ __forceinline__ void env_backward_block(int block, const EnvBackward& a, const CloseAdam& ad, bool update)
 {
     __shared__ float s_part[4];
     const int He = a.He, We = a.We;
@@ -174,8 +175,16 @@
         if (w < We - 1) { const float d = a.env[i + 3] - x; g -= inv_h * 2.f * d; tv += inv_h * d * d; }
         const float r = a.raw[i];
         const float dsoft = r > 20.f ? 1.f : sigmoidf_(r);
-        a.g_raw[i] = (a.dL_denv[i] + a.w_tv * g) * dsoft;
+        const float g_raw = (a.dL_denv[i] + a.w_tv * g) * dsoft;
+        a.g_raw[i] = g_raw;
         if (a.consume) a.dL_denv[i] = 0.f;
+        const r3dg_adam_group& grp = ad.g[CLOSE_GROUPS - 1];
+        if (update && grp.exp_avg != nullptr) {
+            float p = r, m = grp.exp_avg[i], v = grp.exp_avg_sq[i];
+            adam_update(p, g_raw, m, v, adam_rate((unsigned int)i, grp.lr, grp.lr_tail, grp.period, grp.split), ad.beta1, ad.beta2,
+                        ad.eps, ad.bias1, ad.inv_sqrt_bias2, ad.grad_scale);
+            const_cast<float*>(a.raw)[i] = p; grp.exp_avg[i] = m; grp.exp_avg_sq[i] = v;
+        }
     }
     const float tot = block_sum_256(tv, s_part);
     if (threadIdx.x == 0 && a.tv_sum != nullptr) atomicAdd(sum_slot(a.tv_sum), tot);
@@ -184,7 +193,71 @@
 __global__ void __launch_bounds__(256)
 s2_env_backward_kernel(EnvBackward a)
 {
-    env_backward_block((int)blockIdx.x, a);
+    env_backward_block((int)blockIdx.x, a, CloseAdam{}, false);
+}
+
+constexpr int CLOSE_SEG_XYZ = 0, CLOSE_SEG_SCALING = 768, CLOSE_SEG_ROTATION = 1536, CLOSE_SEG_OPACITY = 2560,
+              CLOSE_SEG_NORMAL = 2816, CLOSE_SEG_BASE = 3584, CLOSE_SEG_ROUGH = 4352, CLOSE_LDS_FLOATS = 4608;
+
+template <int C>
+__device__ __forceinline__ void close_write(float* __restrict__ g_out, const float* seg, int rows, bool vec)
+{
+    const int t = threadIdx.x, n = rows * C, nq = n >> 2;
+    float* __restrict__ g = g_out + (size_t)blockIdx.x * 256 * C;
+    if (!vec) {
+        for (int k = t; k < n; k += 256) g[k] = seg[k];
+    } else if (t < nq) {
+        *reinterpret_cast<float4*>(g + 4 * t) = *reinterpret_cast<const float4*>(seg + 4 * t);
+    } else if (t - nq < (n & 3)) {
+        g[4 * nq + (t - nq)] = seg[4 * nq + (t - nq)];
+    }
+}
+
+struct CloseRegs {
+    float p[4], m[4], v[4];
+};
+
+template <int C>
+__device__ __forceinline__ void close_load(const float* param, int rows, const r3dg_adam_group& grp, const float* spare,
+                                           CloseRegs& r)
+{
+    const int t = threadIdx.x;
+    const bool mine = grp.exp_avg != nullptr && t < (rows * C) >> 2;
+    const size_t at = (size_t)blockIdx.x * 256 * C + 4 * t;
+    *reinterpret_cast<float4*>(r.p) = *reinterpret_cast<const float4*>(mine ? param + at : spare);
+    *reinterpret_cast<float4*>(r.m) = adam_load(mine ? grp.exp_avg + at : spare, true);
+    *reinterpret_cast<float4*>(r.v) = adam_load(mine ? grp.exp_avg_sq + at : spare, true);
+}
+
+template <int C>
+__device__ __forceinline__ void close_finish(const float* param, const float* seg, int rows, const CloseAdam& ad,
+                                             const r3dg_adam_group& grp, CloseRegs& r)
+{
+    if (grp.exp_avg == nullptr) return;
+    const int t = threadIdx.x, n = rows * C, nq = n >> 2;
+    const size_t run = (size_t)blockIdx.x * 256 * C;
+    float* p = const_cast<float*>(param) + run;
+    float* __restrict__ m = grp.exp_avg + run;
+    float* __restrict__ v = grp.exp_avg_sq + run;
+    if (t < nq) {
+        const int at = 4 * t;
+        const float4 gq = *reinterpret_cast<const float4*>(seg + at);
+        const float gv[4] = {gq.x, gq.y, gq.z, gq.w};
+#pragma unroll
+        for (int k = 0; k < 4; k++) {
+            const float lr = adam_rate((unsigned int)(run + at + k), grp.lr, grp.lr_tail, grp.period, grp.split);
+            adam_update(r.p[k], gv[k], r.m[k], r.v[k], lr, ad.beta1, ad.beta2, ad.eps, ad.bias1, ad.inv_sqrt_bias2, ad.grad_scale);
+        }
+        *reinterpret_cast<float4*>(p + at) = *reinterpret_cast<float4*>(r.p);
+        adam_store(m + at, r.m, true);
+        adam_store(v + at, r.v, true);
+    } else if (t - nq < (n & 3)) {
+        const int e = 4 * nq + (t - nq);
+        float pe = p[e], me = m[e], ve = v[e];
+        const float lr = adam_rate((unsigned int)(run + e), grp.lr, grp.lr_tail, grp.period, grp.split);
+        adam_update(pe, seg[e], me, ve, lr, ad.beta1, ad.beta2, ad.eps, ad.bias1, ad.inv_sqrt_bias2, ad.grad_scale);
+        p[e] = pe; m[e] = me; v[e] = ve;
+    }
 }
 
 __global__ void __launch_bounds__(256)
@@ -199,69 +272,106 @@
                             const float* __restrict__ dL_dmeans3D, float* __restrict__ g_xyz,
                             float* __restrict__ g_scaling, float* __restrict__ g_rotation,
                             float* __restrict__ g_opacity, float* __restrict__ g_normal, float* __restrict__ g_base,
-                            float* __restrict__ g_rough, int nb_main, EnvBackward env_job)
-{
+                            float* __restrict__ g_rough, int nb_main, EnvBackward env_job, int vec, CloseAdam ad)
+{
+    const bool update = ad.any != 0 && !(ad.skip_flag != nullptr && *ad.skip_flag != 0.0f);
     if ((int)blockIdx.x >= nb_main) {
-        env_backward_block((int)blockIdx.x - nb_main, env_job);
+        env_backward_block((int)blockIdx.x - nb_main, env_job, ad, update);
         return;
     }
-    const int i = blockIdx.x * 256 + threadIdx.x;
-    if (i >= P) return;
-    const size_t i3 = 3 * (size_t)i, i4 = 4 * (size_t)i;
-    const float4* gf = reinterpret_cast<const float4*>(dL_dfeatures + 16 * (size_t)i);
-    const float4 f0 = gf[0], f1 = gf[1], f2 = gf[2];
-    {
-        const float gfeat[3] = {f2.x, f2.y, f2.z};
-#pragma unroll
-        for (int c = 0; c < 3; c++) {
-            const float s = sigmoidf_(base_raw[i3 + c]);
-            g_base[i3 + c] = (gfeat[c] + dL_dbase_shade[i3 + c]) * 0.77f * s * (1.f - s);
-        }
-        const float s = sigmoidf_(rough_raw[i]);
-        g_rough[i] = (f2.w + dL_drough_shade[i]) * 0.9f * s * (1.f - s);
-    }
-    if (g_xyz == nullptr) return;
-
-#pragma unroll
-    for (int c = 0; c < 3; c++) g_scaling[i3 + c] = dL_dscales[i3 + c] * __expf(scaling_raw[i3 + c]);
-    {
-        const float q[4] = {rotation_raw[i4], rotation_raw[i4 + 1], rotation_raw[i4 + 2], rotation_raw[i4 + 3]};
-        const float g[4] = {dL_drot[i4], dL_drot[i4 + 1], dL_drot[i4 + 2], dL_drot[i4 + 3]};
-        const float n = sqrtf(q[0] * q[0] + q[1] * q[1] + q[2] * q[2] + q[3] * q[3]);
-        if (n > 1e-12f) {
-            const float inv = 1.f / n;
-            const float u[4] = {q[0] / n, q[1] / n, q[2] / n, q[3] / n};
-            const float d = u[0] * g[0] + u[1] * g[1] + u[2] * g[2] + u[3] * g[3];
-#pragma unroll
-            for (int c = 0; c < 4; c++) g_rotation[i4 + c] = (g[c] - u[c] * d) * inv;
-        } else {
-#pragma unroll
-            for (int c = 0; c < 4; c++) g_rotation[i4 + c] = g[c] * 1e12f;
-        }
-    }
-    {
-        const float s = sigmoidf_(opacity_raw[i]);
-        g_opacity[i] = dL_dopacity[i] * s * (1.f - s);
-    }
-    {
-        const float v[3] = {normal_raw[i3], normal_raw[i3 + 1], normal_raw[i3 + 2]};
-        const float g[3] = {f1.y, f1.z, f1.w};
-        float o[3];
-        normalize3_backward(v, 1e-3f, g, o);
-        g_normal[i3] = o[0]; g_normal[i3 + 1] = o[1]; g_normal[i3 + 2] = o[2];
-    }
-    {
-        const float p[3] = {xyz[i3], xyz[i3 + 1], xyz[i3 + 2]};
-        const float depth = p[0] * viewmatrix[2] + p[1] * viewmatrix[6] + p[2] * viewmatrix[10] + viewmatrix[14];
-        const float gd = f0.x + 2.f * depth * f0.y;
-        const float d[3] = {campos[0] - p[0], campos[1] - p[1], campos[2] - p[2]};
-        const float gv[3] = {dL_dviewdirs[i3], dL_dviewdirs[i3 + 1], dL_dviewdirs[i3 + 2]};
-        float gdd[3];
-        normalize3_backward(d, 1e-12f, gv, gdd);
-        g_xyz[i3] = dL_dmeans3D[i3] + gd * viewmatrix[2] - gdd[0];
-        g_xyz[i3 + 1] = dL_dmeans3D[i3 + 1] + gd * viewmatrix[6] - gdd[1];
-        g_xyz[i3 + 2] = dL_dmeans3D[i3 + 2] + gd * viewmatrix[10] - gdd[2];
-    }
+    __shared__ __align__(16) float s_g[CLOSE_LDS_FLOATS];
+    const int t = threadIdx.x;
+    const int i = blockIdx.x * 256 + t;
+    const bool geometry = g_xyz != nullptr;
+    const int rows = min(256, P - (int)blockIdx.x * 256);
+    if (i < P) {
+        const size_t i3 = 3 * (size_t)i, i4 = 4 * (size_t)i;
+        const float4* gf = reinterpret_cast<const float4*>(dL_dfeatures + 16 * (size_t)i);
+        const float4 f0 = gf[0], f1 = gf[1], f2 = gf[2];
+        {
+            const float gfeat[3] = {f2.x, f2.y, f2.z};
+#pragma unroll
+            for (int c = 0; c < 3; c++) {
+                const float s = sigmoidf_(base_raw[i3 + c]);
+                s_g[CLOSE_SEG_BASE + 3 * t + c] = (gfeat[c] + dL_dbase_shade[i3 + c]) * 0.77f * s * (1.f - s);
+            }
+            const float s = sigmoidf_(rough_raw[i]);
+            s_g[CLOSE_SEG_ROUGH + t] = (f2.w + dL_drough_shade[i]) * 0.9f * s * (1.f - s);
+        }
+        if (geometry) {
+#pragma unroll
+            for (int c = 0; c < 3; c++) s_g[CLOSE_SEG_SCALING + 3 * t + c] = dL_dscales[i3 + c] * __expf(scaling_raw[i3 + c]);
+            {
+                float* g_rotation_t = s_g + CLOSE_SEG_ROTATION + 4 * t;
+                const float q[4] = {rotation_raw[i4], rotation_raw[i4 + 1], rotation_raw[i4 + 2], rotation_raw[i4 + 3]};
+                const float g[4] = {dL_drot[i4], dL_drot[i4 + 1], dL_drot[i4 + 2], dL_drot[i4 + 3]};
+                const float n = sqrtf(q[0] * q[0] + q[1] * q[1] + q[2] * q[2] + q[3] * q[3]);
+                if (n > 1e-12f) {
+                    const float inv = 1.f / n;
+                    const float u[4] = {q[0] / n, q[1] / n, q[2] / n, q[3] / n};
+                    const float d = u[0] * g[0] + u[1] * g[1] + u[2] * g[2] + u[3] * g[3];
+#pragma unroll
+                    for (int c = 0; c < 4; c++) g_rotation_t[c] = (g[c] - u[c] * d) * inv;
+                } else {
+#pragma unroll
+                    for (int c = 0; c < 4; c++) g_rotation_t[c] = g[c] * 1e12f;
+                }
+            }
+            {
+                const float s = sigmoidf_(opacity_raw[i]);
+                s_g[CLOSE_SEG_OPACITY + t] = dL_dopacity[i] * s * (1.f - s);
+            }
+            {
+                const float v[3] = {normal_raw[i3], normal_raw[i3 + 1], normal_raw[i3 + 2]};
+                const float g[3] = {f1.y, f1.z, f1.w};
+                float o[3];
+                normalize3_backward(v, 1e-3f, g, o);
+                float* g_normal_t = s_g + CLOSE_SEG_NORMAL + 3 * t;
+                g_normal_t[0] = o[0]; g_normal_t[1] = o[1]; g_normal_t[2] = o[2];
+            }
+            {
+                const float p[3] = {xyz[i3], xyz[i3 + 1], xyz[i3 + 2]};
+                const float depth = p[0] * viewmatrix[2] + p[1] * viewmatrix[6] + p[2] * viewmatrix[10] + viewmatrix[14];
+                const float gd = f0.x + 2.f * depth * f0.y;
+                const float d[3] = {campos[0] - p[0], campos[1] - p[1], campos[2] - p[2]};
+                const float gv[3] = {dL_dviewdirs[i3], dL_dviewdirs[i3 + 1], dL_dviewdirs[i3 + 2]};
+                float gdd[3];
+                normalize3_backward(d, 1e-12f, gv, gdd);
+                float* g_xyz_t = s_g + CLOSE_SEG_XYZ + 3 * t;
+                g_xyz_t[0] = dL_dmeans3D[i3] + gd * viewmatrix[2] - gdd[0];
+                g_xyz_t[1] = dL_dmeans3D[i3 + 1] + gd * viewmatrix[6] - gdd[1];
+                g_xyz_t[2] = dL_dmeans3D[i3 + 2] + gd * viewmatrix[10] - gdd[2];
+            }
+        }
+    }
+    __syncthreads();
+    const bool v4 = vec != 0;
+    close_write<3>(g_base, s_g + CLOSE_SEG_BASE, rows, v4);
+    close_write<1>(g_rough, s_g + CLOSE_SEG_ROUGH, rows, v4);
+    if (geometry) {
+        close_write<3>(g_xyz, s_g + CLOSE_SEG_XYZ, rows, v4);
+        close_write<3>(g_scaling, s_g + CLOSE_SEG_SCALING, rows, v4);
+        close_write<4>(g_rotation, s_g + CLOSE_SEG_ROTATION, rows, v4);
+        close_write<1>(g_opacity, s_g + CLOSE_SEG_OPACITY, rows, v4);
+        close_write<3>(g_normal, s_g + CLOSE_SEG_NORMAL, rows, v4);
+    }
+    if (!update) return;
+    const float* spare = dL_dfeatures + 16 * 256 * (size_t)blockIdx.x;
+    CloseRegs r0, r1, r2, r3;
+    close_load<4>(rotation_raw, rows, ad.g[2], spare, r0);
+    close_load<3>(xyz, rows, ad.g[0], spare, r1);
+    close_load<3>(scaling_raw, rows, ad.g[1], spare, r2);
+    close_load<3>(normal_raw, rows, ad.g[4], spare, r3);
+    close_finish<4>(rotation_raw, s_g + CLOSE_SEG_ROTATION, rows, ad, ad.g[2], r0);
+    close_load<3>(base_raw, rows, ad.g[5], spare, r0);
+    close_finish<3>(xyz, s_g + CLOSE_SEG_XYZ, rows, ad, ad.g[0], r1);
+    close_load<1>(opacity_raw, rows, ad.g[3], spare, r1);
+    close_finish<3>(scaling_raw, s_g + CLOSE_SEG_SCALING, rows, ad, ad.g[1], r2);
+    close_load<1>(rough_raw, rows, ad.g[6], spare, r2);
+    close_finish<3>(normal_raw, s_g + CLOSE_SEG_NORMAL, rows, ad, ad.g[4], r3);
+    close_finish<3>(base_raw, s_g + CLOSE_SEG_BASE, rows, ad, ad.g[5], r0);
+    close_finish<1>(opacity_raw, s_g + CLOSE_SEG_OPACITY, rows, ad, ad.g[3], r1);
+    close_finish<1>(rough_raw, s_g + CLOSE_SEG_ROUGH, rows, ad, ad.g[6], r2);
 }
 
 __global__ void __launch_bounds__(256)
@@ -439,17 +549,22 @@
                                  const float* dL_drot, const float* dL_dopacity, const float* dL_dmeans3D, float* g_xyz,
                                  float* g_scaling, float* g_rotation, float* g_opacity, float* g_normal, float* g_base,
                                  float* g_rough, int He, int We, const float* env_raw, const float* env, float* dL_denv,
-                                 float w_tv, float* g_env_raw, float* tv_sum, int consume)
+                                 float w_tv, float* g_env_raw, float* tv_sum, int consume, const CloseAdam* adam)
 {
     EnvBackward job;
     job.He = He; job.We = We; job.raw = env_raw; job.env = env; job.dL_denv = dL_denv; job.w_tv = w_tv; job.g_raw = g_env_raw;
     job.tv_sum = tv_sum; job.consume = consume;
     const int nb_main = (P + 255) / 256;
     const int nb_env = env_raw != nullptr ? (He * We * 3 + 255) / 256 : 0;
+    if (nb_main + nb_env == 0) return;
+    const uintptr_t low = (uintptr_t)g_xyz | (uintptr_t)g_scaling | (uintptr_t)g_rotation | (uintptr_t)g_opacity |
+                          (uintptr_t)g_normal | (uintptr_t)g_base | (uintptr_t)g_rough;
+    const CloseAdam none = {};
     s2_activate_backward_kernel<<<nb_main + nb_env, 256, 0, s>>>(
         P, xyz, scaling_raw, rotation_raw, opacity_raw, normal_raw, base_raw, rough_raw, viewmatrix, campos,
         dL_dfeatures, dL_dbase_shade, dL_drough_shade, dL_dviewdirs, dL_dscales, dL_drot, dL_dopacity, dL_dmeans3D, g_xyz,
-        g_scaling, g_rotation, g_opacity, g_normal, g_base, g_rough, nb_main, job);
+        g_scaling, g_rotation, g_opacity, g_normal, g_base, g_rough, nb_main, job, (low & 15) == 0 ? 1 : 0,
+        adam != nullptr ? *adam : none);
     check_launch(s, false, "s2_activate_backward_kernel");
 }
 
diff --git a/relightable3dgaussian_amd/fused_adam.py b/relightable3dgaussian_amd/fused_adam.py
--- a/relightable3dgaussian_amd/fused_adam.py
+++ b/relightable3dgaussian_amd/fused_adam.py
@@ -40,6 +40,21 @@
         return (C.addressof(self._fused_desc), self.betas[0], self.betas[1], self.eps, int(step), float(grad_scale),
                 skip_flag.data_ptr() if skip_flag is not None else None)
 
+    def fused_steps_of(self, indices, step, grad_scale=1.0, skip_flag=None):
+        descs = []
+        for i in indices:
+            if i is None:
+                descs.append(None)
+                continue
+            g = self.groups[i]
+            p = g["param"]
+            descs.append(AdamGroup(p.data_ptr(), None, g["exp_avg"].data_ptr(), g["exp_avg_sq"].data_ptr(), p.numel(),
+                                   g["lr"], g["lr_tail"], g.get("period", 0), g.get("split", 0)))
+        table = (C.c_void_p * len(descs))(*[None if d is None else C.addressof(d) for d in descs])
+        self._fused_table = (table, descs)
+        return (C.cast(table, C.POINTER(C.c_void_p)), self.betas[0], self.betas[1], self.eps, int(step), float(grad_scale),
+                skip_flag.data_ptr() if skip_flag is not None else None)
+
     def step_groups(self, indices, grads, grad_scale=1.0, skip_flag=None):
         L = _lib.lib()
         indices = list(indices)
diff --git a/relightable3dgaussian_amd/fused_step.py b/relightable3dgaussian_amd/fused_step.py
--- a/relightable3dgaussian_amd/fused_step.py
+++ b/relightable3dgaussian_amd/fused_step.py
@@ -98,6 +98,7 @@
             self._samples.acquire(self.xyz, self.a_scales, self.a_rot, self.a_opacity, self.a_normal)
         self._pre_rotated = None
         self._chain_deferred = None
+        self._closed = ()
         two_rates = lambda k: dict(lr_tail=tail(k), period=3 * self.M, split=3) if k in ("shs", "incidents") else {}
         self.opt = FusedAdam([dict(param=raw[k], lr=rate(k), **two_rates(k)) for k in self._opt_order])
         live = lambda idx: tuple(i for i in idx if self._opt_order[i] not in self.frozen)
@@ -183,7 +184,7 @@
 
     @_in_context
     def forward_backward(self, cam, bg, gt, early_adam=False, image_mask=None, split_geometry=None, chain_incidents=False,
-                         gt_depth=None, mvs_normal=None, sh_adam_in_backward=False):
+                         gt_depth=None, mvs_normal=None, sh_adam_in_backward=False, close_in_chain_rule=False):
         H, W = cam.image_height, cam.image_width
         if self._supervised and (gt_depth is None or (self.w["normal_mvs_depth"] != 0.0 and mvs_normal is None)):
             raise RuntimeError("FusedStage2Step: the depth / normal_mvs_depth terms need gt_depth%s" % (
@@ -201,7 +202,8 @@
             dL_dfeatures, bw, geo_stream, handle_a = self._raster_backward(
                 v, fw, g, active, early_adam if split_geometry is None else split_geometry, fused_a)
             b_early = self._schedule_early(v, handle_a, geo_stream, use_bounded, early_adam, chain_incidents, fused_a)
-            self._shade_backward(v, env_c, taps, packed, dL_dfeatures, bw, geo_stream, b_early, chain_incidents)
+            self._shade_backward(v, env_c, taps, packed, dL_dfeatures, bw, geo_stream, b_early, chain_incidents,
+                                 close_in_chain_rule)
             self._remaining_buckets(handle_a)
         return self._end_forward_backward(fw, None if bw is None else bw[0], use_bounded, v.N)
 
@@ -391,7 +393,18 @@
                 _lib.stream_wait(v.order_stream, side)
         return b_early
 
-    def _shade_backward(self, v, env_c, taps, packed, dL_dfeatures, bw, geo_stream, b_early, chain_incidents):
+    _CLOSED_BY_CHAIN_RULE = ("xyz", "scaling", "rotation", "opacity", "normal", "base_color", "roughness", "env")
+
+    def _closes_in_chain_rule(self, L):
+        switch = os.environ.get("R3DG_CLOSE_IN_CHAIN_RULE")
+        if switch == "0" or self.dp or self.frozen_geometry or not self._groups_c:
+            return False
+        if switch != "1" and self.dev.type != "cuda":
+            return False
+        return L.r3dg_stage2_activate_backward_adam_supported() == 1
+
+    def _shade_backward(self, v, env_c, taps, packed, dL_dfeatures, bw, geo_stream, b_early, chain_incidents,
+                        close_in_chain_rule=False):
         L = _lib.lib()
         P, gr = self.P, self.grads
         _lib.check(L.r3dg_stage2_unpack_gradients(
@@ -425,11 +438,20 @@
                    self.w["env_smooth"], gr["env"].data_ptr(), self.sums[4].data_ptr(), 1)
         geo = (lambda t: None) if self.frozen_geometry else (lambda t: t.data_ptr())
         _means2D, _dcol, dL_dopacity, dL_dmeans3D, _dfeat, _dcov, _dsh, dL_dscales, dL_drot = bw or (None,) * 9
-        _lib.check(L.r3dg_stage2_activate_backward_with(v.raw, P, geo(self.xyz), geo(self.scaling), geo(self.rotation),
+        args = (v.raw, P, geo(self.xyz), geo(self.scaling), geo(self.rotation),
             geo(self.opacity), geo(self.normal), self.base_color.data_ptr(), self.roughness.data_ptr(), geo(v.vm), geo(v.campos),
             dL_dfeatures.data_ptr(), d_base.data_ptr(), d_rough.data_ptr(), geo(d_view), geo(dL_dscales), geo(dL_drot),
             geo(dL_dopacity), geo(dL_dmeans3D), geo(gr["xyz"]), geo(gr["scaling"]), geo(gr["rotation"]), geo(gr["opacity"]),
-            geo(gr["normal"]), gr["base_color"].data_ptr(), gr["roughness"].data_ptr(), *env_job), "stage2_activate_backward")
+            geo(gr["normal"]), gr["base_color"].data_ptr(), gr["roughness"].data_ptr(), *env_job)
+        self._closed = ()
+        if close_in_chain_rule and self._closes_in_chain_rule(L):
+            table = [self._opt_order.index(k) if k not in self.frozen else None for k in self._CLOSED_BY_CHAIN_RULE]
+            step = self.opt.step_count if self._early else self.opt.step_count + 1
+            _lib.check(L.r3dg_stage2_activate_backward_adam(*args, *self.opt.fused_steps_of(table, step, 1.0, self._skip_cur)),
+                       "stage2_activate_backward_adam")
+            self._closed = tuple(i for i in table if i is not None)
+        else:
+            _lib.check(L.r3dg_stage2_activate_backward_with(*args), "stage2_activate_backward")
 
     def _remaining_buckets(self, handle_a):
         comm, it = self._comm, self._iter
@@ -474,6 +496,7 @@
                 self.opt.begin_step()
                 todo = self._groups_a + self._groups_c + self._groups_b
             self._early = self._b_early = self._a_late = False
+            todo, self._closed = tuple(i for i in todo if i not in self._closed), ()
             if todo:
                 self.opt.step_groups(todo, grads, skip_flag=self._skip_cur)
                 if set(todo) & set(self._groups_b):
@@ -550,6 +573,7 @@
     def __call__(self, cam, bg, gt, image_mask=None, gt_depth=None, mvs_normal=None):
         early = os.environ.get("R3DG_EARLY_ADAM", "1" if self.P <= 1_000_000 else "0") != "0" and not self.serial_streams
         outs = self.forward_backward(cam, bg, gt, early_adam=early, image_mask=image_mask, chain_incidents=True,
-                                     gt_depth=gt_depth, mvs_normal=mvs_normal, sh_adam_in_backward=True)
+                                     gt_depth=gt_depth, mvs_normal=mvs_normal, sh_adam_in_backward=True,
+                                     close_in_chain_rule=True)
         self.optimizer_step()
         return outs
```

Measured after the change: 838.4 iters/s (median of 6 runs). About the same (+0.4%).
